# zouyunkai/MedicalSemSeg

Measured on AMD Instinct MI355X. Metric: 96^3 vols/sec fwd+bwd (train), higher is better.
Workload: dtype bf16; 1 GPU; UNet base (MONAI BasicUNet 32-32-64-128-256-32) 1->3cls, 96^3 patches, DiceCE + AdamW, per-GPU batch 2; global_batch=2, parallelism=dp1, grad_sync=none (single rank)

## Files before the change

### include/msseg.h

```cpp
#ifndef MSSEG_H_
#define MSSEG_H_

#include <stddef.h>
#include <stdint.h>

#ifdef __cplusplus
extern "C" {
#endif

#define MSSEG_ABI_VERSION 1

#define MSSEG_OK 0
#define MSSEG_EINVAL (-1)
#define MSSEG_ELAUNCH (-2)
#define MSSEG_EWORKSPACE (-3)

#define MSSEG_F32 0
#define MSSEG_BF16 1

typedef void* msseg_stream_t;

int msseg_abi_version(void);
const char* msseg_last_error(void);
int msseg_num_cus(void);

int msseg_ktimer_enable(int on);
int msseg_ktimer_reset(void);
int msseg_ktimer_count(void);
int msseg_ktimer_get(int i, char* name, int cap, float* ms);

size_t msseg_packed_weight_bytes(int M, int T, int K, int cout_block, int dtype);
int msseg_pack_weights(const float* src, void* dst, int dtype, int M, int M0, int T, int K, int K0,
                       long long s_m1, long long s_m0, long long s_t, long long s_k1, long long s_k0,
                       int flip, int cout_block, msseg_stream_t stream);
typedef struct msseg_pack_job {
    const float* src;
    void* dst;
    long long s_m1, s_m0, s_t, s_k1, s_k0;
    long long total;
    int M, M0, T, K, K0, flip, cout_block, nkb;
} msseg_pack_job;
int msseg_pack_weights_batch(const msseg_pack_job* jobs_dev, int njobs, long long max_total, long long sum_total, int dtype,
                             msseg_stream_t stream);
int msseg_cout_block(int M);
int msseg_conv3d_k3_cout_block(int N, int D, int H, int W, int Cout);
int msseg_conv3d_k3_variant(int N, int D, int H, int W, int Cout);
int msseg_conv3d_k3_kernel(int N, int D, int H, int W, int Cin, int Cout, int dtype);

int msseg_conv3d_k3_fwd(const void* x, long long ldx, const void* wp, const float* bias, void* y, long long ldy,
                        int N, int D, int H, int W, int Cin, int Cout, float* stats ,
                        void* scratch, size_t scratch_bytes, int dtype, msseg_stream_t stream);
int msseg_conv3d_k3_fwd_accumulate(const void* x, long long ldx, const void* wp, void* y, long long ldy, int N, int D, int H,
                                   int W, int Cin, int Cout, float* stats, void* scratch, size_t scratch_bytes, int dtype,
                                   msseg_stream_t stream);
int msseg_conv3d_k3_dgrad_inbwd(const void* dy, long long lddy, const void* wp, void* da, long long ldda, int N, int D,
                                int H, int W, int Cin, int Cout, const void* yraw, long long ldyraw, const void* act,
                                long long ldact, const float* fwd_stats, float slope, float eps, float* red,
                                float* dgamma, float* dbeta, int accumulate, void* scratch, size_t scratch_bytes,
                                int dtype, msseg_stream_t stream);
int msseg_conv3d_k3s2_fwd(const void* x, long long ldx, const void* wp, const float* bias, void* y, long long ldy,
                          int N, int ID, int IH, int IW, int Cin, int Cout, int dtype, msseg_stream_t stream);
int msseg_zero_stuff2(const void* dy, long long lddy, void* out, long long ldo, int N, int OD, int OH, int OW, int ID,
                      int IH, int IW, int C, int dtype, msseg_stream_t stream);
int msseg_conv3d_stem_fwd(const void* x, long long ldx, const void* wp, const float* bias, void* y, long long ldy,
                          int N, int D, int H, int W, int Cout, float* stats, void* scratch, size_t scratch_bytes,
                          int dtype, msseg_stream_t stream);
int msseg_conv3d_stem_k1_fwd(const void* x, long long ldx, const void* wp, const float* bias, void* y, long long ldy,
                             int N, int D, int H, int W, int Cout, float* stats, void* scratch, size_t scratch_bytes,
                             int dtype, msseg_stream_t stream);
int msseg_conv3d_stem_norm_fwd(const void* x, long long ldx, const void* wp, const float* bias, const float* stats,
                               const float* gamma, const float* beta, float eps, float slope, void* y, long long ldy, int N,
                               int D, int H, int W, int Cout, int dtype, msseg_stream_t stream);
int msseg_conv3d_k1_fwd(const void* x, long long ldx, const void* wp, const float* bias, void* y, long long ldy,
                        long long NV, int Cin, int Cout, int dtype, msseg_stream_t stream);
int msseg_conv3d_k1_head_fwd(const void* x, long long ldx, const float* w, const float* bias, void* y, long long ldy,
                             long long NV, int Cin, int Cout, int dtype, msseg_stream_t stream);
int msseg_conv3d_k1_head_dgrad_inbwd(const void* dy, long long lddy, const float* w, void* da, long long ldda, int N,
                                     long long S, int C, int Cout, const void* yraw, long long ldyraw,
                                     const float* fwd_stats, const float* gamma, const float* beta, float slope, float eps,
                                     float* red, float* dgamma, float* dbeta, int accumulate, void* scratch,
                                     size_t scratch_bytes, int dtype, msseg_stream_t stream);
int msseg_conv3d_k1_head_norm_fwd(const void* x, long long ldx, const float* stats, const float* gamma, const float* beta,
                                  float slope, float eps, const float* w, const float* bias, void* y, long long ldy, int N,
                                  long long S, int Cin, int Cout, int dtype, msseg_stream_t stream);
int msseg_conv3d_k1_head_bwd_fused(const void* dy, long long lddy, const float* w, void* da, long long ldda, int N,
                                   long long S, int C, int Cout, const void* yraw, long long ldyraw, const float* fwd_stats,
                                   const float* gamma, const float* beta, float slope, float eps, float* red, float* dgamma,
                                   float* dbeta, int accumulate, float* dw, int dw_accumulate, void* scratch,
                                   size_t scratch_bytes, int dtype, msseg_stream_t stream);

int msseg_conv3d_gather_fwd(const void* x, long long ldx, const void* wp, const float* bias, void* y, long long ldy,
                            int N, int ID, int IH, int IW, int Cin, int Cout, int k, int s, int p, int dtype,
                            msseg_stream_t stream);
int msseg_deconv_k2s2_fwd(const void* x, long long ldx, const void* wp, const float* bias, void* y, long long ldy,
                          int N, int D, int H, int W, int Cin, int Cout, int dtype, msseg_stream_t stream);
int msseg_deconv_k2s2_bwd_data(const void* dy, long long lddy, const void* wp, void* dx, long long lddx,
                               int N, int D, int H, int W, int Cin, int Cout, int dtype, msseg_stream_t stream);
int msseg_conv3d_k1_dgrad_inbwd(const void* dy, long long lddy, const void* wp, void* da, long long ldda, int N,
                                long long S, int Cin, int Cout, const void* yraw, long long ldyraw, const void* act,
                                long long ldact, const float* fwd_stats, float slope, float eps, float* red,
                                float* dgamma, float* dbeta, int accumulate, void* scratch, size_t scratch_bytes,
                                int dtype, msseg_stream_t stream);
int msseg_deconv_k2s2_bwd_data_inbwd(const void* dy, long long lddy, const void* wp, void* dx, long long lddx, int N,
                                     int D, int H, int W, int Cin, int Cout, const void* yraw, long long ldyraw,
                                     const void* act, long long ldact, const float* fwd_stats, float slope, float eps,
                                     float* red, float* dgamma, float* dbeta, int accumulate, void* scratch,
                                     size_t scratch_bytes, int dtype, msseg_stream_t stream);
int msseg_deconv_k2s2_bwd_fused(const void* dy, long long lddy, const void* wp, void* dx, long long lddx, int N,
                                int D, int H, int W, int Cin, int Cout, const void* yraw, long long ldyraw,
                                const void* act, long long ldact, const float* fwd_stats, float slope, float eps,
                                float* red, float* dgamma, float* dbeta, int accumulate, float* dbias, int dbias_accumulate,
                                void* scratch, size_t scratch_bytes, int dtype, msseg_stream_t stream);

int msseg_deconv_k2s2_bwd_partials_ok(int Cin, int Cout, int dtype);
int msseg_deconv_k2s2_bwd_partials(const void* dy, long long lddy, const void* wp, float* part, size_t part_bytes, int N,
                                   int D, int H, int W, int Cin, int Cout, int dtype, msseg_stream_t stream);


size_t msseg_wgrad_workspace_bytes(int M, int T, int K);
int msseg_conv3d_k3_wgrad_kernel(int N, int D, int H, int W, int Cin, int Cout, int dtype);
int msseg_conv3d_k3_wgrad(const void* x, long long ldx, const void* dy, long long lddy, float* dw,
                          int N, int D, int H, int W, int Cin, int Cout, int accumulate,
                          void* workspace, size_t workspace_bytes, int dtype, msseg_stream_t stream);
int msseg_conv3d_k1_wgrad(const void* x, long long ldx, const void* dy, long long lddy, float* dw,
                          long long NV, int Cin, int Cout, int accumulate,
                          void* workspace, size_t workspace_bytes, int dtype, msseg_stream_t stream);
int msseg_linear_wgrad_ok(long long NV, int Cin, int Cout, int dtype);
int msseg_linear_wgrad(const void* x, long long ldx, const void* dy, long long lddy, float* dw, float* dbias, long long NV,
                       int Cin, int Cout, int accumulate_w, int accumulate_b, void* workspace, size_t workspace_bytes,
                       int dtype, msseg_stream_t stream);
int msseg_conv3d_gather_wgrad(const void* x, long long ldx, const void* dy, long long lddy, float* dw,
                              int N, int ID, int IH, int IW, int Cin, int Cout, int k, int s, int p, int accumulate,
                              void* workspace, size_t workspace_bytes, int dtype, msseg_stream_t stream);
int msseg_deconv_k2s2_wgrad(const void* x, long long ldx, const void* dy, long long lddy, float* dw,
                            int N, int D, int H, int W, int Cin, int Cout, int accumulate,
                            void* workspace, size_t workspace_bytes, int dtype, msseg_stream_t stream);

int msseg_conv3d_k3_small_ok(int N, int D, int H, int W, int Cin, int Cout, int dtype);
int msseg_conv3d_k3_small_stage_groups(int N, int D, int H, int W, int Cin, int Cout);
size_t msseg_conv3d_k3_small_workspace_bytes(int N, int D, int H, int W, int Cin, int Cout);
int msseg_conv3d_k3_small_partials(const void* x, long long ldx, const void* wp, float* part, size_t part_bytes, int N,
                                   int D, int H, int W, int Cin, int Cout, msseg_stream_t stream);
int msseg_conv3d_k3_small_fwd_finish(const float* part, int nstages, const float* bias, const float* gamma,
                                     const float* beta, float eps, float slope, void* yraw, long long ldy, void* act,
                                     long long lda, void* pooled, long long ldp, float* stats, int N, int D, int H, int W,
                                     int Cout, msseg_stream_t stream);
int msseg_conv3d_k3_small_fwd_finish_res(const float* part, int nstages, const float* bias, const float* gamma,
                                         const float* beta, float eps, float slope, void* yraw, long long ldy, void* act,
                                         long long lda, const void* residual, long long ldr, void* pooled, long long ldp,
                                         float* stats, int N, int D, int H, int W, int Cout, msseg_stream_t stream);
int msseg_conv3d_k3_small_bwd_finish(const float* part, int nstages, void* dx, long long lddx, const void* unit_yraw,
                                     long long lduy, const float* unit_stats, const float* unit_gamma,
                                     const float* unit_beta, float eps, float slope, float* dgamma, float* dbeta,
                                     int accumulate, int N, int D, int H, int W, int Cin, msseg_stream_t stream);

int msseg_dwconv3d_k3_fwd(const void* x, long long ldx, const void* w_taps, const float* bias, void* y, long long ldy, int N,
                          int D, int H, int W, int C, int flip, int dtype, msseg_stream_t stream);
int msseg_avgpool3d_k3(const void* x, long long ldx, void* y, long long ldy, int N, int D, int H, int W, int C, int dtype,
                       msseg_stream_t stream);
int msseg_dwconv3d_k3_wgrad(const void* x, long long ldx, const void* dy, long long lddy, float* dw, float* dbias,
                            int accumulate_w, int accumulate_b, int N, int D, int H, int W, int C, void* scratch,
                            size_t scratch_bytes, int dtype, msseg_stream_t stream);

int msseg_interp_trilinear_fwd(const void* x, long long ldx, void* y, long long ldy, int N, int ID, int IH, int IW, int OD,
                               int OH, int OW, int C, int dtype, msseg_stream_t stream);
size_t msseg_interp_trilinear_bwd_workspace_bytes(int N, int ID, int IH, int IW, int OD, int OH, int OW, int C);
int msseg_interp_trilinear_bwd(const void* dy, long long lddy, void* dx, long long lddx, int N, int ID, int IH, int IW, int OD,
                               int OH, int OW, int C, void* workspace, size_t workspace_bytes, int dtype, msseg_stream_t stream);
int msseg_kv_attention_fwd(const void* q, const void* kv, void* o, float* lse, int B, int N, int M, int heads, int head_dim,
                           float scale, int dtype, msseg_stream_t stream);
size_t msseg_kv_attention_bwd_workspace_bytes(int B, int N, int M, int heads, int head_dim);
int msseg_kv_attention_bwd(const void* q, const void* kv, const void* o, const float* lse, const void* dout, void* dq, void* dkv,
                           int B, int N, int M, int heads, int head_dim, float scale, void* workspace, size_t workspace_bytes,
                           int dtype, msseg_stream_t stream);
int msseg_scale_channels(const void* x, const float* scale, void* y, int N, long long S, int C, int dtype, msseg_stream_t stream);

size_t msseg_reduce_scratch_bytes(void);
int msseg_channel_stats(const void* x, long long ldx, float* stats, int N, long long S, int C, void* scratch,
                        size_t scratch_bytes, int dtype, msseg_stream_t stream);
int msseg_instnorm_act_fwd(const void* x, long long ldx, const float* stats, const float* gamma, const float* beta,
                           const void* residual, long long ldr, void* y, long long ldy, int N, long long S, int C,
                           float eps, float slope, int dtype, msseg_stream_t stream);
int msseg_instnorm_act_pool_fwd(const void* x, long long ldx, const float* stats, const float* gamma, const float* beta,
                                void* y, long long ldy, void* pooled, long long ldp, int N, int D, int H, int W, int C,
                                float eps, float slope, int dtype, msseg_stream_t stream);
int msseg_instnorm_act_poolbwd_reduce(const void* x, long long ldx, const float* stats, const float* gamma,
                                      const float* beta, const void* skip, long long lds, const void* g, long long ldg,
                                      void* da, long long ldda, float* red, float* dgamma, float* dbeta, int accumulate,
                                      int N, int D, int H, int W, int C, float eps, float slope, void* scratch,
                                      size_t scratch_bytes, int dtype, msseg_stream_t stream);
int msseg_instnorm_act_bwd_reduce(const void* x, long long ldx, const float* stats, const float* gamma,
                                  const float* beta, const void* y, long long ldy,
                                  const void* dy, long long lddy, float* red, float* dgamma, float* dbeta,
                                  int accumulate, int N, long long S, int C, float eps, float slope, void* scratch,
                                  size_t scratch_bytes, int dtype, msseg_stream_t stream);
int msseg_instnorm_act_bwd_apply(const void* x, long long ldx, const float* stats, const float* gamma,
                                 const float* beta, const void* y, long long ldy, const void* dy, long long lddy, const float* red, void* dx,
                                 long long lddx, void* dres, long long lddres, int N, long long S, int C, float eps,
                                 float slope, int dtype, msseg_stream_t stream);
int msseg_maxpool2_fwd(const void* x, long long ldx, void* y, long long ldy, int N, int D, int H, int W, int C,
                       int dtype, msseg_stream_t stream);
int msseg_maxpool2_bwd(const void* x, long long ldx, const void* dy, long long lddy, void* dx, long long lddx,
                       int N, int D, int H, int W, int C, int accumulate, int dtype, msseg_stream_t stream);
int msseg_ncdhw_to_ndhwc(const void* src, int src_dtype, void* dst, long long ldd, int dst_dtype, int N, int C,
                         long long S, msseg_stream_t stream);
int msseg_ndhwc_to_ncdhw(const void* src, long long lds, int src_dtype, void* dst, int dst_dtype, int N, int C,
                         long long S, msseg_stream_t stream);
int msseg_channel_sum(const void* x, long long ldx, float* out, long long rows, int C, int accumulate, void* scratch,
                      size_t scratch_bytes, int dtype, msseg_stream_t stream);
int msseg_add(const void* a, long long lda, const void* b, long long ldb, void* y, long long ldy, long long rows,
              int C, int dtype, msseg_stream_t stream);
int msseg_axpy_rows(const void* a, const void* b, const float* scale, void* y, int N, long long elems_per_sample, int dtype,
                    msseg_stream_t stream);


int msseg_window_attention_fwd(const void* qkv, const float* qkv_bias, const float* table, void* out, float* lse, int B,
                               int S, int H, int W, int C, int heads, int ws, int shift, int dtype,
                               msseg_stream_t stream);
int msseg_window_attention_bwd(const void* qkv, const float* qkv_bias, const float* table, const void* out,
                               const float* lse, const void* dout, void* dqkv, float* dtable, int B, int S, int H, int W,
                               int C, int heads, int ws, int shift, int dtype, msseg_stream_t stream);
size_t msseg_window_attention_bwd_workspace_bytes(int B, int S, int H, int W, int C, int heads, int ws, int shift, int dtype);
int msseg_window_attention_fwd2(const void* qkv, const float* qkv_bias, const float* table, void* out, float* lse, int B,
                                int S, int H, int W, int C, int heads, int ws, int shift, int bias_ws, int dtype,
                                msseg_stream_t stream);
int msseg_window_attention_bwd2(const void* qkv, const float* qkv_bias, const float* table, const void* out,
                                const float* lse, const void* dout, void* dqkv, float* dtable, int B, int S, int H, int W,
                                int C, int heads, int ws, int shift, int bias_ws, int dtype, void* workspace,
                                size_t workspace_bytes, msseg_stream_t stream);
int msseg_window_attention_bwd_ws(const void* qkv, const float* qkv_bias, const float* table, const void* out,
                                  const float* lse, const void* dout, void* dqkv, float* dtable, int B, int S, int H, int W,
                                  int C, int heads, int ws, int shift, int dtype, void* workspace, size_t workspace_bytes,
                                  msseg_stream_t stream);
int msseg_window_attention_fwd3(const void* qkv, const float* qkv_bias, const float* table, void* out, float* lse, int B,
                                int S, int H, int W, int C, int heads, int ws, int shift, int bias_ws, long long table_stride,
                                int dtype, msseg_stream_t stream);
int msseg_window_attention_bwd3(const void* qkv, const float* qkv_bias, const float* table, const void* out,
                                const float* lse, const void* dout, void* dqkv, float* dtable, int B, int S, int H, int W,
                                int C, int heads, int ws, int shift, int bias_ws, long long table_stride, int dtype,
                                void* workspace, size_t workspace_bytes, msseg_stream_t stream);
size_t msseg_window_attention_bwd3_workspace_bytes(int B, int S, int H, int W, int C, int heads, int ws, int shift,
                                                   int bias_ws, long long table_stride, int dtype);
int msseg_rel_bias_affine_fold(const float* table, const float* emb, const float* lin_w, const float* lin_b,
                               const float* aff, float* T, int B, int M3, int heads, msseg_stream_t stream);
size_t msseg_rel_bias_affine_grad_workspace_bytes(int M3, int heads);
#define MSSEG_AFFINE_ACC_TABLE 1
#define MSSEG_AFFINE_ACC_EMB 2
#define MSSEG_AFFINE_ACC_LIN_W 4
#define MSSEG_AFFINE_ACC_LIN_B 8
int msseg_rel_bias_affine_grad(const float* dT, const float* emb, const float* lin_w, const float* aff, float* dtable,
                               float* demb, float* dlin_w, float* dlin_b, int B, int M3, int heads, int flags,
                               void* workspace, size_t workspace_bytes, msseg_stream_t stream);
int msseg_layernorm_fwd(const void* x, long long ldx, const float* gamma, const float* beta, void* y, long long ldy,
                        float* mean, float* rstd, long long rows, int C, float eps, int dtype, msseg_stream_t stream);
int msseg_layernorm_bwd(const void* x, long long ldx, const float* gamma, const float* mean, const float* rstd,
                        const void* dy, long long lddy, void* dx, long long lddx, long long rows, int C, int dtype,
                        msseg_stream_t stream);
int msseg_layernorm_bwd_add(const void* x, long long ldx, const float* gamma, const float* mean, const float* rstd,
                            const void* dy, long long lddy, const void* add, long long ldadd, void* dx, long long lddx,
                            long long rows, int C, int dtype, msseg_stream_t stream);
int msseg_layernorm_param_grad(const void* x, long long ldx, const float* mean, const float* rstd, const void* dy,
                               long long lddy, float* dgamma, float* dbeta, int accumulate, long long rows, int C,
                               void* scratch, size_t scratch_bytes, int dtype, msseg_stream_t stream);
int msseg_gelu_fwd(const void* x, void* y, long long n, int dtype, msseg_stream_t stream);
int msseg_gelu_bwd(const void* x, const void* dy, void* dx, long long n, int dtype, msseg_stream_t stream);
int msseg_linear_gelu_ok(long long NV, int Cin, int Cout, int dtype);
int msseg_linear_gelu_fwd(const void* x, long long ldx, const void* wp, const float* bias, void* pre, long long ldpre, void* act,
                          long long ldact, long long NV, int Cin, int Cout, int dtype, msseg_stream_t stream);
int msseg_linear_gelu_bwd(const void* dy, long long lddy, const void* wp, const void* pre, long long ldpre, void* dpre,
                          long long lddpre, long long NV, int Cin, int Cout, int dtype, msseg_stream_t stream);
int msseg_linear_add_ok(long long NV, int Cin, int Cout, int dtype);
int msseg_linear_add_fwd(const void* x, long long ldx, const void* wp, const float* bias, const void* res, long long ldres,
                         void* y, long long ldy, long long NV, int Cin, int Cout, int dtype, msseg_stream_t stream);

int msseg_dice_ce_partials(const void* logits, long long ld, int dtype, const void* labels, int label_dtype,
                           float* partial, float* hard, int N, long long S, int C, msseg_stream_t stream);
// ... 56 lines not shown
```

### medicalsemseg_amd/csrc/conv3d_k3_wgrad_pp.hip

```cpp
#include "k3pp.h"

#include <stdlib.h>

#include <type_traits>

namespace {

constexpr int TD = 4, TH = 4, TW = 16;
constexpr int PD = TD + 2, PH = TH + 2, PW = TW + 2;
constexpr int PWP = PW;
constexpr int HV = PD * PH * PWP;
constexpr int TV = TD * TH * TW;
constexpr int Q_BYTES = HV * 64;
constexpr int P_BYTES = TV * 64;
constexpr int GRP_BYTES = Q_BYTES + P_BYTES;
constexpr int NIQ = (HV + 15) / 16;
constexpr int NIP = TV / 16;
constexpr int NIQ_W = (NIQ + 3) / 4, NIP_W = NIP / 4;
constexpr int NKS = TV / 16;
constexpr int TAPW = 7;
constexpr int NTHREADS = 512;
constexpr int SLAB_FLOATS = 27 * 32 * 32;

__device__ u32x4_t g_wg_zero_chunk;
__device__ unsigned long long g_k3wg_cycles[8];

MSSEG_DEVFN void glds16(const void* g, void* l) {
    __builtin_amdgcn_global_load_lds((const __attribute__((address_space(1))) void*)g,
                                     (__attribute__((address_space(3))) void*)l, 16, 0, 0);
}

typedef __attribute__((address_space(3))) unsigned char lds_u8;
typedef __attribute__((ext_vector_type(16))) float f32x16_t;

MSSEG_DEVFN bf16x4_t lds_tr(lds_u8* p) {
    return __builtin_amdgcn_ds_read_tr16_b64_v4bf16((__attribute__((address_space(3))) bf16x4_t*)p);
}

MSSEG_DEVFN u32x4_t tr_frag(lds_u8* r0, lds_u8* r1) {
    const bf16x4_t lo = lds_tr(r0), hi = lds_tr(r1);
    const bf16x8_t f = {lo[0], lo[1], lo[2], lo[3], hi[0], hi[1], hi[2], hi[3]};
    return __builtin_bit_cast(u32x4_t, f);
}

struct TileCo { int n, d0, h0, w0; };

constexpr int ks_row(int ks) { return ((ks / TH) * PH + ks % TH) * PWP; }

template <int TIMING>
__global__ __launch_bounds__(NTHREADS, 1) void k3wg_pp_kernel(const K3WgParams p) {
    extern __shared__ __attribute__((aligned(256))) unsigned char smem[];
    const int tid = threadIdx.x, lane = tid & 63;
    const int wave = __builtin_amdgcn_readfirstlane(tid >> 6);
    const int grp = wave >> 2, wq = wave & 3;
    lds_u8* smem3 = (lds_u8*)smem;
    unsigned char* ldsQ = smem + grp * GRP_BYTES;
    unsigned char* ldsP = ldsQ + Q_BYTES;
    const int mblk = blockIdx.y / p.kblks, kblk = blockIdx.y % p.kblks;
    const unsigned char* pg = (const unsigned char*)p.pten + mblk * 64;
    const unsigned char* qg = (const unsigned char*)p.qten + kblk * 64;

    const int tiles_w = (p.W + TW - 1) / TW, tiles_h = (p.H + TH - 1) / TH, tiles_d = (p.D + TD - 1) / TD;
    const int ntiles = p.N * tiles_d * tiles_h * tiles_w;
    int t_first, t_step, t_end;
    if ((gridDim.x & 7) == 0) {
        const int chunk = (ntiles + 7) >> 3, xcd = blockIdx.x & 7;
        t_first = xcd * chunk + (blockIdx.x >> 3);
        t_step = gridDim.x >> 3;
        t_end = min(ntiles, (xcd + 1) * chunk);
    } else {
        t_first = blockIdx.x; t_step = gridDim.x; t_end = ntiles;
    }
    const int n_my = t_first < t_end ? (t_end - t_first + t_step - 1) / t_step : 0;
    auto tile_of = [&](int k) {
        int t = t_first + k * t_step;
        TileCo tc;
        tc.w0 = (t % tiles_w) * TW; t /= tiles_w;
        tc.h0 = (t % tiles_h) * TH; t /= tiles_h;
        tc.d0 = (t % tiles_d) * TD; t /= tiles_d;
        tc.n = t;
        return tc;
    };

    const int lrow = lane >> 2;
    const int lchunk = lane & 3;
    constexpr unsigned SKIP = 0xffffffffu;
    unsigned q_off[NIQ_W], p_off[NIP_W];
#pragma unroll
    for (int j = 0; j < NIQ_W; ++j) {
        const int hv = (wq + 4 * j) * 16 + lrow;
        const int hd = hv / (PH * PWP), rem = hv - hd * (PH * PWP), hh = rem / PWP, hw = rem - hh * PWP;
        q_off[j] = (hv < HV && hw < PW) ? (unsigned)((((long long)hd * p.H + hh) * p.W + hw) * p.ldq * 2 + lchunk * 16) : SKIP;
    }
#pragma unroll
    for (int j = 0; j < NIP_W; ++j) {
        const int tv = (wq + 4 * j) * 16 + lrow;
        const int td = tv / (TH * TW), th = (tv / TW) % TH, tw = tv % TW;
        p_off[j] = (unsigned)((((long long)td * p.H + th) * p.W + tw) * p.ldp * 2 + lchunk * 16);
    }
    const bool p_cok = mblk * 32 + lchunk * 8 < p.M, q_cok = kblk * 32 + lchunk * 8 < p.K;
    const bool chunks_full = (mblk + 1) * 32 <= p.M && (kblk + 1) * 32 <= p.K;
    auto load_tile = [&](const TileCo& tc) {
        const int dB = tc.d0 - 1, hB = tc.h0 - 1, wB = tc.w0 - 1;
        const long long qvox = (((long long)tc.n * p.D + dB) * p.H + hB) * p.W + wB;
        const long long pvox = (((long long)tc.n * p.D + tc.d0) * p.H + tc.h0) * p.W + tc.w0;
        const unsigned char* qb = qg + qvox * p.ldq * 2;
        const unsigned char* pb = pg + pvox * p.ldp * 2;
        const bool interior = chunks_full && dB >= 0 && dB + PD <= p.D && hB >= 0 && hB + PH <= p.H && wB >= 0 && wB + PW <= p.W;
        if (interior) {
#pragma unroll
            for (int j = 0; j < NIQ_W; ++j) {
                if (q_off[j] != SKIP) glds16(qb + q_off[j], ldsQ + (wq + 4 * j) * 1024);
            }
#pragma unroll
            for (int j = 0; j < NIP_W; ++j) glds16(pb + p_off[j], ldsP + (wq + 4 * j) * 1024);
        } else {
            const unsigned char* zsrc = (const unsigned char*)&g_wg_zero_chunk;
#pragma unroll
            for (int j = 0; j < NIQ_W; ++j) {
                const int it = wq + 4 * j;
                const int hv = it * 16 + lrow;
                const int hd = hv / (PH * PWP), rem = hv - hd * (PH * PWP), hh = rem / PWP, hw = rem - hh * PWP;
                const bool inb = q_cok && (unsigned)(dB + hd) < (unsigned)p.D && (unsigned)(hB + hh) < (unsigned)p.H &&
                                 (unsigned)(wB + hw) < (unsigned)p.W;
                const unsigned char* src = inb ? qb + q_off[j] : zsrc;
                if (q_off[j] != SKIP) glds16(src, ldsQ + it * 1024);
            }
#pragma unroll
            for (int j = 0; j < NIP_W; ++j) {
                const int tv = (wq + 4 * j) * 16 + lrow;
                const int td = tv / (TH * TW), th = (tv / TW) % TH, tw = tv % TW;
                const bool inb = p_cok && tc.d0 + td < p.D && tc.h0 + th < p.H && tc.w0 + tw < p.W;
                const unsigned char* src = inb ? pb + p_off[j] : zsrc;
                glds16(src, ldsP + (wq + 4 * j) * 1024);
            }
        }
    };

    const int G = lane >> 4, qr = (lane >> 2) & 3, pc = lane & 3;
    const unsigned qbase = grp * GRP_BYTES, pbase = qbase + Q_BYTES;
    unsigned p_rd[2], q_rd[TAPW][2];
#pragma unroll
    for (int i = 0; i < 2; ++i) {
        const int lrow = 8 * (G >> 1) + 4 * i + qr;
        p_rd[i] = pbase + lrow * 64 + ((G & 1) << 5) + pc * 8;
#pragma unroll
        for (int tt = 0; tt < TAPW; ++tt) {
            int tap = wq * TAPW + tt;
            if (tap > 26) tap = 26;
            const int row = ((tap / 9) * PH + ((tap / 3) % 3)) * PWP + (tap % 3) + lrow;
            q_rd[tt][i] = qbase + row * 64 + ((G & 1) << 5) + pc * 8;
        }
    }

    f32x16_t acc[TAPW];
#pragma unroll
    for (int t = 0; t < TAPW; ++t)
#pragma unroll
        for (int e = 0; e < 16; ++e) acc[t][e] = 0.f;

    auto compute = [&]() {
        constexpr int NSTEP = NKS * TAPW;
        constexpr int QA = 2;
        u32x4_t pf[2], qf[QA + 1];
        auto ldp = [&](int ks) { pf[ks & 1] = tr_frag(smem3 + p_rd[0] + ks * 1024, smem3 + p_rd[1] + ks * 1024); };
        auto ldq = [&](int s) {
            const int ks = s / TAPW, tt = s % TAPW;
            qf[s % (QA + 1)] = tr_frag(smem3 + q_rd[tt][0] + ks_row(ks) * 64, smem3 + q_rd[tt][1] + ks_row(ks) * 64);
        };
        ldp(0);
#pragma unroll
        for (int s = 0; s < QA; ++s) ldq(s);
#pragma unroll
        for (int ks = 0; ks < NKS; ++ks) {
#pragma unroll
            for (int tt = 0; tt < TAPW; ++tt) {
                const int s = ks * TAPW + tt;
                if (s + QA < NSTEP) ldq(s + QA);
                if (tt == 0 && ks + 1 < NKS) ldp(ks + 1);
                __builtin_amdgcn_sched_barrier(0);
                acc[tt] = __builtin_amdgcn_mfma_f32_32x32x16_bf16(__builtin_bit_cast(bf16x8_t, pf[ks & 1]),
                                                                  __builtin_bit_cast(bf16x8_t, qf[s % (QA + 1)]),
                                                                  acc[tt], 0, 0, 0);
                __builtin_amdgcn_sched_barrier(0);
            }
        }
    };

    if (grp == 0 && n_my > 0) load_tile(tile_of(0));
    asm volatile("s_waitcnt vmcnt(0)" ::: "memory");
    __syncthreads();

    unsigned long long tcyc[4] = {0, 0, 0, 0};
    for (int ph = 0; ph < n_my; ++ph) {
        unsigned long long t0 = 0;
        if constexpr (TIMING) t0 = __builtin_readcyclecounter();
        if ((ph & 1) == grp) {
            compute();
            if constexpr (TIMING) tcyc[0] += __builtin_readcyclecounter() - t0;
        } else {
            if (ph + 1 < n_my && !(TIMING && p.dbg_noload)) load_tile(tile_of(ph + 1));
            if constexpr (TIMING) tcyc[1] += __builtin_readcyclecounter() - t0;
        }
        if constexpr (TIMING) t0 = __builtin_readcyclecounter();
        asm volatile("s_waitcnt vmcnt(0)" ::: "memory");
        if constexpr (TIMING) { tcyc[2] += __builtin_readcyclecounter() - t0; t0 = __builtin_readcyclecounter(); }
        __syncthreads();
        if constexpr (TIMING) tcyc[3] += __builtin_readcyclecounter() - t0;
    }
    if constexpr (TIMING) {
        if (blockIdx.x == 0 && blockIdx.y == 0 && lane == 0 && wave == 0) {
#pragma unroll
            for (int k = 0; k < 4; ++k) g_k3wg_cycles[k] = tcyc[k];
        }
    }

    float* xch = (float*)smem;
    const int col = lane & 31, rb = 4 * (lane >> 5);
    const int tap0 = wq * TAPW;
    if (grp == 1) {
#pragma unroll
        for (int tt = 0; tt < TAPW; ++tt) {
            if (tap0 + tt < 27) {
#pragma unroll
                for (int e = 0; e < 16; ++e)
                    xch[((tap0 + tt) * 32 + (e & 3) + 8 * (e >> 2) + rb) * 32 + col] = acc[tt][e];
            }
        }
    }
    __syncthreads();
    if (grp == 0) {
        float* slab = p.slabs + ((long long)blockIdx.y * gridDim.x + blockIdx.x) * SLAB_FLOATS;
#pragma unroll
        for (int tt = 0; tt < TAPW; ++tt) {
            if (tap0 + tt < 27) {
#pragma unroll
                for (int e = 0; e < 16; ++e) {
                    const int idx = ((tap0 + tt) * 32 + (e & 3) + 8 * (e >> 2) + rb) * 32 + col;
                    slab[idx] = acc[tt][e] + xch[idx];
                }
            }
        }
    }
}

}

bool msseg_k3wg_pp_eligible(const K3WgParams& p) {
    static const bool off = getenv("MSSEG_NO_K3PP") != nullptr;
    if (off) return false;
    if (p.M % 8 || p.K % 8) return false;
    if ((p.ldp % 8) || (p.ldq % 8) || ((uintptr_t)p.pten & 15) || ((uintptr_t)p.qten & 15)) return false;
    const long long ldm = p.ldp > p.ldq ? p.ldp : p.ldq;
    if ((long long)(PD + 1) * p.H * p.W * ldm * 2 >= 0x7fffffffLL) return false;
    const long long tiles = (long long)p.N * ceil_div(p.D, TD) * ceil_div(p.H, TH) * ceil_div(p.W, TW);
    if (tiles > 0x7fffffffLL) return false;
    return tiles * ceil_div(p.M, 32) * ceil_div(p.K, 32) >= 2LL * msseg_num_cus();
}

int msseg_k3wg_pp_grid(const K3WgParams& p) {
    const int pairs = ceil_div(p.M, 32) * ceil_div(p.K, 32);
    const int tiles = p.N * ceil_div(p.D, TD) * ceil_div(p.H, TH) * ceil_div(p.W, TW);
    int gx = msseg_num_cus() / pairs;
    gx &= ~7;
    if (gx < 8) gx = 8;
    if (gx > tiles) gx = tiles;
    return gx;
}

int msseg_k3wg_pp_launch(const K3WgParams& p, int gx, hipStream_t stream) {
    static const bool timing = getenv("MSSEG_K3PP_TIMING") != nullptr;
    static const bool noload = getenv("MSSEG_K3PP_NOLOAD") != nullptr;
    K3WgParams pl = p;
    pl.dbg_noload = noload ? 1 : 0;
    const int lds = 2 * GRP_BYTES;
    static msseg_lds_attr_once attr[2];
    if (!attr[0].ensure((const void*)k3wg_pp_kernel<0>, lds) || !attr[1].ensure((const void*)k3wg_pp_kernel<1>, lds))
        MSSEG_FAIL(MSSEG_ELAUNCH, "conv3d_k3_wgrad_pp: cannot set dynamic LDS size %d", lds);
    const int pairs = ceil_div(p.M, 32) * ceil_div(p.K, 32);
    if (timing) hipLaunchKernelGGL(k3wg_pp_kernel<1>, dim3(gx, pairs, 1), dim3(NTHREADS), lds, stream, pl);
    else MSSEG_KTIMED("k3wg_pp_kernel", stream, hipLaunchKernelGGL(k3wg_pp_kernel<0>, dim3(gx, pairs, 1), dim3(NTHREADS), lds, stream, pl));
    MSSEG_CHECK_LAUNCH("conv3d_k3_wgrad_pp");
    return MSSEG_OK;
}

extern "C" int msseg_debug_k3wg_cycles(unsigned long long* out4) {
    return hipMemcpyFromSymbol(out4, HIP_SYMBOL(g_k3wg_cycles), 4 * sizeof(unsigned long long)) == hipSuccess ? 0 : -1;
}
```

### medicalsemseg_amd/csrc/elementwise.hip

```cpp
#include "common.h"

#include <stdarg.h>
#include <string.h>

static thread_local char g_err[512] = "";
void msseg_set_error(const char* fmt, ...) {
    va_list ap;
    va_start(ap, fmt);
    vsnprintf(g_err, sizeof(g_err), fmt, ap);
    va_end(ap);
}

extern "C" {
int msseg_abi_version(void) { return MSSEG_ABI_VERSION; }
const char* msseg_last_error(void) { return g_err; }
int msseg_num_cus(void) {
    static int cus = 0;
    if (cus == 0) {
        int dev = 0;
        hipDeviceProp_t prop;
        if (hipGetDevice(&dev) == hipSuccess && hipGetDeviceProperties(&prop, dev) == hipSuccess)
            cus = prop.multiProcessorCount;
        if (cus <= 0) cus = 256;
    }
    return cus;
}
}

namespace {

template <typename T> struct Chunk {
    static constexpr int EPC = DT<T>::EPC;
    float v[EPC];
    MSSEG_DEVFN void load(const T* p) {
        if constexpr (sizeof(T) == 4) {
            f32x4_t t = *(const f32x4_t*)p;
#pragma unroll
            for (int e = 0; e < 4; ++e) v[e] = t[e];
        } else {
            bf16x8_t t = *(const bf16x8_t*)p;
#pragma unroll
            for (int e = 0; e < 8; ++e) v[e] = (float)t[e];
        }
    }
    MSSEG_DEVFN void store(T* p) const {
        if constexpr (sizeof(T) == 4) {
            f32x4_t t = {v[0], v[1], v[2], v[3]};
            *(f32x4_t*)p = t;
        } else {
            bf16x8_t t;
#pragma unroll
            for (int e = 0; e < 8; ++e) t[e] = (bf16_t)v[e];
            *(bf16x8_t*)p = t;
        }
    }
};

inline bool vec_ok(const void* p, long long ld, int C, int esz) {
    const int epc = 16 / esz;
    return (C % epc) == 0 && (ld % epc) == 0 && (((uintptr_t)p) & 15) == 0;
}

struct RowMap {
    int groups;
    int rows_par;
};
inline RowMap row_map(int C, int width, int nthr = 256) {
    RowMap m;
    m.groups = ceil_div(C, width);
    if (m.groups > nthr) m.groups = nthr;
    m.rows_par = nthr / m.groups;
    if (m.rows_par < 1) m.rows_par = 1;
    return m;
}

MSSEG_DEVFN void finalize_channels(const float* ws, int N, int nblk, int C, int nper, int mode, float* out,
                                   float* dp0, float* dp1, int accumulate) {
    __shared__ float fin[256];
    const int L = C * nper;
    const int cols = L < 256 ? L : 256;
    const int G = 256 / cols;
    const int col = threadIdx.x % cols, rg = threadIdx.x / cols;
    const bool in256 = threadIdx.x < 256;
    const int n_step = mode == 0 ? (int)gridDim.y : 1, n_first = mode == 0 ? (int)blockIdx.y : 0;
    for (int c0 = blockIdx.x * cols; c0 < L; c0 += gridDim.x * cols) {
        const int o = c0 + col;
        const bool ok = in256 && o < L && rg < G;
        float tot = 0.f;
        for (int n = n_first; n < N; n += n_step) {
            float s = 0.f;
            if (ok) {
                const float* src = ws + (long long)n * nblk * L + o;
#pragma unroll 16
                for (int bb = rg; bb < nblk; bb += G) s += src[(long long)bb * L];
            }
            __syncthreads();
            if (in256) fin[threadIdx.x] = s;
            __syncthreads();
            if (ok && rg == 0) {
                float t = 0.f;
                for (int g = 0; g < G; ++g) t += fin[g * cols + col];
                if (mode != 1) out[(long long)n * L + o] = t;
                tot += t;
            }
        }
        if (ok && rg == 0) {
            if (mode == 1) {
                out[o] = accumulate ? out[o] + tot : tot;
            } else if (mode == 2) {
                const int c = o / nper, k = o % nper;
                float* dp = (k == 0) ? dp0 : dp1;
                if (dp) dp[c] = accumulate ? dp[c] + tot : tot;
            }
        }
    }
}

struct FinalizeArgs {
    const float* ws; int N, nblk, C, nper, mode; float* out; float* dp0; float* dp1; int accumulate;
};
__global__ __launch_bounds__(256) void channels_finalize_kernel(const FinalizeArgs a) {
    finalize_channels(a.ws, a.N, a.nblk, a.C, a.nper, a.mode, a.out, a.dp0, a.dp1, a.accumulate);
}

static inline dim3 channels_finalize_grid(const FinalizeArgs& a) {
    const int L = a.C * a.nper;
    int gx = (L + 255) / 256;
    if (gx > 64) gx = 64;
    if (gx < 1) gx = 1;
    return dim3((unsigned)gx, a.mode == 0 ? (unsigned)(a.N < 1 ? 1 : a.N) : 1u);
}

constexpr int RED_THREADS = 512;
constexpr int RED_STAGE2 = 16;

template <int W>
MSSEG_DEVFN void block_rows_reduce(float* red, int groups, int rows_par, int g, int rl, bool act) {
    if (act && rl < RED_STAGE2 && rl < rows_par) {
#pragma unroll
        for (int e = 0; e < W; ++e) {
            float a = 0.f, b = 0.f;
            for (int k = rl; k < rows_par; k += RED_STAGE2) {
                a += red[((k * groups + g) * W + e) * 2 + 0];
                b += red[((k * groups + g) * W + e) * 2 + 1];
            }
            red[((rl * groups + g) * W + e) * 2 + 0] = a;
            red[((rl * groups + g) * W + e) * 2 + 1] = b;
        }
    }
    __syncthreads();
}

template <typename T, bool VEC>
// ... 44 lines not shown
#pragma unroll
            for (int e = 0; e < W; ++e) {
                float a = 0.f, b = 0.f;
                for (int k = 0; k < kmax; ++k) {
                    a += red[((k * groups + g) * W + e) * 2 + 0];
                    b += red[((k * groups + g) * W + e) * 2 + 1];
                }
                const int c = gg * W + e;
                wsb[c * nacc + 0] = a;
                if (nacc == 2) wsb[c * nacc + 1] = b;
            }
        }
    }
}

template <typename T, bool VEC>
__global__ __launch_bounds__(256) void ln_param_grad_kernel(const T* __restrict__ x, long long ldx,
                                                            const T* __restrict__ dy, long long lddy,
                                                            const float* __restrict__ mean, const float* __restrict__ rstd,
                                                            long long rows, int C, int groups, int rows_par,
                                                            long long rows_per_block, float* ws, unsigned int* counter,
                                                            float* dgamma, float* dbeta, int accumulate) {
    constexpr int W = VEC ? DT<T>::EPC : 1;
    __shared__ float red[256 * 2 * (VEC ? DT<T>::EPC : 1)];
    __shared__ int lflag;
    const int g = threadIdx.x % groups, rl = threadIdx.x / groups;
    const long long r0 = (long long)blockIdx.x * rows_per_block;
    long long r1 = r0 + rows_per_block;
    if (r1 > rows) r1 = rows;
    float* wsb = ws + (long long)blockIdx.x * C * 2;
    for (int gbase = 0; gbase * W < C; gbase += groups) {
        const int gg = gbase + g;
        const bool act = gg * W < C;
        float s[W], s2[W];
#pragma unroll
        for (int e = 0; e < W; ++e) s[e] = s2[e] = 0.f;
        if (act && rl < rows_par) {
#pragma unroll 4
            for (long long r = r0 + rl; r < r1; r += rows_par) {
                const float mu = mean[r], rs = rstd[r];
                if constexpr (VEC) {
                    Chunk<T> cx, cd;
                    cx.load(x + r * ldx + gg * W);
                    cd.load(dy + r * lddy + gg * W);
#pragma unroll
                    for (int e = 0; e < W; ++e) { s[e] += cd.v[e] * (cx.v[e] - mu) * rs; s2[e] += cd.v[e]; }
                } else {
                    const float d = DT<T>::ld(dy + r * lddy + gg);
                    s[0] += d * (DT<T>::ld(x + r * ldx + gg) - mu) * rs;
                    s2[0] += d;
                }
            }
        }
        __syncthreads();
#pragma unroll
        for (int e = 0; e < W; ++e) {
            red[(threadIdx.x * W + e) * 2 + 0] = s[e];
            red[(threadIdx.x * W + e) * 2 + 1] = s2[e];
        }
        __syncthreads();
        if (act && rl == 0) {
#pragma unroll
            for (int e = 0; e < W; ++e) {
                float a = 0.f, b = 0.f;
                for (int k = 0; k < rows_par; ++k) {
                    a += red[((k * groups + g) * W + e) * 2 + 0];
                    b += red[((k * groups + g) * W + e) * 2 + 1];
                }
                wsb[(gg * W + e) * 2 + 0] = a;
                wsb[(gg * W + e) * 2 + 1] = b;
            }
        }
    }
}

inline long long reduce_blocks(long long S, int rows_par, int N, int C, int nper);

template <typename T>
int launch_ln_param_grad(const void* x, long long ldx, const void* dy, long long lddy, const float* mean, const float* rstd,
                         float* dgamma, float* dbeta, int accumulate, long long rows, int C, void* scratch, hipStream_t st) {
    const bool vec = vec_ok(x, ldx, C, sizeof(T)) && vec_ok(dy, lddy, C, sizeof(T));
    const RowMap m = row_map(C, vec ? DT<T>::EPC : 1);
    long long blocks = reduce_blocks(rows, m.rows_par, 1, C, 2);
    const long long rpb = ceil_div_ll(rows, blocks);
    blocks = ceil_div_ll(rows, rpb);
    unsigned int* counter = (unsigned int*)scratch;
    float* ws = (float*)((unsigned char*)scratch + MSSEG_SCRATCH_COUNTER_BYTES);
    if (vec)
        hipLaunchKernelGGL((ln_param_grad_kernel<T, true>), dim3((unsigned)blocks), dim3(256), 0, st, (const T*)x, ldx,
                           (const T*)dy, lddy, mean, rstd, rows, C, m.groups, m.rows_par, rpb, ws, counter, dgamma, dbeta, accumulate);
    else
        hipLaunchKernelGGL((ln_param_grad_kernel<T, false>), dim3((unsigned)blocks), dim3(256), 0, st, (const T*)x, ldx,
                           (const T*)dy, lddy, mean, rstd, rows, C, m.groups, m.rows_par, rpb, ws, counter, dgamma, dbeta, accumulate);
    MSSEG_CHECK_LAUNCH("ln_param_grad");
    {
        FinalizeArgs a{ws, 1, (int)blocks, C, 2, 2, ws + blocks * C * 2, dgamma, dbeta, accumulate};
        hipLaunchKernelGGL(channels_finalize_kernel, channels_finalize_grid(a), dim3(256), 0, st, a);
        MSSEG_CHECK_LAUNCH("channels_finalize");
    }
    return MSSEG_OK;
}

inline long long reduce_blocks(long long S, int rows_par, int N, int C, int nper) {
    long long blocks = ceil_div_ll(S, (long long)rows_par * 8);
    long long cap = (long long)msseg_num_cus() / (N > 0 ? N : 1);
    if (cap < 1) cap = 1;
    const long long fit = (long long)(((size_t)16 << 20) / ((size_t)N * C * nper * 4));
    if (cap > fit) cap = fit;
    if (blocks > cap) blocks = cap;
    if (blocks < 1) blocks = 1;
    return blocks;
}

template <typename T>
int launch_stats(const void* x, long long ldx, float* out, int N, long long S, int C, int nacc, int accumulate,
                 void* scratch, hipStream_t st) {
    const bool vec = vec_ok(x, ldx, C, sizeof(T));
    const RowMap m = row_map(C, vec ? DT<T>::EPC : 1, RED_THREADS);
    long long blocks = reduce_blocks(S, m.rows_par, N, C, nacc);
    const long long rpb = ceil_div_ll(S, blocks);
    blocks = ceil_div_ll(S, rpb);
    dim3 grid((unsigned)blocks, N);
    unsigned int* counter = (unsigned int*)scratch;
    float* ws = (float*)((unsigned char*)scratch + MSSEG_SCRATCH_COUNTER_BYTES);
    if (vec)
        hipLaunchKernelGGL((channel_stats_kernel<T, true>), grid, dim3(RED_THREADS), 0, st, (const T*)x, ldx, out, S, C,
                           m.groups, m.rows_par, rpb, nacc, accumulate, ws, counter);
    else
        hipLaunchKernelGGL((channel_stats_kernel<T, false>), grid, dim3(RED_THREADS), 0, st, (const T*)x, ldx, out, S, C,
                           m.groups, m.rows_par, rpb, nacc, accumulate, ws, counter);
    MSSEG_CHECK_LAUNCH("channel_stats");
    {
        FinalizeArgs a{ws, N, (int)blocks, C, nacc, nacc == 2 ? 0 : 1, out, nullptr, nullptr, accumulate};
        hipLaunchKernelGGL(channels_finalize_kernel, channels_finalize_grid(a), dim3(256), 0, st, a);
        MSSEG_CHECK_LAUNCH("channels_finalize");
    }
    return MSSEG_OK;
}

struct NormParams {
    const void* x; long long ldx;
    const float* stats; const float* gamma; const float* beta;
    const void* res; long long ldr;
    void* y; long long ldy;
    const void* dy; long long lddy;
    float* red;
    void* dx; long long lddx;
    void* dres; long long lddres;
    long long S; int C; float eps, slope;
    long long rows_per_block; int groups, rows_par;
    float* ws; unsigned int* counter; float* dgamma; float* dbeta; int accumulate;
};

MSSEG_DEVFN void mean_rstd(const float* stats, int n, int C, int c, long long S, float eps, float& mean, float& rstd) {
    const float inv = 1.0f / (float)S;
    const float s = stats[((long long)n * C + c) * 2 + 0], s2 = stats[((long long)n * C + c) * 2 + 1];
    mean = s * inv;
    float var = s2 * inv - mean * mean;
    var = var > 0.f ? var : 0.f;
    rstd = rsqrtf(var + eps);
}

template <typename T, bool VEC, int MODE>
__global__ __launch_bounds__(MODE == 1 ? RED_THREADS : 256) void instnorm_kernel(const NormParams p) {
    constexpr int W = VEC ? DT<T>::EPC : 1;
    __shared__ float red[(MODE == 1) ? RED_THREADS * 2 * W : 1];
    __shared__ int lflag;
    const int n = blockIdx.y;
    const int g = threadIdx.x % p.groups, rl = threadIdx.x / p.groups;
    const long long r0 = (long long)blockIdx.x * p.rows_per_block;
    long long r1 = r0 + p.rows_per_block;
    if (r1 > p.S) r1 = p.S;
    const T* xn = (const T*)p.x + (long long)n * p.S * p.ldx;
    const T* yn = (MODE != 0 && p.y != nullptr) ? (const T*)p.y + (long long)n * p.S * p.ldy : nullptr;
    T* yo = (MODE == 0) ? (T*)p.y + (long long)n * p.S * p.ldy : nullptr;
    const T* dyn = (MODE != 0) ? (const T*)p.dy + (long long)n * p.S * p.lddy : nullptr;
    const T* resn = (MODE == 0 && p.res) ? (const T*)p.res + (long long)n * p.S * p.ldr : nullptr;
    T* dxn = (MODE == 2) ? (T*)p.dx + (long long)n * p.S * p.lddx : nullptr;
    T* drn = (MODE == 2 && p.dres) ? (T*)p.dres + (long long)n * p.S * p.lddres : nullptr;
    const float invS = 1.0f / (float)p.S;

    for (int gbase = 0; gbase * W < p.C; gbase += p.groups) {
        const int gg = gbase + g;
        const bool act = gg * W < p.C;
        float mean[W], rstd[W], sc[W], sh[W], k0[W], k1[W], a0[W], a1[W];
#pragma unroll
        for (int e = 0; e < W; ++e) {
            const int c = act ? gg * W + e : 0;
            mean_rstd(p.stats, n, p.C, c, p.S, p.eps, mean[e], rstd[e]);
            const float ga = p.gamma ? p.gamma[c] : 1.f;
            sc[e] = rstd[e] * ga;
            sh[e] = (p.beta ? p.beta[c] : 0.f) - mean[e] * sc[e];
            a0[e] = a1[e] = 0.f;
            if constexpr (MODE == 2) {
                k0[e] = p.red[((long long)n * p.C + c) * 2 + 0] * invS;
                k1[e] = p.red[((long long)n * p.C + c) * 2 + 1] * invS;
            }
        }
        if (act && rl < p.rows_par) {
#pragma unroll 4
            for (long long r = r0 + rl; r < r1; r += p.rows_par) {
                float xv[W], o[W], yv[W], dv[W];
                if constexpr (VEC) {
                    Chunk<T> c; c.load(xn + r * p.ldx + gg * W);
#pragma unroll
                    for (int e = 0; e < W; ++e) xv[e] = c.v[e];
                } else {
                    xv[0] = DT<T>::ld(xn + r * p.ldx + gg);
                }
                if constexpr (MODE == 0) {
                    float rv[W];
#pragma unroll
                    for (int e = 0; e < W; ++e) rv[e] = 0.f;
                    if (resn) {
                        if constexpr (VEC) {
                            Chunk<T> c; c.load(resn + r * p.ldr + gg * W);
#pragma unroll
                            for (int e = 0; e < W; ++e) rv[e] = c.v[e];
                        } else {
                            rv[0] = DT<T>::ld(resn + r * p.ldr + gg);
                        }
                    }
#pragma unroll
                    for (int e = 0; e < W; ++e) {
                        const float z = xv[e] * sc[e] + sh[e] + rv[e];
                        o[e] = z > 0.f ? z : z * p.slope;
                    }
                    if constexpr (VEC) {
                        Chunk<T> c;
#pragma unroll
                        for (int e = 0; e < W; ++e) c.v[e] = o[e];
                        c.store(yo + r * p.ldy + gg * W);
                    } else {
                        DT<T>::st(yo + r * p.ldy + gg, o[0]);
                    }
                } else {
                    if constexpr (VEC) {
                        Chunk<T> d; d.load(dyn + r * p.lddy + gg * W);
#pragma unroll
                        for (int e = 0; e < W; ++e) dv[e] = d.v[e];
                        if (yn != nullptr) {
                            Chunk<T> c; c.load(yn + r * p.ldy + gg * W);
#pragma unroll
                            for (int e = 0; e < W; ++e) yv[e] = c.v[e];
                        } else {
#pragma unroll
                            for (int e = 0; e < W; ++e) yv[e] = xv[e] * sc[e] + sh[e];
                        }
                    } else {
                        dv[0] = DT<T>::ld(dyn + r * p.lddy + gg);
                        yv[0] = (yn != nullptr) ? DT<T>::ld(yn + r * p.ldy + gg) : xv[0] * sc[0] + sh[0];
                    }
#pragma unroll
                    for (int e = 0; e < W; ++e) {
                        const float dz = yv[e] > 0.f ? dv[e] : dv[e] * p.slope;
                        const float xh = (xv[e] - mean[e]) * rstd[e];
                        if constexpr (MODE == 1) {
                            a0[e] += dz;
                            a1[e] += dz * xh;
                        } else {
                            o[e] = sc[e] * (dz - k0[e] - xh * k1[e]);
                            dv[e] = dz;
                        }
                    }
                    if constexpr (MODE == 2) {
                        if constexpr (VEC) {
                            Chunk<T> c;
#pragma unroll
                            for (int e = 0; e < W; ++e) c.v[e] = o[e];
                            c.store(dxn + r * p.lddx + gg * W);
                            if (drn) {
#pragma unroll
                                for (int e = 0; e < W; ++e) c.v[e] = dv[e];
                                c.store(drn + r * p.lddres + gg * W);
                            }
                        } else {
                            DT<T>::st(dxn + r * p.lddx + gg, o[0]);
                            if (drn) DT<T>::st(drn + r * p.lddres + gg, dv[0]);
                        }
                    }
                }
            }
        }
        if constexpr (MODE == 1) {
            __syncthreads();
#pragma unroll
            for (int e = 0; e < W; ++e) {
                red[(threadIdx.x * W + e) * 2 + 0] = a0[e];
                red[(threadIdx.x * W + e) * 2 + 1] = a1[e];
            }
            __syncthreads();
            block_rows_reduce<W>(red, p.groups, p.rows_par, g, rl, act);
            if (act && rl == 0) {
                const int kmax = p.rows_par < RED_STAGE2 ? p.rows_par : RED_STAGE2;
#pragma unroll
                for (int e = 0; e < W; ++e) {
                    float a = 0.f, b = 0.f;
                    for (int k = 0; k < kmax; ++k) {
                        a += red[((k * p.groups + g) * W + e) * 2 + 0];
                        b += red[((k * p.groups + g) * W + e) * 2 + 1];
                    }
                    const int c = gg * W + e;
                    float* wsb = p.ws + ((long long)n * gridDim.x + blockIdx.x) * p.C * 2;
                    wsb[c * 2 + 0] = a;
                    wsb[c * 2 + 1] = b;
                }
            }
        }
    }
}

struct NormPoolParams {
    const void* x; long long ldx;
    const float* stats; const float* gamma; const float* beta;
    void* y; long long ldy;
    void* pooled; long long ldp;
    int N, D, H, W, C; float eps, slope;
};

template <typename T>
__global__ __launch_bounds__(256) void instnorm_pool_fwd_kernel(const NormPoolParams p) {
    constexpr int WD = DT<T>::EPC;
    const int OD = p.D / 2, OH = p.H / 2, OW = p.W / 2;
    const unsigned ug = (unsigned)(p.C / WD);
    const unsigned total = (unsigned)((long long)p.N * OD * OH * OW * ug);
    const long long S = (long long)p.D * p.H * p.W;
    for (unsigned i = blockIdx.x * 256u + threadIdx.x; i < total; i += gridDim.x * 256u) {
        unsigned t = i / ug;
        const int g = (int)(i - t * ug);
        unsigned t2 = t / (unsigned)OW;
        const int ow = (int)(t - t2 * (unsigned)OW);
        t = t2 / (unsigned)OH;
        const int oh = (int)(t2 - t * (unsigned)OH);
        const int n = (int)(t / (unsigned)OD);
        const int od = (int)(t - (unsigned)n * (unsigned)OD);
        float sc[WD], sh[WD], best[WD];
#pragma unroll
        for (int e = 0; e < WD; ++e) {
            const int c = g * WD + e;
            float mean, rstd;
            mean_rstd(p.stats, n, p.C, c, S, p.eps, mean, rstd);
            sc[e] = rstd * (p.gamma ? p.gamma[c] : 1.f);
            sh[e] = (p.beta ? p.beta[c] : 0.f) - mean * sc[e];
            best[e] = -INFINITY;
        }
        Chunk<T> in[8];
#pragma unroll
        for (int k = 0; k < 8; ++k) {
            const long long vox = (((long long)n * p.D + 2 * od + (k >> 2)) * p.H + 2 * oh + ((k >> 1) & 1)) * p.W + 2 * ow + (k & 1);
            in[k].load((const T*)p.x + vox * p.ldx + g * WD);
        }
#pragma unroll
        for (int k = 0; k < 8; ++k) {
            const long long vox = (((long long)n * p.D + 2 * od + (k >> 2)) * p.H + 2 * oh + ((k >> 1) & 1)) * p.W + 2 * ow + (k & 1);
            Chunk<T> o;
#pragma unroll
            for (int e = 0; e < WD; ++e) {
                const float z = in[k].v[e] * sc[e] + sh[e];
                const float a = (float)(T)(z > 0.f ? z : z * p.slope);
                o.v[e] = a;
                if (a > best[e] || a != a) best[e] = a;
            }
            o.store((T*)p.y + vox * p.ldy + g * WD);
        }
        Chunk<T> b;
#pragma unroll
        for (int e = 0; e < WD; ++e) b.v[e] = best[e];
        const long long ovox = (((long long)n * OD + od) * OH + oh) * OW + ow;
        b.store((T*)p.pooled + ovox * p.ldp + g * WD);
    }
}

struct NormPoolBwdParams {
    const void* x; long long ldx;
    const float* stats; const float* gamma; const float* beta;
    const void* skip; long long lds;
    const void* g; long long ldg;
    void* da; long long ldda;
    int N, D, H, W, C; float eps, slope;
    int groups, rows_par; long long cells_per_block;
    float* ws;
};

template <typename T>
__global__ __launch_bounds__(RED_THREADS) void instnorm_poolbwd_reduce_kernel(const NormPoolBwdParams p) {
    constexpr int WD = DT<T>::EPC;
    __shared__ float red[RED_THREADS * 2 * WD];
    const int n = blockIdx.y;
    const int g = threadIdx.x % p.groups, rl = threadIdx.x / p.groups;
    const int OD = p.D / 2, OH = p.H / 2, OW = p.W / 2;
    const long long cells = (long long)OD * OH * OW, S = (long long)p.D * p.H * p.W;
    const long long c0 = (long long)blockIdx.x * p.cells_per_block;
    long long c1 = c0 + p.cells_per_block;
    if (c1 > cells) c1 = cells;
    const T* xn = (const T*)p.x + (long long)n * S * p.ldx;
    const T* sn = (const T*)p.skip + (long long)n * S * p.lds;
    const T* gn = (const T*)p.g + (long long)n * cells * p.ldg;
    T* dn = (T*)p.da + (long long)n * S * p.ldda;
    for (int gbase = 0; gbase * WD < p.C; gbase += p.groups) {
        const int gg = gbase + g;
        const bool act = gg * WD < p.C;
        float mean[WD], rstd[WD], sc[WD], sh[WD], a0[WD], a1[WD];
#pragma unroll
        for (int e = 0; e < WD; ++e) {
            const int c = act ? gg * WD + e : 0;
            mean_rstd(p.stats, n, p.C, c, S, p.eps, mean[e], rstd[e]);
            sc[e] = rstd[e] * (p.gamma ? p.gamma[c] : 1.f);
            sh[e] = (p.beta ? p.beta[c] : 0.f) - mean[e] * sc[e];
            a0[e] = a1[e] = 0.f;
        }
        if (act && rl < p.rows_par) {
            for (long long cell = c0 + rl; cell < c1; cell += p.rows_par) {
                const int ow = (int)(cell % OW), oh = (int)((cell / OW) % OH), od = (int)(cell / ((long long)OW * OH));
                Chunk<T> xin[8], gv;
// ... 1082 lines not shown
```

### medicalsemseg_amd/csrc/igemm_wgrad.hip

```cpp
#include "common.h"
#include "k3pp.h"

#include <stdlib.h>

namespace {

enum { Q_DIRECT = 0, Q_GATHER = 1, Q_DECONV = 2 };

struct WgradParams {
    const void* pten;
    long long ldp;
    const void* qten;
    long long ldq;
    float* slabs;
    int N, D, H, W;
    int ID, IH, IW;
    int OD, OH, OW;
    int M, K;
    int mblks, kblks;
    int tiles_d, tiles_h, tiles_w, ntiles;
    int cin, k, s, p;
    int creal;
    int rel32_ok;
};
// ... 407 lines not shown
    const int nk = min(32, p.K - kb * 32);
    float* dst = p.dw + (long long)m * p.s_m0 + (long long)kb * 32 * T;
    for (int o = threadIdx.x; o < nk * T; o += 256) {
        const int k = o / T, t = o - k * T;
        dst[o] = p.accumulate ? dst[o] + tile[t][k] : tile[t][k];
    }
}

int launch_reduce(const ReduceParams& rp, hipStream_t stream) {
    const long long total = (long long)rp.M * rp.T * rp.K;
    if (total >= 0x7fffffffLL) MSSEG_FAIL(MSSEG_EINVAL, "wgrad: weight tensor too large");
    const bool conv_layout = rp.s_t == 1 && rp.s_k0 == rp.T && rp.K0 == rp.K && rp.M0 == rp.M && rp.T > 1 && rp.T <= 32 &&
                             rp.s_m0 == (long long)rp.K * rp.T && (rp.cbw == 32 || rp.cbw == 16);
    static const bool no_rows = getenv("MSSEG_NO_REDUCE_ROWS") != nullptr;
    if (rp.nslots <= 32 && conv_layout && !no_rows && ceil_div(rp.K, 32) <= 65535) {
        hipLaunchKernelGGL(wgrad_reduce_rows_kernel, dim3(rp.M, ceil_div(rp.K, 32)), dim3(256), 0, stream, rp);
    } else if (rp.nslots <= 32) {
        int rb = (int)((total + 255) / 256);
        if (rb > 8192) rb = 8192;
        hipLaunchKernelGGL(wgrad_reduce_small_kernel, dim3(rb), dim3(256), 0, stream, rp);
    } else {
        int rb = (int)((total + 31) / 32);
        if (rb > 4096) rb = 4096;
        hipLaunchKernelGGL(wgrad_reduce_kernel, dim3(rb), dim3(256), 0, stream, rp);
    }
    MSSEG_CHECK_LAUNCH("wgrad_reduce");
    return MSSEG_OK;
}

template <typename T, int NTAPS, int QSRC, int TD, int TH, int TW>
int launch_wg(WgradParams& p, ReduceParams& rp, void* workspace, size_t ws_bytes, hipStream_t stream) {
    using C = WgCfg<T, NTAPS, TD, TH, TW>;
    p.tiles_d = ceil_div(p.D, TD);
    p.tiles_h = ceil_div(p.H, TH);
    p.tiles_w = ceil_div(p.W, TW);
    const long long nt = (long long)p.N * p.tiles_d * p.tiles_h * p.tiles_w;
    if (nt > 0x7fffffffLL) MSSEG_FAIL(MSSEG_EINVAL, "wgrad: too many tiles");
    p.ntiles = (int)nt;
    p.mblks = ceil_div(p.M, C::CBW);
    p.kblks = ceil_div(p.K, C::CBW);
    {
        const long long ldm = p.ldp > p.ldq ? p.ldp : p.ldq;
        p.rel32_ok = ((long long)(C::PD + 1) * p.H * p.W * ldm < 0x7fffffffLL) ? 1 : 0;
    }
    const int pairs = p.mblks * p.kblks;
    const int wave_slots = 1;
    const size_t slab_bytes = (size_t)C::SLAB_FLOATS * 4;
    long long gx = msseg_num_cus() * ((C::LDS_BYTES > 80 * 1024) ? 1 : 2);
    static const int flat_per_cu = getenv("MSSEG_WG_FLAT_PER_CU") ? atoi(getenv("MSSEG_WG_FLAT_PER_CU")) : 3;
    if (NTAPS == 1 && C::LDS_BYTES * flat_per_cu <= 160 * 1024) gx = (long long)msseg_num_cus() * flat_per_cu;
    static const int wgs_env = getenv("MSSEG_WG_TOTAL") ? atoi(getenv("MSSEG_WG_TOTAL")) : 0;
    if (NTAPS == 27 && (long long)p.ntiles * pairs <= 4LL * msseg_num_cus()) gx = wgs_env > 0 ? wgs_env : msseg_num_cus() / 2;
    if (pairs > 1) gx = (gx + pairs - 1) / pairs;
    if (gx > p.ntiles) gx = p.ntiles;
    const long long fit = (long long)(ws_bytes / (slab_bytes * pairs * wave_slots));
    if (fit < 1) MSSEG_FAIL(MSSEG_EWORKSPACE, "wgrad: workspace %zu B too small (need >= %zu)", ws_bytes,
                            slab_bytes * pairs * wave_slots);
    if (gx > fit) gx = fit;
    if (gx < 1) gx = 1;
    p.slabs = (float*)workspace;
    auto kern = igemm_wgrad_kernel<T, NTAPS, QSRC, TD, TH, TW>;
    static msseg_lds_attr_once attr;
    if (!attr.ensure((const void*)kern, C::LDS_BYTES)) MSSEG_FAIL(MSSEG_ELAUNCH, "wgrad: cannot set dynamic LDS size %d", C::LDS_BYTES);
    MSSEG_KTIMED(NTAPS == 27 ? "igemm_wgrad_kernel<27>" : "igemm_wgrad_kernel<flat>", stream,
                 hipLaunchKernelGGL(kern, dim3((unsigned)gx, pairs, 1), dim3(256), C::LDS_BYTES, stream, p));
    MSSEG_CHECK_LAUNCH("igemm_wgrad");
    rp.slabs = p.slabs;
    rp.mblks = p.mblks; rp.kblks = p.kblks; rp.nslots = (int)gx * wave_slots; rp.cbw = C::CBW;
    return launch_reduce(rp, stream);
}

template <typename T> int launch_wg_k3(WgradParams& p, ReduceParams& rp, void* ws, size_t wsb, hipStream_t st) {
    if constexpr (sizeof(T) == 2) {
        K3WgParams pp{};
        pp.pten = p.pten; pp.ldp = p.ldp; pp.qten = p.qten; pp.ldq = p.ldq;
        pp.N = p.N; pp.D = p.D; pp.H = p.H; pp.W = p.W; pp.M = p.M; pp.K = p.K; pp.kblks = ceil_div(p.K, 32);
        static const int pp_min_dim = getenv("MSSEG_K3WG_MINDIM") ? atoi(getenv("MSSEG_K3WG_MINDIM")) : 8;
        const int mnd = p.D < p.H ? (p.D < p.W ? p.D : p.W) : (p.H < p.W ? p.H : p.W);
        if (mnd >= pp_min_dim && msseg_k3wg_pp_eligible(pp)) {
            const int pairs = ceil_div(p.M, 32) * ceil_div(p.K, 32);
            int gx = msseg_k3wg_pp_grid(pp);
            const long long fit = (long long)(wsb / ((size_t)27 * 32 * 32 * 4 * pairs));
            if (fit >= 8) {
                if (gx > fit) gx = (int)(fit & ~7LL);
                pp.slabs = (float*)ws;
                const int rc = msseg_k3wg_pp_launch(pp, gx, st);
                if (rc) return rc;
                rp.slabs = pp.slabs;
                rp.mblks = ceil_div(p.M, 32); rp.kblks = ceil_div(p.K, 32); rp.nslots = gx; rp.cbw = 32;
                return launch_reduce(rp, st);
            }
        }
    }
    const int mn = p.D < p.H ? (p.D < p.W ? p.D : p.W) : (p.H < p.W ? p.H : p.W);
    if (mn >= 32) {
        static const bool two_wg = getenv("MSSEG_WGRAD_2WG") != nullptr;
        if (two_wg) return launch_wg<T, 27, Q_DIRECT, 2, 8, 16>(p, rp, ws, wsb, st);
        return launch_wg<T, 27, Q_DIRECT, 4, 8, 16>(p, rp, ws, wsb, st);
    }
    if (mn >= 12) return launch_wg<T, 27, Q_DIRECT, 4, 4, 8>(p, rp, ws, wsb, st);
    return launch_wg<T, 27, Q_DIRECT, 2, 4, 8>(p, rp, ws, wsb, st);
}

int wg_check(const void* a, long long lda, const void* b, long long ldb, const void* dw, const void* ws, int dtype) {
    if (!a || !b || !dw || !ws) MSSEG_FAIL(MSSEG_EINVAL, "wgrad: null pointer");
    if (dtype != MSSEG_F32 && dtype != MSSEG_BF16) MSSEG_FAIL(MSSEG_EINVAL, "wgrad: bad dtype");
    const int esz = dtype == MSSEG_F32 ? 4 : 2;
    if ((((uintptr_t)a | (uintptr_t)b | (uintptr_t)ws) & 15) || (lda * esz) % 16 || (ldb * esz) % 16)
        MSSEG_FAIL(MSSEG_EINVAL, "wgrad: operands must be 16-byte aligned with 16-byte row strides");
    return MSSEG_OK;
}

}

bool msseg_lwg_deconv_ok(int dtype, long long NV, int Cin, int Cout, const void* x, long long ldx, const void* dy, long long lddy);
int msseg_lwg_deconv_wgrad(const void* x, long long ldx, const void* dy, long long lddy, float* dw, int N, int D, int H, int W,
                           int Cin, int Cout, int accumulate, void* workspace, size_t workspace_bytes, hipStream_t stream);

extern "C" {

size_t msseg_wgrad_workspace_bytes(int M, int T, int K) {
    const size_t padM = (size_t)((M + 31) / 32) * 32, padK = (size_t)((K + 31) / 32) * 32;
    const size_t per_slot = padM * padK * (size_t)T * 4;
    size_t slots = 256;
    while (slots > 8 && per_slot * slots * (T == 1 ? 4 : 1) > ((size_t)256 << 20)) slots /= 2;
    return per_slot * slots * (T == 1 ? 4 : 1);
}

int msseg_conv3d_k3_wgrad_kernel(int N, int D, int H, int W, int Cin, int Cout, int dtype) {
    if (dtype != MSSEG_BF16) return 0;
    K3WgParams pp{};
    pp.pten = (const void*)256; pp.ldp = Cout; pp.qten = (const void*)256; pp.ldq = Cin;
    pp.N = N; pp.D = D; pp.H = H; pp.W = W; pp.M = Cout; pp.K = Cin; pp.kblks = ceil_div(Cin, 32);
    return msseg_k3wg_pp_eligible(pp) ? 3 : 0;
}

int msseg_conv3d_k3_wgrad(const void* x, long long ldx, const void* dy, long long lddy, float* dw, int N, int D, int H,
                          int W, int Cin, int Cout, int accumulate, void* workspace, size_t workspace_bytes, int dtype,
                          msseg_stream_t stream) {
    int rc = wg_check(x, ldx, dy, lddy, dw, workspace, dtype);
    if (rc) return rc;
    const int esz = dtype == MSSEG_F32 ? 4 : 2;
    if (Cin % (16 / esz)) MSSEG_FAIL(MSSEG_EINVAL, "conv3d_k3_wgrad: Cin %% %d != 0", 16 / esz);
    WgradParams p{};
    p.pten = dy; p.ldp = lddy; p.qten = x; p.ldq = ldx;
    p.N = N; p.D = D; p.H = H; p.W = W; p.M = Cout; p.K = Cin;
    ReduceParams rp{};
    rp.dw = dw; rp.M = Cout; rp.M0 = Cout; rp.T = 27; rp.K = Cin; rp.K0 = Cin;
    rp.s_m1 = 0; rp.s_m0 = (long long)Cin * 27; rp.s_t = 1; rp.s_k1 = 0; rp.s_k0 = 27; rp.accumulate = accumulate;
    return dtype == MSSEG_F32 ? launch_wg_k3<float>(p, rp, workspace, workspace_bytes, (hipStream_t)stream)
                              : launch_wg_k3<bf16_t>(p, rp, workspace, workspace_bytes, (hipStream_t)stream);
}

int msseg_conv3d_k1_wgrad(const void* x, long long ldx, const void* dy, long long lddy, float* dw, long long NV, int Cin,
                          int Cout, int accumulate, void* workspace, size_t workspace_bytes, int dtype,
                          msseg_stream_t stream) {
    int rc = wg_check(x, ldx, dy, lddy, dw, workspace, dtype);
    if (rc) return rc;
    const int esz = dtype == MSSEG_F32 ? 4 : 2;
    if (Cin % (16 / esz) || NV < 1 || NV > 0x7fffffffLL) MSSEG_FAIL(MSSEG_EINVAL, "conv3d_k1_wgrad: bad shape");
    WgradParams p{};
    p.pten = dy; p.ldp = lddy; p.qten = x; p.ldq = ldx;
    p.N = 1; p.D = 1; p.H = 1; p.W = (int)NV; p.M = Cout; p.K = Cin;
    ReduceParams rp{};
    rp.dw = dw; rp.M = Cout; rp.M0 = Cout; rp.T = 1; rp.K = Cin; rp.K0 = Cin;
    rp.s_m0 = Cin; rp.s_k0 = 1; rp.accumulate = accumulate;
    return dtype == MSSEG_F32
               ? launch_wg<float, 1, Q_DIRECT, 1, 1, 256>(p, rp, workspace, workspace_bytes, (hipStream_t)stream)
               : launch_wg<bf16_t, 1, Q_DIRECT, 1, 1, 256>(p, rp, workspace, workspace_bytes, (hipStream_t)stream);
}

int msseg_conv3d_gather_wgrad(const void* x, long long ldx, const void* dy, long long lddy, float* dw, int N, int ID,
                              int IH, int IW, int Cin, int Cout, int k, int s, int pd, int accumulate, void* workspace,
                              size_t workspace_bytes, int dtype, msseg_stream_t stream) {
    if (!x || !dy || !dw || !workspace) MSSEG_FAIL(MSSEG_EINVAL, "conv3d_gather_wgrad: null pointer");
    if (dtype != MSSEG_F32 && dtype != MSSEG_BF16) MSSEG_FAIL(MSSEG_EINVAL, "conv3d_gather_wgrad: bad dtype");
    const int esz = dtype == MSSEG_F32 ? 4 : 2;
    if (((uintptr_t)dy & 15) || (lddy * esz) % 16) MSSEG_FAIL(MSSEG_EINVAL, "conv3d_gather_wgrad: dy alignment");
    if (k < 1 || s < 1 || pd < 0) MSSEG_FAIL(MSSEG_EINVAL, "conv3d_gather_wgrad: bad kernel");
    const int OD = (ID + 2 * pd - k) / s + 1, OH = (IH + 2 * pd - k) / s + 1, OW = (IW + 2 * pd - k) / s + 1;
    const long long NV = (long long)N * OD * OH * OW;
    if (OD < 1 || OH < 1 || OW < 1 || NV > 0x7fffffffLL) MSSEG_FAIL(MSSEG_EINVAL, "conv3d_gather_wgrad: bad shape");
    const int KT = k * k * k;
    if (msseg_stem_eligible(dtype, Cin, Cout, k, s, pd, ldx, lddy, dy) && (lddy % 8) == 0 &&
        workspace_bytes >= (size_t)8 * 4096 * ceil_div(Cout, 32)) {
        StemWgParams sp{};
        sp.x = x; sp.ldx = ldx; sp.dy = dy; sp.lddy = lddy; sp.N = N; sp.D = ID; sp.H = IH; sp.W = IW; sp.M = Cout;
        int gx = msseg_stem_wgrad_grid(sp);
        const long long fit = (long long)(workspace_bytes / ((size_t)4096 * ceil_div(Cout, 32)));
        if (gx > fit) gx = (int)(fit & ~7LL);
        sp.slabs = (float*)workspace;
        int rc = msseg_stem_wgrad_launch(sp, gx, (hipStream_t)stream);
        if (rc) return rc;
        ReduceParams rq{};
        rq.dw = dw; rq.M = Cout; rq.M0 = Cout; rq.T = 1; rq.K = KT; rq.K0 = 1;
        rq.s_m0 = KT; rq.s_k1 = 1; rq.s_k0 = KT; rq.accumulate = accumulate;
        rq.slabs = sp.slabs + (k == 1 ? 13 : 0); rq.mblks = ceil_div(Cout, 32); rq.kblks = 1; rq.nslots = gx; rq.cbw = 32;
        return launch_reduce(rq, (hipStream_t)stream);
    }
    WgradParams p{};
    p.pten = dy; p.ldp = lddy; p.qten = x; p.ldq = ldx;
    p.N = 1; p.D = 1; p.H = 1; p.W = (int)NV; p.M = Cout; p.K = Cin * KT;
    p.ID = ID; p.IH = IH; p.IW = IW; p.OD = OD; p.OH = OH; p.OW = OW; p.cin = Cin; p.k = k; p.s = s; p.p = pd;
    ReduceParams rp{};
    rp.dw = dw; rp.M = Cout; rp.M0 = Cout; rp.T = 1; rp.K = Cin * KT; rp.K0 = Cin;
    rp.s_m0 = (long long)Cin * KT; rp.s_k1 = 1; rp.s_k0 = KT; rp.accumulate = accumulate;
    return dtype == MSSEG_F32
               ? launch_wg<float, 1, Q_GATHER, 1, 1, 256>(p, rp, workspace, workspace_bytes, (hipStream_t)stream)
               : launch_wg<bf16_t, 1, Q_GATHER, 1, 1, 256>(p, rp, workspace, workspace_bytes, (hipStream_t)stream);
}

int msseg_deconv_k2s2_wgrad(const void* x, long long ldx, const void* dy, long long lddy, float* dw, int N, int D, int H,
                            int W, int Cin, int Cout, int accumulate, void* workspace, size_t workspace_bytes,
                            int dtype, msseg_stream_t stream) {
    int rc = wg_check(x, ldx, dy, lddy, dw, workspace, dtype);
    if (rc) return rc;
    const int esz = dtype == MSSEG_F32 ? 4 : 2;
    const long long NV = (long long)N * D * H * W;
    if (Cout % (16 / esz) || NV < 1 || NV > 0x7fffffffLL / 8) MSSEG_FAIL(MSSEG_EINVAL, "deconv_k2s2_wgrad: bad shape");
    if (msseg_lwg_deconv_ok(dtype, NV, Cin, Cout, x, ldx, dy, lddy))
        return msseg_lwg_deconv_wgrad(x, ldx, dy, lddy, dw, N, D, H, W, Cin, Cout, accumulate, workspace, workspace_bytes,
                                      (hipStream_t)stream);
    WgradParams p{};
    p.pten = x; p.ldp = ldx; p.qten = dy; p.ldq = lddy;
    p.N = 1; p.D = 1; p.H = 1; p.W = (int)NV; p.M = Cin; p.K = 8 * Cout;
    p.OD = D; p.OH = H; p.OW = W; p.creal = Cout;
    ReduceParams rp{};
    rp.dw = dw; rp.M = Cin; rp.M0 = Cin; rp.T = 1; rp.K = 8 * Cout; rp.K0 = Cout;
    rp.s_m0 = (long long)Cout * 8; rp.s_k1 = 1; rp.s_k0 = 8; rp.accumulate = accumulate;
    return dtype == MSSEG_F32
               ? launch_wg<float, 1, Q_DECONV, 1, 1, 256>(p, rp, workspace, workspace_bytes, (hipStream_t)stream)
               : launch_wg<bf16_t, 1, Q_DECONV, 1, 1, 256>(p, rp, workspace, workspace_bytes, (hipStream_t)stream);
}

}
```

### medicalsemseg_amd/csrc/k3pp.h

```cpp
#pragma once
#include "common.h"

struct K3ppParams {
    const void* x;
    long long ldx;
    const void* wp;
    const float* bias;
    void* y;
    long long ldy;
    int N, D, H, W, K, M;
    float* stats;
    float* stats_ws;
    unsigned int* counter;
    const void* nb_y; long long nb_ldy;
    const void* nb_a; long long nb_lda;
    const float* nb_stats;
    float nb_slope, nb_eps; long long nb_S;
    float* nb_dgamma; float* nb_dbeta; int nb_acc;
    int accumulate;
};

bool msseg_k3pp_eligible(const K3ppParams& p);
int msseg_k3pp_launch(const K3ppParams& p, hipStream_t stream);

bool msseg_k3c48_shape_ok(int N, int D, int H, int W, int M);
bool msseg_k3c48_eligible(const K3ppParams& p);
int msseg_k3c48_launch(const K3ppParams& p, hipStream_t stream);

struct K3FinParams {
    const float* ws;
    int R, N, coutb, M;
    float* stats;
    const float* nb_stats;
    float nb_eps; long long nb_S;
    float* nb_dgamma; float* nb_dbeta; int nb_acc;
};
int msseg_k3_stats_finalize(const K3FinParams& f, int ncb, hipStream_t stream);

struct K3WgParams {
    const void* pten; long long ldp;
    const void* qten; long long ldq;
    float* slabs;
    int N, D, H, W, M, K, kblks;
    int dbg_noload;
};
bool msseg_k3wg_pp_eligible(const K3WgParams& p);
int msseg_k3wg_pp_grid(const K3WgParams& p);
int msseg_k3wg_pp_launch(const K3WgParams& p, int gx, hipStream_t stream);

struct StemParams {
    const void* x; long long ldx;
    const void* wp;
    const float* bias;
    void* y; long long ldy;
    int N, D, H, W, M;
    float* stats; float* stats_ws;
    int taps;
    const float* nstats; const float* gamma; const float* beta; float eps, slope;
};
struct StemWgParams {
    const void* x; long long ldx;
    const void* dy; long long lddy;
    float* slabs;
    int N, D, H, W, M;
};
bool msseg_stem_eligible(int dtype, int Cin, int Cout, int k, int s, int pd, long long ldx, long long ldy, const void* y);
int msseg_stem_fwd_launch(const StemParams& p, hipStream_t stream);
int msseg_stem_wgrad_grid(const StemWgParams& p);
int msseg_stem_wgrad_launch(const StemWgParams& p, int gx, hipStream_t stream);

bool msseg_deconv2_fast_eligible(int dtype, int Cin, int Cout, const void* coarse, long long ldc, const void* fine,
                                 long long ldf, const float* bias);
int msseg_deconv2_fwd_launch(const void* x, long long ldx, const void* wp, const float* bias, void* y, long long ldy, int N,
                             int D, int H, int W, int Cin, int Cout, hipStream_t stream);
int msseg_deconv2_bwd_launch(const void* dy, long long lddy, const void* wp, void* dx, long long lddx, int N, int D, int H,
                             int W, int Cin, int Cout, const void* yraw, long long ldyraw, const void* act, long long ldact,
                             const float* fwd_stats, float slope, float eps, float* red, float* dgamma, float* dbeta,
                             int accumulate, float* dbias, int dbias_accumulate, void* scratch, size_t scratch_bytes,
                             hipStream_t stream);

bool msseg_deconv2g_fwd_eligible(int dtype, int Cin, int Cout, const void* coarse, long long ldc, const void* fine,
                                 long long ldf, const float* bias);
int msseg_deconv2g_fwd_launch(const void* x, long long ldx, const void* wp, const float* bias, void* y, long long ldy, int N,
                              int D, int H, int W, int Cin, int Cout, hipStream_t stream);
bool msseg_deconv2g_bwd_eligible(int dtype, int Cin, int Cout, const void* coarse, long long ldc, const void* fine,
                                 long long ldf);
int msseg_deconv2g_bwd_launch(const void* dy, long long lddy, const void* wp, void* dx, long long lddx, float* part, int N,
                              int D, int H, int W, int Cin, int Cout, hipStream_t stream);
bool msseg_linear_regw_eligible(int dtype, long long NV, int Cin, int Cout, const void* x, long long ldx, const void* y,
                                long long ldy, const float* bias);
int msseg_linear_regw_launch(const void* x, long long ldx, const void* wp, const float* bias, void* y, long long ldy,
                             long long NV, int Cin, int Cout, hipStream_t stream);
```

### medicalsemseg_amd/csrc/stem_conv.hip

```cpp
#include "k3pp.h"

namespace {

constexpr int TD = 4, TH = 4, TW = 16;
constexpr int PD = TD + 2, PH = TH + 2, PW = TW + 2;
constexpr int HV = PD * PH * PW;

typedef __attribute__((address_space(3))) unsigned char lds_u8;
typedef __attribute__((ext_vector_type(16))) float f32x16_t;

struct TileCo { int n, d0, h0, w0; };

struct Sched {
    int tiles_w, tiles_h, tiles_d, t_first, t_step, n_my;
    MSSEG_DEVFN void init(int N, int D, int H, int W) {
        tiles_w = (W + TW - 1) / TW; tiles_h = (H + TH - 1) / TH; tiles_d = (D + TD - 1) / TD;
        const int ntiles = N * tiles_d * tiles_h * tiles_w;
        int t_end;
        if ((gridDim.x & 7) == 0) {
            const int chunk = (ntiles + 7) >> 3, xcd = blockIdx.x & 7;
            t_first = xcd * chunk + (blockIdx.x >> 3);
            t_step = gridDim.x >> 3;
            t_end = min(ntiles, (xcd + 1) * chunk);
        } else {
            t_first = blockIdx.x; t_step = gridDim.x; t_end = ntiles;
        }
        n_my = t_first < t_end ? (t_end - t_first + t_step - 1) / t_step : 0;
    }
    MSSEG_DEVFN TileCo tile(int k) const {
        int t = t_first + k * t_step;
        TileCo tc;
        tc.w0 = (t % tiles_w) * TW; t /= tiles_w;
        tc.h0 = (t % tiles_h) * TH; t /= tiles_h;
        tc.d0 = (t % tiles_d) * TD; t /= tiles_d;
        tc.n = t;
        return tc;
    }
};

constexpr int F_THREADS = 512;
template <int STATS, int JT, int NORM = 0>
__global__ __launch_bounds__(F_THREADS) void stem_fwd_kernel(const StemParams p) {
    constexpr int CBW = JT * 16;
    constexpr int F_STAT_FLOATS = 8 * MSSEG_STATS_NMAX * CBW * 2;
    __shared__ __attribute__((aligned(16))) unsigned short halo[2][HV + 8];
    __shared__ float ldsS[STATS ? F_STAT_FLOATS : 1];
    const int tid = threadIdx.x, lane = tid & 63;
    const int wave = __builtin_amdgcn_readfirstlane(tid >> 6);
    const int r = lane & 15, q = lane >> 4;
    const int coutblk = blockIdx.y;
    const unsigned short* __restrict__ xg = (const unsigned short*)p.x;
    bf16_t* __restrict__ yg = (bf16_t*)p.y;
    Sched sc;
    sc.init(p.N, p.D, p.H, p.W);

    u32x4_t wf[JT];
#pragma unroll
    for (int jt = 0; jt < JT; ++jt)
        wf[jt] = *(const u32x4_t*)((const unsigned char*)p.wp + (long long)coutblk * (4 * CBW * 16) + (q * CBW + jt * 16 + r) * 16);
    f32x4_t bv[JT];
#pragma unroll
    for (int jt = 0; jt < JT; ++jt) {
        bv[jt] = f32x4_t{0.f, 0.f, 0.f, 0.f};
        if (p.bias) bv[jt] = *(const f32x4_t*)(p.bias + coutblk * CBW + jt * 16 + q * 4);
    }
    const int ntaps = p.taps == 1 ? 1 : 27;
    int toff[8];
#pragma unroll
    for (int j = 0; j < 8; ++j) {
        const int k = q * 8 + j;
        toff[j] = ntaps == 1 ? (PH + 1) * PW + 1 : ((k < 27) ? ((k / 9) * PH + ((k / 3) % 3)) * PW + (k % 3) : 0);
    }
    if (STATS) {
        for (int i = tid; i < F_STAT_FLOATS; i += F_THREADS) ldsS[i] = 0.f;
    }
    float nsc[NORM ? JT : 1][4], nsh[NORM ? JT : 1][4];
    int n_n = -1;
    auto load_norm = [&](int n) {
        if constexpr (NORM != 0) {
            const float inv = 1.0f / (float)((long long)p.D * p.H * p.W);
#pragma unroll
            for (int jt = 0; jt < JT; ++jt)
#pragma unroll
                for (int e = 0; e < 4; ++e) {
                    const int c = coutblk * CBW + jt * 16 + q * 4 + e;
                    const float su = p.nstats[((long long)n * p.M + c) * 2 + 0], su2 = p.nstats[((long long)n * p.M + c) * 2 + 1];
                    const float mean = su * inv;
                    float var = su2 * inv - mean * mean;
                    var = var > 0.f ? var : 0.f;
                    const float rstd = rsqrtf(var + p.eps);
                    nsc[jt][e] = rstd * (p.gamma ? p.gamma[c] : 1.f);
                    nsh[jt][e] = (p.beta ? p.beta[c] : 0.f) - mean * nsc[jt][e];
                }
        }
    };
    float s1[JT][4], s2[JT][4];
    int s_n = -1;
#pragma unroll
    for (int jt = 0; jt < JT; ++jt)
#pragma unroll
        for (int e = 0; e < 4; ++e) s1[jt][e] = s2[jt][e] = 0.f;
    auto flush_stats = [&]() {
        if (s_n < 0) return;
        float* slot = ldsS + ((wave * MSSEG_STATS_NMAX + s_n) * CBW) * 2;
#pragma unroll
        for (int jt = 0; jt < JT; ++jt)
#pragma unroll
            for (int e = 0; e < 4; ++e) {
                float a = s1[jt][e], b = s2[jt][e];
#pragma unroll
                for (int o = 1; o < 16; o <<= 1) {
                    a += __shfl_xor(a, o);
                    b += __shfl_xor(b, o);
                }
                if (r == 0) {
                    float* sp = slot + (jt * 16 + q * 4 + e) * 2;
                    sp[0] += a;
                    sp[1] += b;
                }
                s1[jt][e] = s2[jt][e] = 0.f;
            }
    };

    unsigned short st[2];
    auto fetch = [&](const TileCo& tc) {
#pragma unroll
        for (int it = 0; it < 2; ++it) {
            const int hv = tid + it * F_THREADS;
            const int hd = hv / (PH * PW), rem = hv - hd * (PH * PW), hh = rem / PW, hw = rem - hh * PW;
            const int d = tc.d0 - 1 + hd, h = tc.h0 - 1 + hh, w = tc.w0 - 1 + hw;
            const bool inb = hv < HV && (unsigned)d < (unsigned)p.D && (unsigned)h < (unsigned)p.H && (unsigned)w < (unsigned)p.W;
            st[it] = inb ? xg[((((long long)tc.n * p.D + d) * p.H + h) * p.W + w) * p.ldx] : (unsigned short)0;
        }
    };
    auto commit = [&](int buf) {
#pragma unroll
        for (int it = 0; it < 2; ++it) {
            const int hv = tid + it * F_THREADS;
            if (hv < HV) halo[buf][hv] = st[it];
        }
    };

    if (sc.n_my > 0) {
        fetch(sc.tile(0));
        commit(0);
    }
    __syncthreads();
    const int dw = wave >> 1, h2 = (wave & 1) * 2;
    for (int k = 0; k < sc.n_my; ++k) {
        const TileCo tc = sc.tile(k);
        if (k + 1 < sc.n_my) fetch(sc.tile(k + 1));
        const unsigned short* hb = halo[k & 1];
        if constexpr (STATS != 0) {
            if (tc.n != s_n) { flush_stats(); s_n = tc.n; }
        }
        if constexpr (NORM != 0) {
            if (tc.n != n_n) { load_norm(tc.n); n_n = tc.n; }
        }
#pragma unroll
        for (int m = 0; m < 2; ++m) {
            const int hrow = h2 + m;
            const int base = (dw * PH + hrow) * PW + r;
            unsigned short v[8];
#pragma unroll
            for (int j = 0; j < 8; ++j) v[j] = hb[base + toff[j]];
            u32x4_t xf;
#pragma unroll
            for (int j = 0; j < 4; ++j) xf[j] = (unsigned)v[2 * j] | ((unsigned)v[2 * j + 1] << 16);
            const int d = tc.d0 + dw, h = tc.h0 + hrow, w = tc.w0 + r;
            const bool ok = d < p.D && h < p.H && w < p.W;
            const long long vox = (((long long)tc.n * p.D + d) * p.H + h) * p.W + w;
#pragma unroll
            for (int jt = 0; jt < JT; ++jt) {
                f32x4_t acc = {0.f, 0.f, 0.f, 0.f};
                mma_chunk<bf16_t>(acc, wf[jt], xf);
                const f32x4_t o = acc + bv[jt];
                const bf16x4_t ob = {(bf16_t)o[0], (bf16_t)o[1], (bf16_t)o[2], (bf16_t)o[3]};
                if constexpr (NORM != 0) {
                    bf16x4_t oa;
#pragma unroll
                    for (int e = 0; e < 4; ++e) {
                        const float z = (float)ob[e] * nsc[jt][e] + nsh[jt][e];
                        oa[e] = (bf16_t)(z > 0.f ? z : z * p.slope);
                    }
                    if (ok) *(bf16x4_t*)(yg + vox * p.ldy + coutblk * CBW + jt * 16 + q * 4) = oa;
                } else {
                    if (ok && yg != nullptr) *(bf16x4_t*)(yg + vox * p.ldy + coutblk * CBW + jt * 16 + q * 4) = ob;
                }
                if constexpr (STATS != 0) {
#pragma unroll
                    for (int e = 0; e < 4; ++e) {
                        const float rv = ok ? (float)ob[e] : 0.f;
                        s1[jt][e] += rv;
                        s2[jt][e] += rv * rv;
                    }
                }
            }
        }
        if (k + 1 < sc.n_my) commit((k + 1) & 1);
        __syncthreads();
    }
    if constexpr (STATS != 0) {
        flush_stats();
        __syncthreads();
        const int PN = p.N * CBW * 2;
        float* wsp = p.stats_ws + ((long long)blockIdx.y * gridDim.x + blockIdx.x) * PN;
        for (int i = tid; i < PN; i += F_THREADS) {
            float s = 0.f;
#pragma unroll
            for (int wv = 0; wv < 8; ++wv) s += ldsS[wv * MSSEG_STATS_NMAX * CBW * 2 + i];
            wsp[i] = s;
        }
    }
}

constexpr int W_THREADS = 256;
constexpr int XP = 24;
constexpr int XS_ELEMS = PD * PH * XP;
constexpr int P_BYTES = TD * TH * TW * 64;

__device__ u32x4_t g_stem_zero_chunk;

MSSEG_DEVFN void glds16(const void* g, void* l) {
    __builtin_amdgcn_global_load_lds((const __attribute__((address_space(1))) void*)g,
                                     (__attribute__((address_space(3))) void*)l, 16, 0, 0);
}
MSSEG_DEVFN bf16x4_t lds_tr(lds_u8* p) {
    return __builtin_amdgcn_ds_read_tr16_b64_v4bf16((__attribute__((address_space(3))) bf16x4_t*)p);
}

__global__ __launch_bounds__(W_THREADS) void stem_wgrad_kernel(const StemWgParams p) {
    extern __shared__ __attribute__((aligned(256))) unsigned char smem[];
    constexpr int BUF_BYTES = P_BYTES + 3 * XS_ELEMS * 2 + 64;
    lds_u8* smem3 = (lds_u8*)smem;
    const int tid = threadIdx.x, lane = tid & 63;
    const int wave = __builtin_amdgcn_readfirstlane(tid >> 6);
    const int mblk = blockIdx.y;
    const unsigned char* dyg = (const unsigned char*)p.dy + mblk * 64;
    const unsigned short* __restrict__ xg = (const unsigned short*)p.x;
    Sched sc;
    sc.init(p.N, p.D, p.H, p.W);

    unsigned p_off[4];
#pragma unroll
    for (int j = 0; j < 4; ++j) {
        const int tv = (wave + 4 * j) * 16 + (lane >> 2);
        const int td = tv / (TH * TW), th = (tv / TW) % TH, tw = tv % TW;
        p_off[j] = (unsigned)((((long long)td * p.H + th) * p.W + tw) * p.lddy * 2 + (lane & 3) * 16);
    }
    unsigned short st[3];
    auto load_tile = [&](const TileCo& tc, int buf) {
        unsigned char* base = smem + buf * BUF_BYTES;
        const long long pvox = (((long long)tc.n * p.D + tc.d0) * p.H + tc.h0) * p.W + tc.w0;
        const unsigned char* pb = dyg + pvox * p.lddy * 2;
        const bool full = tc.d0 + TD <= p.D && tc.h0 + TH <= p.H && tc.w0 + TW <= p.W;
        const unsigned char* zsrc = (const unsigned char*)&g_stem_zero_chunk;
        const bool ch_ok = mblk * 32 + (lane & 3) * 8 < p.M;
#pragma unroll
        for (int j = 0; j < 4; ++j) {
            const unsigned char* src = pb + p_off[j];
            if (!ch_ok) src = zsrc;
            if (!full) {
                const int tv = (wave + 4 * j) * 16 + (lane >> 2);
                const int td = tv / (TH * TW), th = (tv / TW) % TH, tw = tv % TW;
                if (!(tc.d0 + td < p.D && tc.h0 + th < p.H && tc.w0 + tw < p.W)) src = zsrc;
            }
            glds16(src, base + (wave + 4 * j) * 1024);
        }
#pragma unroll
        for (int it = 0; it < 3; ++it) {
            const int hv = tid + it * W_THREADS;
            const int hd = hv / (PH * PW), rem = hv - hd * (PH * PW), hh = rem / PW, hw = rem - hh * PW;
            const int d = tc.d0 - 1 + hd, h = tc.h0 - 1 + hh, w = tc.w0 - 1 + hw;
            const bool inb = hv < HV && (unsigned)d < (unsigned)p.D && (unsigned)h < (unsigned)p.H && (unsigned)w < (unsigned)p.W;
            st[it] = inb ? xg[((((long long)tc.n * p.D + d) * p.H + h) * p.W + w) * p.ldx] : (unsigned short)0;
        }
    };
    auto commit_x = [&](int buf) {
        unsigned short* xs = (unsigned short*)(smem + buf * BUF_BYTES + P_BYTES);
#pragma unroll
        for (int it = 0; it < 3; ++it) {
            const int hv = tid + it * W_THREADS;
            if (hv < HV) {
                const int hd = hv / (PH * PW), rem = hv - hd * (PH * PW), hh = rem / PW, hw = rem - hh * PW;
#pragma unroll
                for (int c = 0; c < 3; ++c) {
                    const int slot = hw - c;
                    if (slot >= 0 && slot < TW) xs[c * XS_ELEMS + (hd * PH + hh) * XP + slot] = st[it];
                }
            }
        }
    };

    const int G = lane >> 4, qr = (lane >> 2) & 3, pc = lane & 3;
    unsigned a_rd[2];
#pragma unroll
    for (int i = 0; i < 2; ++i) a_rd[i] = (8 * (G >> 1) + 4 * i + qr) * 64 + ((G & 1) << 5) + pc * 8;
    const int tap = lane & 31;
    const bool tap_ok = tap < 27;
    const int tkd = tap / 9, tkh = (tap / 3) % 3, tkw = tap % 3;
    const unsigned b_rd = tap_ok ? (unsigned)(P_BYTES + (tkw * XS_ELEMS + (tkd * PH + tkh) * XP + 8 * (lane >> 5)) * 2) : 0u;

    f32x16_t acc;
#pragma unroll
    for (int e = 0; e < 16; ++e) acc[e] = 0.f;

    if (sc.n_my > 0) {
        load_tile(sc.tile(0), 0);
        commit_x(0);
    }
    asm volatile("s_waitcnt vmcnt(0)" ::: "memory");
    __syncthreads();
    for (int k = 0; k < sc.n_my; ++k) {
        const int buf = k & 1;
        if (k + 1 < sc.n_my) load_tile(sc.tile(k + 1), buf ^ 1);
        lds_u8* bb = smem3 + buf * BUF_BYTES;
#pragma unroll
        for (int i4 = 0; i4 < 4; ++i4) {
            const int row = wave * 4 + i4;
            const int td = row >> 2, th = row & 3;
            const bf16x4_t lo = lds_tr(bb + a_rd[0] + row * 1024), hi = lds_tr(bb + a_rd[1] + row * 1024);
            const bf16x8_t af = {lo[0], lo[1], lo[2], lo[3], hi[0], hi[1], hi[2], hi[3]};
            u32x4_t bfr = *(const u32x4_t*)(smem + buf * BUF_BYTES + b_rd + ((td * PH + th) * XP) * 2);
            if (!tap_ok) bfr = u32x4_t{0u, 0u, 0u, 0u};
            acc = __builtin_amdgcn_mfma_f32_32x32x16_bf16(af, __builtin_bit_cast(bf16x8_t, bfr), acc, 0, 0, 0);
        }
        if (k + 1 < sc.n_my) commit_x(buf ^ 1);
        asm volatile("s_waitcnt vmcnt(0)" ::: "memory");
        __syncthreads();
    }
    float* xch = (float*)smem;
    const int col = lane & 31, rb = 4 * (lane >> 5);
#pragma unroll
    for (int e = 0; e < 16; ++e) xch[(wave * 32 + (e & 3) + 8 * (e >> 2) + rb) * 32 + col] = acc[e];
    __syncthreads();
    float* slab = p.slabs + ((long long)blockIdx.y * gridDim.x + blockIdx.x) * 1024;
    for (int i = tid; i < 1024; i += W_THREADS) slab[i] = xch[i] + xch[1024 + i] + xch[2048 + i] + xch[3072 + i];
}

}

bool msseg_stem_eligible(int dtype, int Cin, int Cout, int k, int s, int pd, long long ldx, long long ldy, const void* y) {
    static const bool off = getenv("MSSEG_NO_STEM") != nullptr;
    return !off && dtype == MSSEG_BF16 && Cin == 1 && ((k == 3 && pd == 1) || (k == 1 && pd == 0)) && s == 1 &&
           (Cout % 32 == 0 || Cout % 48 == 0) && Cout <= 256 &&
           ldx >= 1 && (ldy % 4) == 0 && (((uintptr_t)y) & 7) == 0;
}

int msseg_stem_fwd_launch(const StemParams& p, hipStream_t stream) {
    const int cbw = (p.M % 32 == 0) ? 32 : 48;
    const int ncb = p.M / cbw;
    const int tiles = p.N * ceil_div(p.D, TD) * ceil_div(p.H, TH) * ceil_div(p.W, TW);
    int gx = msseg_num_cus() * 2 / ncb;
    gx &= ~7;
    if (gx < 8) gx = 8;
    if (gx > tiles) gx = tiles;
    if (p.nstats != nullptr && p.stats != nullptr) MSSEG_FAIL(MSSEG_EINVAL, "stem_fwd: the normalised form emits no statistics");
    if (p.y == nullptr && p.stats == nullptr) MSSEG_FAIL(MSSEG_EINVAL, "stem_fwd: nothing to produce");
    if (cbw == 32) {
        if (p.nstats) hipLaunchKernelGGL((stem_fwd_kernel<0, 2, 1>), dim3(gx, ncb), dim3(F_THREADS), 0, stream, p);
        else if (p.stats) hipLaunchKernelGGL((stem_fwd_kernel<1, 2>), dim3(gx, ncb), dim3(F_THREADS), 0, stream, p);
        else hipLaunchKernelGGL((stem_fwd_kernel<0, 2>), dim3(gx, ncb), dim3(F_THREADS), 0, stream, p);
    } else {
        if (p.nstats) hipLaunchKernelGGL((stem_fwd_kernel<0, 3, 1>), dim3(gx, ncb), dim3(F_THREADS), 0, stream, p);
        else if (p.stats) hipLaunchKernelGGL((stem_fwd_kernel<1, 3>), dim3(gx, ncb), dim3(F_THREADS), 0, stream, p);
        else hipLaunchKernelGGL((stem_fwd_kernel<0, 3>), dim3(gx, ncb), dim3(F_THREADS), 0, stream, p);
    }
    MSSEG_CHECK_LAUNCH("stem_fwd");
    if (p.stats) {
        K3FinParams f{};
        f.ws = p.stats_ws; f.R = gx; f.N = p.N; f.coutb = cbw; f.M = p.M; f.stats = p.stats;
        return msseg_k3_stats_finalize(f, ncb, stream);
    }
    return MSSEG_OK;
}

int msseg_stem_wgrad_grid(const StemWgParams& p) {
    const int tiles = p.N * ceil_div(p.D, TD) * ceil_div(p.H, TH) * ceil_div(p.W, TW);
    int gx = msseg_num_cus() * 2 / ceil_div(p.M, 32);
    gx &= ~7;
    if (gx < 8) gx = 8;
    if (gx > tiles) gx = tiles;
    return gx;
}

int msseg_stem_wgrad_launch(const StemWgParams& p, int gx, hipStream_t stream) {
    const int lds = 2 * (P_BYTES + 3 * XS_ELEMS * 2 + 64);
    static msseg_lds_attr_once attr;
    if (!attr.ensure((const void*)stem_wgrad_kernel, lds)) MSSEG_FAIL(MSSEG_ELAUNCH, "stem_wgrad: cannot set dynamic LDS size %d", lds);
    hipLaunchKernelGGL(stem_wgrad_kernel, dim3(gx, ceil_div(p.M, 32)), dim3(W_THREADS), lds, stream, p);
    MSSEG_CHECK_LAUNCH("stem_wgrad");
    return MSSEG_OK;
}
```

### medicalsemseg_amd/hip.py

```python
from __future__ import annotations

import ctypes as C
import os
from typing import Optional

import torch

_HERE = os.path.dirname(os.path.abspath(__file__))
LIB_PATH = os.environ.get("MSSEG_LIB") or os.path.join(_HERE, "libmsseg_hip.so")

F32, BF16 = 0, 1
_DT = {torch.float32: F32, torch.bfloat16: BF16}
_LAB = {torch.float32: 0, torch.bfloat16: 1, torch.uint8: 2, torch.int64: 3}

_lib = None

_vp, _ll, _i, _f, _sz = C.c_void_p, C.c_longlong, C.c_int, C.c_float, C.c_size_t

SIGNATURES = {
    "msseg_abi_version": ([], _i),
    "msseg_last_error": ([], C.c_char_p),
    "msseg_num_cus": ([], _i),
    "msseg_packed_weight_bytes": ([_i, _i, _i, _i, _i], _sz),
    "msseg_pack_weights": ([_vp, _vp, _i, _i, _i, _i, _i, _i, _ll, _ll, _ll, _ll, _ll, _i, _i, _vp], _i),
    "msseg_pack_weights_batch": ([_vp, _i, _ll, _ll, _i, _vp], _i),
    "msseg_cout_block": ([_i], _i),
    "msseg_conv3d_k3_cout_block": ([_i, _i, _i, _i, _i], _i),
    "msseg_conv3d_k3_variant": ([_i, _i, _i, _i, _i], _i),
    "msseg_conv3d_k3_kernel": ([_i, _i, _i, _i, _i, _i, _i], _i),
    "msseg_conv3d_k3_fwd": ([_vp, _ll, _vp, _vp, _vp, _ll, _i, _i, _i, _i, _i, _i, _vp, _vp, _sz, _i, _vp], _i),
    "msseg_conv3d_k3_fwd_accumulate": ([_vp, _ll, _vp, _vp, _ll, _i, _i, _i, _i, _i, _i, _vp, _vp, _sz, _i, _vp], _i),
    "msseg_dwconv3d_k3_fwd": ([_vp, _ll, _vp, _vp, _vp, _ll, _i, _i, _i, _i, _i, _i, _i, _vp], _i),
    "msseg_dwconv3d_k3_wgrad": ([_vp, _ll, _vp, _ll, _vp, _vp, _i, _i, _i, _i, _i, _i, _i, _vp, _sz, _i, _vp], _i),
    "msseg_interp_trilinear_fwd": ([_vp, _ll, _vp, _ll, _i, _i, _i, _i, _i, _i, _i, _i, _i, _vp], _i),
    "msseg_interp_trilinear_bwd_workspace_bytes": ([_i, _i, _i, _i, _i, _i, _i, _i], _sz),
    "msseg_interp_trilinear_bwd": ([_vp, _ll, _vp, _ll, _i, _i, _i, _i, _i, _i, _i, _i, _vp, _sz, _i, _vp], _i),
    "msseg_kv_attention_fwd": ([_vp, _vp, _vp, _vp, _i, _i, _i, _i, _i, _f, _i, _vp], _i),
    "msseg_kv_attention_bwd_workspace_bytes": ([_i, _i, _i, _i, _i], _sz),
    "msseg_kv_attention_bwd": ([_vp, _vp, _vp, _vp, _vp, _vp, _vp, _i, _i, _i, _i, _i, _f, _vp, _sz, _i, _vp], _i),
    "msseg_scale_channels": ([_vp, _vp, _vp, _i, _ll, _i, _i, _vp], _i),
    "msseg_reduce_scratch_bytes": ([], _sz),
    "msseg_conv3d_k3_dgrad_inbwd": ([_vp, _ll, _vp, _vp, _ll, _i, _i, _i, _i, _i, _i, _vp, _ll, _vp, _ll, _vp, _f, _f, _vp,
                                     _vp, _vp, _i, _vp, _sz, _i, _vp], _i),
    "msseg_conv3d_k1_dgrad_inbwd": ([_vp, _ll, _vp, _vp, _ll, _i, _ll, _i, _i, _vp, _ll, _vp, _ll, _vp, _f, _f, _vp,
                                     _vp, _vp, _i, _vp, _sz, _i, _vp], _i),
    "msseg_deconv_k2s2_bwd_data_inbwd": ([_vp, _ll, _vp, _vp, _ll, _i, _i, _i, _i, _i, _i, _vp, _ll, _vp, _ll, _vp, _f, _f,
                                          _vp, _vp, _vp, _i, _vp, _sz, _i, _vp], _i),
    "msseg_deconv_k2s2_bwd_fused": ([_vp, _ll, _vp, _vp, _ll, _i, _i, _i, _i, _i, _i, _vp, _ll, _vp, _ll, _vp, _f, _f,
                                     _vp, _vp, _vp, _i, _vp, _i, _vp, _sz, _i, _vp], _i),
    "msseg_conv3d_k3s2_fwd": ([_vp, _ll, _vp, _vp, _vp, _ll, _i, _i, _i, _i, _i, _i, _i, _vp], _i),
    "msseg_zero_stuff2": ([_vp, _ll, _vp, _ll, _i, _i, _i, _i, _i, _i, _i, _i, _i, _vp], _i),
    "msseg_window_attention_fwd": ([_vp, _vp, _vp, _vp, _vp, _i, _i, _i, _i, _i, _i, _i, _i, _i, _vp], _i),
    "msseg_window_attention_bwd": ([_vp, _vp, _vp, _vp, _vp, _vp, _vp, _vp, _i, _i, _i, _i, _i, _i, _i, _i, _i, _vp], _i),
    "msseg_window_attention_bwd_ws": ([_vp, _vp, _vp, _vp, _vp, _vp, _vp, _vp, _i, _i, _i, _i, _i, _i, _i, _i, _i, _vp,
                                       _sz, _vp], _i),
    "msseg_window_attention_fwd2": ([_vp, _vp, _vp, _vp, _vp, _i, _i, _i, _i, _i, _i, _i, _i, _i, _i, _vp], _i),
    "msseg_window_attention_bwd2": ([_vp, _vp, _vp, _vp, _vp, _vp, _vp, _vp, _i, _i, _i, _i, _i, _i, _i, _i, _i, _i, _vp,
                                     _sz, _vp], _i),
    "msseg_window_attention_bwd_workspace_bytes": ([_i, _i, _i, _i, _i, _i, _i, _i, _i], _sz),
    "msseg_window_attention_fwd3": ([_vp, _vp, _vp, _vp, _vp, _i, _i, _i, _i, _i, _i, _i, _i, _i, _ll, _i, _vp], _i),
    "msseg_window_attention_bwd3": ([_vp, _vp, _vp, _vp, _vp, _vp, _vp, _vp, _i, _i, _i, _i, _i, _i, _i, _i, _i, _ll, _i,
                                     _vp, _sz, _vp], _i),
    "msseg_window_attention_bwd3_workspace_bytes": ([_i, _i, _i, _i, _i, _i, _i, _i, _i, _ll, _i], _sz),
    "msseg_rel_bias_affine_fold": ([_vp, _vp, _vp, _vp, _vp, _vp, _i, _i, _i, _vp], _i),
    "msseg_rel_bias_affine_grad_workspace_bytes": ([_i, _i], _sz),
    "msseg_rel_bias_affine_grad": ([_vp, _vp, _vp, _vp, _vp, _vp, _vp, _vp, _i, _i, _i, _i, _vp, _sz, _vp], _i),
    "msseg_layernorm_fwd": ([_vp, _ll, _vp, _vp, _vp, _ll, _vp, _vp, _ll, _i, _f, _i, _vp], _i),
    "msseg_layernorm_bwd": ([_vp, _ll, _vp, _vp, _vp, _vp, _ll, _vp, _ll, _ll, _i, _i, _vp], _i),
    "msseg_layernorm_bwd_add": ([_vp, _ll, _vp, _vp, _vp, _vp, _ll, _vp, _ll, _vp, _ll, _ll, _i, _i, _vp], _i),
    "msseg_layernorm_param_grad": ([_vp, _ll, _vp, _vp, _vp, _ll, _vp, _vp, _i, _ll, _i, _vp, _sz, _i, _vp], _i),
    "msseg_gelu_fwd": ([_vp, _vp, _ll, _i, _vp], _i),
    "msseg_gelu_bwd": ([_vp, _vp, _vp, _ll, _i, _vp], _i),
    "msseg_linear_wgrad_ok": ([_ll, _i, _i, _i], _i),
    "msseg_linear_wgrad": ([_vp, _ll, _vp, _ll, _vp, _vp, _ll, _i, _i, _i, _i, _vp, _sz, _i, _vp], _i),
    "msseg_linear_gelu_ok": ([_ll, _i, _i, _i], _i),
    "msseg_linear_gelu_fwd": ([_vp, _ll, _vp, _vp, _vp, _ll, _vp, _ll, _ll, _i, _i, _i, _vp], _i),
    "msseg_linear_gelu_bwd": ([_vp, _ll, _vp, _vp, _ll, _vp, _ll, _ll, _i, _i, _i, _vp], _i),
    "msseg_linear_add_ok": ([_ll, _i, _i, _i], _i),
    "msseg_linear_add_fwd": ([_vp, _ll, _vp, _vp, _vp, _ll, _vp, _ll, _ll, _i, _i, _i, _vp], _i),
    "msseg_conv3d_stem_fwd": ([_vp, _ll, _vp, _vp, _vp, _ll, _i, _i, _i, _i, _i, _vp, _vp, _sz, _i, _vp], _i),
    "msseg_conv3d_stem_k1_fwd": ([_vp, _ll, _vp, _vp, _vp, _ll, _i, _i, _i, _i, _i, _vp, _vp, _sz, _i, _vp], _i),
    "msseg_conv3d_stem_norm_fwd": ([_vp, _ll, _vp, _vp, _vp, _vp, _vp, _f, _f, _vp, _ll, _i, _i, _i, _i, _i, _i, _vp], _i),
    "msseg_conv3d_k1_head_dgrad_inbwd": ([_vp, _ll, _vp, _vp, _ll, _i, _ll, _i, _i, _vp, _ll, _vp, _vp, _vp, _f, _f, _vp, _vp,
                                          _vp, _i, _vp, _sz, _i, _vp], _i),
    "msseg_conv3d_k1_head_norm_fwd": ([_vp, _ll, _vp, _vp, _vp, _f, _f, _vp, _vp, _vp, _ll, _i, _ll, _i, _i, _i, _vp], _i),
    "msseg_conv3d_k1_head_bwd_fused": ([_vp, _ll, _vp, _vp, _ll, _i, _ll, _i, _i, _vp, _ll, _vp, _vp, _vp, _f, _f, _vp, _vp,
                                        _vp, _i, _vp, _i, _vp, _sz, _i, _vp], _i),
    "msseg_conv3d_k1_head_fwd": ([_vp, _ll, _vp, _vp, _vp, _ll, _ll, _i, _i, _i, _vp], _i),
    "msseg_conv3d_k1_fwd": ([_vp, _ll, _vp, _vp, _vp, _ll, _ll, _i, _i, _i, _vp], _i),
    "msseg_conv3d_gather_fwd": ([_vp, _ll, _vp, _vp, _vp, _ll, _i, _i, _i, _i, _i, _i, _i, _i, _i, _i, _vp], _i),
    "msseg_deconv_k2s2_fwd": ([_vp, _ll, _vp, _vp, _vp, _ll, _i, _i, _i, _i, _i, _i, _i, _vp], _i),
    "msseg_deconv_k2s2_bwd_data": ([_vp, _ll, _vp, _vp, _ll, _i, _i, _i, _i, _i, _i, _i, _vp], _i),
    "msseg_wgrad_workspace_bytes": ([_i, _i, _i], _sz),
    "msseg_conv3d_k3_wgrad_kernel": ([_i, _i, _i, _i, _i, _i, _i], _i),
    "msseg_conv3d_k3_wgrad": ([_vp, _ll, _vp, _ll, _vp, _i, _i, _i, _i, _i, _i, _i, _vp, _sz, _i, _vp], _i),
    "msseg_conv3d_k1_wgrad": ([_vp, _ll, _vp, _ll, _vp, _ll, _i, _i, _i, _vp, _sz, _i, _vp], _i),
    "msseg_conv3d_gather_wgrad": ([_vp, _ll, _vp, _ll, _vp, _i, _i, _i, _i, _i, _i, _i, _i, _i, _i, _vp, _sz, _i, _vp], _i),
    "msseg_deconv_k2s2_wgrad": ([_vp, _ll, _vp, _ll, _vp, _i, _i, _i, _i, _i, _i, _i, _vp, _sz, _i, _vp], _i),
    "msseg_channel_stats": ([_vp, _ll, _vp, _i, _ll, _i, _vp, _sz, _i, _vp], _i),
    "msseg_instnorm_act_fwd": ([_vp, _ll, _vp, _vp, _vp, _vp, _ll, _vp, _ll, _i, _ll, _i, _f, _f, _i, _vp], _i),
    "msseg_instnorm_act_poolbwd_reduce": ([_vp, _ll, _vp, _vp, _vp, _vp, _ll, _vp, _ll, _vp, _ll, _vp, _vp, _vp, _i,
                                           _i, _i, _i, _i, _i, _f, _f, _vp, _sz, _i, _vp], _i),
    "msseg_instnorm_act_pool_fwd": ([_vp, _ll, _vp, _vp, _vp, _vp, _ll, _vp, _ll, _i, _i, _i, _i, _i, _f, _f, _i, _vp], _i),
    "msseg_instnorm_act_bwd_reduce": ([_vp, _ll, _vp, _vp, _vp, _vp, _ll, _vp, _ll, _vp, _vp, _vp, _i, _i, _ll, _i, _f, _f, _vp, _sz, _i, _vp], _i),
    "msseg_instnorm_act_bwd_apply": ([_vp, _ll, _vp, _vp, _vp, _vp, _ll, _vp, _ll, _vp, _vp, _ll, _vp, _ll, _i, _ll, _i, _f, _f, _i, _vp], _i),
    "msseg_maxpool2_fwd": ([_vp, _ll, _vp, _ll, _i, _i, _i, _i, _i, _i, _vp], _i),
    "msseg_maxpool2_bwd": ([_vp, _ll, _vp, _ll, _vp, _ll, _i, _i, _i, _i, _i, _i, _i, _vp], _i),
    "msseg_ncdhw_to_ndhwc": ([_vp, _i, _vp, _ll, _i, _i, _i, _ll, _vp], _i),
    "msseg_ndhwc_to_ncdhw": ([_vp, _ll, _i, _vp, _i, _i, _i, _ll, _vp], _i),
    "msseg_channel_sum": ([_vp, _ll, _vp, _ll, _i, _i, _vp, _sz, _i, _vp], _i),
    "msseg_axpy_rows": ([_vp, _vp, _vp, _vp, _i, _ll, _i, _vp], _i),
    "msseg_add": ([_vp, _ll, _vp, _ll, _vp, _ll, _ll, _i, _i, _vp], _i),
    "msseg_dice_ce_partials": ([_vp, _ll, _i, _vp, _i, _vp, _vp, _i, _ll, _i, _vp], _i),
    "msseg_dice_ce_fwd": ([_vp, _ll, _i, _vp, _i, _vp, _vp, _vp, _i, _ll, _i, _f, _f, _vp, _sz, _vp], _i),
    "msseg_dice_ce_finalize": ([_vp, _vp, _i, _ll, _i, _f, _f, _vp], _i),
    "msseg_dice_ce_bwd": ([_vp, _ll, _i, _vp, _i, _vp, _vp, _vp, _ll, _i, _ll, _i, _f, _f, _vp], _i),
    "msseg_adamw_step": ([_vp, _vp, _vp, _vp, _vp, _ll, _f, _f, _f, _f, _f, _i, _vp, _vp, _vp], _i),
    "msseg_sumsq": ([_vp, _ll, _vp, _vp, _i, _vp], _i),
    "msseg_sw_blend": ([_vp, _ll, _i, _vp, _vp, _vp, _i, _i, _i, _i, _i, _i, _i, _i, _i, _i, _vp], _i),
    "msseg_sw_normalize": ([_vp, _vp, _i, _ll, _vp], _i),
    "msseg_sw_gather": ([_vp, _vp, _i, _i, _i, _i, _i, _i, _i, _i, _i, _i, _i, _f, _vp], _i),
    "msseg_box_copy": ([_vp, _ll, _i, _i, _i, _vp, _ll, _i, _i, _i, _i, _i, _i, _vp], _i),
    "msseg_merge_gather_fwd": ([_vp, _ll, _i, _i, _i, _vp, _ll, _i, _i, C.c_uint, _i, _vp], _i),
    "msseg_merge_gather_bwd": ([_vp, _ll, _vp, _ll, _i, _i, _i, _i, _i, C.c_uint, _i, _vp], _i),
    "msseg_argmax_u8": ([_vp, _i, _ll, _vp, _vp], _i),
    "msseg_resample_nearest_u8": ([_vp, _i, _i, _i, _vp, _i, _i, _i, _vp], _i),
    "msseg_majority_vote_u8": ([_vp, _i, _ll, _i, _vp, _vp], _i),
    "msseg_aug_crop_batch": ([_vp, _vp, _i, _i, _i, _i, _vp, _i, _vp, _i, _vp, _i, _vp], _i),
    "msseg_sw_gather_batch": ([_vp, _ll, _vp, _ll, _i, _vp, _i, _i, _i, _i, _i, _i, _i, _i, _f, _vp], _i),
    "msseg_sw_blend_batch": ([_vp, _ll, _i, _vp, _vp, _ll, _vp, _ll, _vp, _i, _i, _i, _i, _i, _i, _i, _i, _vp], _i),
    "msseg_deconv_k2s2_bwd_partials_ok": ([_i, _i, _i], _i),
    "msseg_deconv_k2s2_bwd_partials": ([_vp, _ll, _vp, _vp, _sz, _i, _i, _i, _i, _i, _i, _i, _vp], _i),
    "msseg_conv3d_k3_small_ok": ([_i, _i, _i, _i, _i, _i, _i], _i),
    "msseg_conv3d_k3_small_workspace_bytes": ([_i, _i, _i, _i, _i, _i], _sz),
    "msseg_conv3d_k3_small_stage_groups": ([_i, _i, _i, _i, _i, _i], _i),
    "msseg_conv3d_k3_small_partials": ([_vp, _ll, _vp, _vp, _sz, _i, _i, _i, _i, _i, _i, _vp], _i),
    "msseg_conv3d_k3_small_fwd_finish": ([_vp, _i, _vp, _vp, _vp, _f, _f, _vp, _ll, _vp, _ll, _vp, _ll, _vp, _i, _i, _i, _i,
                                          _i, _vp], _i),
    "msseg_conv3d_k3_small_fwd_finish_res": ([_vp, _i, _vp, _vp, _vp, _f, _f, _vp, _ll, _vp, _ll, _vp, _ll, _vp, _ll, _vp, _i, _i, _i, _i,
                                              _i, _vp], _i),
    "msseg_conv3d_k3_small_bwd_finish": ([_vp, _i, _vp, _ll, _vp, _ll, _vp, _vp, _vp, _f, _f, _vp, _vp, _i, _i, _i, _i, _i,
                                          _i, _vp], _i),
    "msseg_avgpool3d_k3": ([_vp, _ll, _vp, _ll, _i, _i, _i, _i, _i, _i, _vp], _i),
    "msseg_hd_edges": ([_vp, _vp, _i, _i, _i, _i, _vp, _vp, _vp, _vp], _i),
    "msseg_hd_directed_workspace_bytes": ([_i, _i, _i], _sz),
    "msseg_hd_directed_hist": ([_vp, _vp, _i, _i, _i, _i, _vp, _vp, _sz, _vp, _i, _vp], _i),
    "msseg_ktimer_enable": ([_i], _i),
    "msseg_ktimer_reset": ([], _i),
    "msseg_ktimer_count": ([], _i),
    "msseg_ktimer_get": ([_i, C.c_char_p, _i, C.POINTER(C.c_float)], _i),
}


def load_library(path: Optional[str] = None):
    global _lib
    if _lib is not None and path is None:
        return _lib
    p = path or LIB_PATH
    if not os.path.exists(p):
        raise RuntimeError(
            f"{p} not found: build it with `python -c 'import __graft_entry__ as g; g.build()'` "
            f"(or `make -C medicalsemseg_amd/csrc`).  There is no CPU fallback.")
    lib = C.CDLL(p)
    for name, (args, res) in SIGNATURES.items():
        fn = getattr(lib, name)
        fn.argtypes = args
        fn.restype = res
    if lib.msseg_abi_version() != 1:
        raise RuntimeError("libmsseg_hip.so ABI version mismatch")
    _lib = lib
    return lib


def lib():
    real = _lib if _lib is not None else load_library()
    if TIMER.enabled:
        return _TimedLib(real)
    return real


class MssegError(RuntimeError):
    pass


def _ck(rc: int, what: str):
    if rc != 0:
        raise MssegError(f"{what} failed ({rc}): {lib().msseg_last_error().decode()}")


def _stream() -> int:
    return torch.cuda.current_stream().cuda_stream


def _need_gpu(*ts):
    for t in ts:
        if t is not None and not t.is_cuda:
            raise RuntimeError("medicalsemseg_amd kernels run on the GPU only (got a CPU tensor); "
                               "there is no CPU fallback")


def dt(t: torch.Tensor) -> int:
    try:
        return _DT[t.dtype]
    except KeyError:
        raise TypeError(f"unsupported dtype {t.dtype} (float32 / bfloat16 only)")


def ld(t: torch.Tensor) -> int:
    C = t.shape[-1]
    if C > 1 and t.stride(-1) != 1:
        raise ValueError("channels-last tensor must have unit channel stride")
    l = None
    exp = None
    for d in range(t.dim() - 2, -1, -1):
        if t.shape[d] > 1:
            if l is None:
                l = t.stride(d)
                exp = l * t.shape[d]
            else:
                if t.stride(d) != exp:
                    raise ValueError(f"tensor is not a dense channels-last volume: shape {tuple(t.shape)} "
                                     f"stride {t.stride()}")
                exp *= t.shape[d]
    if l is None:
        l = C
    if l < C:
        raise ValueError("voxel stride smaller than the channel count")
    return l


def _nbytes(*ts) -> float:
    return float(sum(t.numel() * t.element_size() for t in ts if t is not None))


def _p(t: Optional[torch.Tensor]):
    return None if t is None else t.data_ptr()


def cout_block(M: int) -> int:
    return lib().msseg_cout_block(M)


def conv_k3_cout_block(N, D, H, W, cout) -> int:
    return lib().msseg_conv3d_k3_cout_block(N, D, H, W, cout)


class PackJob(C.Structure):
    _fields_ = [("src", C.c_void_p), ("dst", C.c_void_p),
# ... 325 lines not shown

def conv3d_k1_head_norm(yraw, stats, gamma, beta, slope, eps, w, bias, y, cin, cout):
    _need_gpu(yraw, stats, w, y)
    N = yraw.shape[0]
    S = yraw.numel() // yraw.shape[-1] // N
    _ck(lib().msseg_conv3d_k1_head_norm_fwd(_p(yraw), ld(yraw), _p(stats), _p(gamma), _p(beta), slope, eps, _p(w), _p(bias),
                                            _p(y), ld(y), N, S, cin, cout, dt(yraw), _stream()), "conv3d_k1_head_norm_fwd")
    return y


def conv3d_k1_head_bwd_fused(dy, w, da, cin, cout, yraw, fwd_stats, gamma, beta, slope, eps, dw, dw_accumulate,
                             dgamma=None, dbeta=None, accumulate=False):
    _need_gpu(dy, w, da, yraw, fwd_stats, dw)
    N = dy.shape[0]
    S = dy.numel() // dy.shape[-1] // N
    red = torch.empty(N, cin, 2, dtype=torch.float32, device=dy.device)
    sc = scratch(dy.device)
    _ck(lib().msseg_conv3d_k1_head_bwd_fused(_p(dy), ld(dy), _p(w), _p(da), ld(da), N, S, cin, cout, _p(yraw), ld(yraw),
                                             _p(fwd_stats), _p(gamma), _p(beta), slope, eps, _p(red), _p(dgamma),
                                             _p(dbeta), int(accumulate), _p(dw), int(dw_accumulate), _p(sc), sc.numel(),
                                             dt(dy), _stream()), "conv3d_k1_head_bwd_fused")
    return red


def conv3d_k1(x, wp, bias, y, cin, cout):
    _need_gpu(x, wp, y)
    nv = x.numel() // x.shape[-1]
    _ck(lib().msseg_conv3d_k1_fwd(_p(x), ld(x), _p(wp), _p(bias), _p(y), ld(y), nv, cin, cout, dt(x), _stream()),
        "conv3d_k1_fwd")
    return y


def conv3d_k1_dgrad_inbwd(dy, wp, da, cin, cout, yraw, act, fwd_stats, slope, eps, dgamma=None, dbeta=None,
                          accumulate=False):
    _need_gpu(dy, wp, da, yraw, act, fwd_stats)
    N = da.shape[0]
    S = da.numel() // (N * da.shape[-1])
    red = torch.empty(N, cout, 2, dtype=torch.float32, device=dy.device)
    sc = scratch(dy.device)
    _ck(lib().msseg_conv3d_k1_dgrad_inbwd(_p(dy), ld(dy), _p(wp), _p(da), ld(da), N, S, cin, cout, _p(yraw), ld(yraw),
                                          _p(act), ld(act), _p(fwd_stats), slope, eps, _p(red), _p(dgamma), _p(dbeta),
                                          int(accumulate), _p(sc), sc.numel(), dt(dy), _stream()), "conv3d_k1_dgrad_inbwd")
    return red


def deconv_k2s2_bwd_data_inbwd(dy, wp, dx, cin, cout, yraw, act, fwd_stats, slope, eps, dgamma=None, dbeta=None,
                               accumulate=False):
    _need_gpu(dy, wp, dx, yraw, act, fwd_stats)
    N, D, H, W = dx.shape[:4]
    red = torch.empty(N, cin, 2, dtype=torch.float32, device=dy.device)
    sc = scratch(dy.device)
    _ck(lib().msseg_deconv_k2s2_bwd_data_inbwd(_p(dy), ld(dy), _p(wp), _p(dx), ld(dx), N, D, H, W, cin, cout, _p(yraw),
                                               ld(yraw), _p(act), ld(act), _p(fwd_stats), slope, eps, _p(red),
                                               _p(dgamma), _p(dbeta), int(accumulate), _p(sc), sc.numel(), dt(dy),
                                               _stream()), "deconv_k2s2_bwd_data_inbwd")
    return red


def deconv_k2s2_bwd_fused(dy, wp, dx, cin, cout, next_norm=None, dbias=None, dbias_accumulate=False, dgamma=None, dbeta=None,
                          accumulate=False):
    _need_gpu(dy, wp, dx)
    N, D, H, W = dx.shape[:4]
    red = None
    yraw = act = stats = None
    slope = eps = 0.0
    if next_norm is not None:
        yraw, act, stats, slope, eps = next_norm
        red = torch.empty(N, cin, 2, dtype=torch.float32, device=dy.device)
    sc = scratch(dy.device)
    _ck(lib().msseg_deconv_k2s2_bwd_fused(_p(dy), ld(dy), _p(wp), _p(dx), ld(dx), N, D, H, W, cin, cout, _p(yraw),
                                          ld(yraw) if yraw is not None else 0, _p(act), ld(act) if act is not None else 0,
                                          _p(stats), slope, eps, _p(red), _p(dgamma), _p(dbeta), int(accumulate), _p(dbias),
                                          int(dbias_accumulate), _p(sc), sc.numel(), dt(dy), _stream()),
        "deconv_k2s2_bwd_fused")
    return red


def conv3d_gather(x, wp, bias, y, cin, cout, k, s, p):
    _need_gpu(x, wp, y)
    N, D, H, W = x.shape[:4]
    _ck(lib().msseg_conv3d_gather_fwd(_p(x), ld(x), _p(wp), _p(bias), _p(y), ld(y), N, D, H, W, cin, cout, k, s, p,
                                      dt(x), _stream()), "conv3d_gather_fwd")
    return y


def conv3d_stem_norm(x, wp, bias, stats, gamma, beta, eps, slope, y, cout):
    _need_gpu(x, wp, y, stats)
    N, D, H, W = x.shape[:4]
    _ck(lib().msseg_conv3d_stem_norm_fwd(_p(x), ld(x), _p(wp), _p(bias), _p(stats), _p(gamma), _p(beta), eps, slope, _p(y), ld(y),
                                         N, D, H, W, cout, dt(x), _stream()), "conv3d_stem_norm_fwd")
    return y


def conv3d_stem(x, wp, bias, y, cout, stats=None, k=3):
    _need_gpu(x, wp)
    N, D, H, W = x.shape[:4]
    sc = scratch(x.device) if stats is not None else None
    fn = lib().msseg_conv3d_stem_fwd if k == 3 else lib().msseg_conv3d_stem_k1_fwd
    _ck(fn(_p(x), ld(x), _p(wp), _p(bias), _p(y), ld(y) if y is not None else 0, N, D, H, W, cout, _p(stats), _p(sc),
                                    sc.numel() if sc is not None else 0, dt(x), _stream()), "conv3d_stem_fwd")
    return y


def deconv_k2s2(x, wp, bias, y, cin, cout):
    _need_gpu(x, wp, y)
    N, D, H, W = x.shape[:4]
    _ck(lib().msseg_deconv_k2s2_fwd(_p(x), ld(x), _p(wp), _p(bias), _p(y), ld(y), N, D, H, W, cin, cout, dt(x),
                                    _stream()), "deconv_k2s2_fwd")
    return y


def deconv_k2s2_bwd_data(dy, wp, dx, cin, cout):
    _need_gpu(dy, wp, dx)
    N, D, H, W = dx.shape[:4]
    _ck(lib().msseg_deconv_k2s2_bwd_data(_p(dy), ld(dy), _p(wp), _p(dx), ld(dx), N, D, H, W, cin, cout, dt(dy),
                                         _stream()), "deconv_k2s2_bwd_data")
    return dx


_ws_cache = {}
_ws_retired = []


def workspace(nbytes: int, device) -> torch.Tensor:
    key = (device.index if device.index is not None else torch.cuda.current_device())
    buf = _ws_cache.get(key)
    if buf is None or buf.numel() < nbytes:
        if buf is not None:
            _ws_retired.append(buf)
        buf = torch.empty(max(nbytes, 64 << 20), dtype=torch.uint8, device=device)
        _ws_cache[key] = buf
    return buf


def _wg_ws(M, T, K, device):
    return workspace(lib().msseg_wgrad_workspace_bytes(M, T, K), device)


def conv3d_k3_wgrad(x, dy, dw, cin, cout, accumulate=False):
    _need_gpu(x, dy, dw)
    N, D, H, W = x.shape[:4]
    ws = _wg_ws(cout, 27, cin, x.device)
    nv = N * D * H * W

    def go():
        _ck(lib().msseg_conv3d_k3_wgrad(_p(x), ld(x), _p(dy), ld(dy), _p(dw), N, D, H, W, cin, cout, int(accumulate),
                                        _p(ws), ws.numel(), dt(x), _stream()), "conv3d_k3_wgrad")
    key = "conv3d_k3_wgrad"
    if TIMER.enabled:
        key += "/v%d" % lib().msseg_conv3d_k3_wgrad_kernel(N, D, H, W, cin, cout, dt(x))
    TIMER.launch(key, 2.0 * nv * 27 * cin * cout, nv * (cin + cout) * x.element_size() + 27 * cin * cout * 4, go)


def conv3d_k1_wgrad(x, dy, dw, cin, cout, accumulate=False):
    _need_gpu(x, dy, dw)
    nv = x.numel() // x.shape[-1]
    ws = _wg_ws(cout, 1, cin, x.device)
    _ck(lib().msseg_conv3d_k1_wgrad(_p(x), ld(x), _p(dy), ld(dy), _p(dw), nv, cin, cout, int(accumulate), _p(ws),
                                    ws.numel(), dt(x), _stream()), "conv3d_k1_wgrad")


def linear_wgrad_ok(x, cin, cout) -> bool:
    return bool(x.is_cuda and x.dtype == torch.bfloat16 and
                lib().msseg_linear_wgrad_ok(x.numel() // x.shape[-1], cin, cout, BF16))


def linear_wgrad(x, dy, dw, dbias, cin, cout, accumulate_w=False, accumulate_b=False):
    _need_gpu(x, dy, dw)
    nv = x.numel() // x.shape[-1]
    ws = _wg_ws(cout, 1, cin, x.device)
    esz = x.element_size()
    TIMER.launch("linear_wgrad", 2.0 * nv * cin * cout, nv * (cin + cout) * esz + cin * cout * 4,
                 lambda: _ck(lib().msseg_linear_wgrad(_p(x), ld(x), _p(dy), ld(dy), _p(dw), _p(dbias), nv, cin, cout,
                                                      int(accumulate_w), int(accumulate_b), _p(ws), ws.numel(), dt(x),
                                                      _stream()), "linear_wgrad"))


def conv3d_gather_wgrad(x, dy, dw, cin, cout, k, s, p, accumulate=False):
    _need_gpu(x, dy, dw)
    N, D, H, W = x.shape[:4]
    ws = _wg_ws(cout, 1, cin * k ** 3, x.device)
    _ck(lib().msseg_conv3d_gather_wgrad(_p(x), ld(x), _p(dy), ld(dy), _p(dw), N, D, H, W, cin, cout, k, s, p,
                                        int(accumulate), _p(ws), ws.numel(), dt(x), _stream()), "conv3d_gather_wgrad")


def deconv_k2s2_wgrad(x, dy, dw, cin, cout, accumulate=False):
    _need_gpu(x, dy, dw)
    N, D, H, W = x.shape[:4]
    ws = _wg_ws(cin, 1, 8 * cout, x.device)
    _ck(lib().msseg_deconv_k2s2_wgrad(_p(x), ld(x), _p(dy), ld(dy), _p(dw), N, D, H, W, cin, cout, int(accumulate),
                                      _p(ws), ws.numel(), dt(x), _stream()), "deconv_k2s2_wgrad")


def _nsc(x):
    N, C = x.shape[0], x.shape[-1]
    return N, x.numel() // (N * C), C


def dwconv3d_k3(x, w_taps, bias, y, flip=False):
    if w_taps.dtype != x.dtype:
        raise ValueError("dwconv3d_k3: the weight table must have the activation dtype")
    _need_gpu(x, w_taps, y)
    N, D, H, W, C = x.shape
    _ck(lib().msseg_dwconv3d_k3_fwd(_p(x), ld(x), _p(w_taps), _p(bias), _p(y), ld(y), N, D, H, W, C, int(flip), dt(x),
                                    _stream()), "dwconv3d_k3_fwd")
    return y


def avgpool3d_k3(x, y):
    _need_gpu(x, y)
    N, D, H, W, Cc = x.shape
    _ck(lib().msseg_avgpool3d_k3(_p(x), ld(x), _p(y), ld(y), N, D, H, W, Cc, dt(x), _stream()), "avgpool3d_k3")
    return y


def dwconv3d_k3_wgrad(x, dy, dw, dbias, acc_w=False, acc_b=False):
    _need_gpu(x, dy)
    N, D, H, W, C = x.shape
    sc = scratch(x.device)
    _ck(lib().msseg_dwconv3d_k3_wgrad(_p(x), ld(x), _p(dy), ld(dy), _p(dw), _p(dbias), int(acc_w), int(acc_b), N, D, H, W, C,
                                      _p(sc), sc.numel(), dt(x), _stream()), "dwconv3d_k3_wgrad")


def interp_trilinear(x, y):
    _need_gpu(x, y)
    N, ID, IH, IW, C = x.shape
    _ck(lib().msseg_interp_trilinear_fwd(_p(x), ld(x), _p(y), ld(y), N, ID, IH, IW, y.shape[1], y.shape[2], y.shape[3], C,
                                         dt(x), _stream()), "interp_trilinear_fwd")
    return y


def interp_trilinear_bwd(dy, dx):
    _need_gpu(dy, dx)
    N, ID, IH, IW, C = dx.shape
    OD, OH, OW = dy.shape[1:4]
    nb = lib().msseg_interp_trilinear_bwd_workspace_bytes(N, ID, IH, IW, OD, OH, OW, C)
    ws = torch.empty(nb, dtype=torch.uint8, device=dx.device)
    _ck(lib().msseg_interp_trilinear_bwd(_p(dy), ld(dy), _p(dx), ld(dx), N, ID, IH, IW, OD, OH, OW, C, _p(ws), nb, dt(dx),
                                         _stream()), "interp_trilinear_bwd")
    return dx


def kv_attention_fwd(q, kv, heads, scale):
    _need_gpu(q, kv)
    B, N, C = q.shape
    M = kv.shape[1]
    o = torch.empty_like(q)
    lse = torch.empty(B, heads, N, dtype=torch.float32, device=q.device)
    _ck(lib().msseg_kv_attention_fwd(_p(q), _p(kv), _p(o), _p(lse), B, N, M, heads, C // heads, scale, dt(q), _stream()),
        "kv_attention_fwd")
    return o, lse


def kv_attention_bwd(q, kv, o, lse, dout, heads, scale):
    _need_gpu(q, kv, o, lse, dout)
    B, N, C = q.shape
    M = kv.shape[1]
    dq, dkv = torch.empty_like(q), torch.empty_like(kv)
    nb = lib().msseg_kv_attention_bwd_workspace_bytes(B, N, M, heads, C // heads)
    ws = torch.empty(nb, dtype=torch.uint8, device=q.device)
    _ck(lib().msseg_kv_attention_bwd(_p(q), _p(kv), _p(o), _p(lse), _p(dout), _p(dq), _p(dkv), B, N, M, heads, C // heads,
                                     scale, _p(ws), nb, dt(q), _stream()), "kv_attention_bwd")
    return dq, dkv


def scale_channels(x, scale, y):
    _need_gpu(x, scale, y)
    N, C = x.shape[0], x.shape[-1]
    _ck(lib().msseg_scale_channels(_p(x), _p(scale), _p(y), N, x.numel() // (N * C), C, dt(x), _stream()), "scale_channels")
    return y


def channel_stats(x, stats=None):
    _need_gpu(x)
    N, S, Cc = _nsc(x)
    if stats is None:
        stats = torch.empty(N, Cc, 2, dtype=torch.float32, device=x.device)
    sc = scratch(x.device)
    _ck(lib().msseg_channel_stats(_p(x), ld(x), _p(stats), N, S, Cc, _p(sc), sc.numel(), dt(x), _stream()),
        "channel_stats")
    return stats


def instnorm_act_fwd(x, stats, gamma, beta, y, slope, eps=1e-5, residual=None):
    _need_gpu(x, stats, y)
    N, S, Cc = _nsc(x)
    TIMER.launch("instnorm_act_fwd", 0.0, _nbytes(x, y, residual), lambda: _ck(lib().msseg_instnorm_act_fwd(_p(x), ld(x), _p(stats), _p(gamma), _p(beta), _p(residual),
                                     ld(residual) if residual is not None else 0, _p(y), ld(y), N, S, Cc, eps, slope,
                                     dt(x), _stream()), "instnorm_act_fwd"))
    return y


def instnorm_pool_ok(x, y, pooled) -> bool:
    epc = 16 // x.element_size()
    return (x.dim() == 5 and all(int(d) % 2 == 0 for d in x.shape[1:4]) and x.shape[-1] % epc == 0
            and all(ld(t) % epc == 0 and t.data_ptr() % 16 == 0 for t in (x, y, pooled)))


def instnorm_act_pool_fwd(x, stats, gamma, beta, y, pooled, slope, eps=1e-5):
    _need_gpu(x, stats, y, pooled)
    N, D, H, W, Cc = x.shape
    TIMER.launch("instnorm_act_pool_fwd", 0.0, _nbytes(x, y, pooled), lambda: _ck(lib().msseg_instnorm_act_pool_fwd(_p(x), ld(x), _p(stats), _p(gamma), _p(beta), _p(y), ld(y), _p(pooled), ld(pooled),
                                          N, D, H, W, Cc, eps, slope, dt(x), _stream()), "instnorm_act_pool_fwd"))
    return y, pooled


# ... 493 lines not shown
```

### medicalsemseg_amd/layers.py

```python
from __future__ import annotations

import os

from typing import Optional

import torch

from . import hip

weights_epoch = 0


def bump_weights_epoch():
    global weights_epoch
    weights_epoch += 1


class _PackRegistry:

    def __init__(self):
        self.groups = {}

    def add(self, device, dtype, src, dst, job):
        g = self.groups.setdefault((device, dtype), {"jobs": [], "table": None, "keep": []})
# ... 112 lines not shown
        with torch.cuda.stream(st):
            fn()

    def run(self, fn, *tensors):
        if self.active is None or self.mode == self.INLINE:
            return fn()
        self.keep.extend(tensors)
        if self.mode == self.DEFER:
            self.deferred.append(fn)
        else:
            self._issue(fn)

    def flush(self):
        if self.active is not None:
            for fn in self.deferred:
                self._issue(fn)
        self.deferred = []

    def join(self):
        self.flush()
        st, self.active = self.active, None
        self.mode = self.INLINE
        if st is not None:
            torch.cuda.current_stream().wait_stream(st)
        self.keep.clear()


WGRAD_SIDE = _WgradSide()


INFERENCE_FORWARD = False


class _Applied:

    def __repr__(self):
        return "APPLIED"


APPLIED = _Applied()


def _grad_buf(p: torch.nn.Parameter):
    if p.grad is None:
        p.grad = torch.empty_like(p, memory_format=torch.contiguous_format)
        return p.grad, False
    owner = getattr(p, "_msseg_gowner", None)
    if owner is not None and not getattr(p, "_msseg_kgrad", False):
        p._msseg_kgrad = True
        p._msseg_gepoch = owner._gepoch
        return p.grad, True
    if owner is not None and getattr(p, "_msseg_gepoch", -1) != owner._gepoch:
        p._msseg_gepoch = owner._gepoch
        return p.grad, False
    return p.grad, True


def _empty_like_vol(x, C, dtype=None):
    return torch.empty(x.shape[:-1] + (C,), dtype=dtype or x.dtype, device=x.device)


def _norm_grad_bufs(nrm):
    if nrm.gamma is not None and nrm.gamma.requires_grad:
        dg, acc = _grad_buf(nrm.gamma)
        db, _ = _grad_buf(nrm.beta)
        return dg, db, acc
    return None, None, False


class Conv3:

    def __init__(self, weight: torch.nn.Parameter, bias: Optional[torch.nn.Parameter]):
        self.w, self.b = weight, bias
        self.cout, self.cin = weight.shape[0], weight.shape[1]
        self.cache = PackedCache()

    def _gather(self, dtype):
        return self.cin % (8 if dtype == torch.bfloat16 else 4) != 0

    def fwd(self, x, out=None, want_stats=False):
        dtype = x.dtype
        if want_stats and out is None and self.halves_ok(tuple(x.shape[:4]), dtype):
            return self.fwd_halves(x)
        y = out if out is not None else _empty_like_vol(x, self.cout)
        stats = None
        if self._gather(dtype):
            wp = self.cache.get(self.w, dtype, "g", lambda: hip.pack_conv_gather(self.w.detach(), dtype))
            if (self.cin == 1 and dtype == torch.bfloat16 and (self.cout % 32 == 0 or self.cout % 48 == 0) and self.cout <= 256
                    and not os.environ.get("MSSEG_NO_STEM")):
                if want_stats and x.shape[0] <= 8:
                    stats = torch.empty(x.shape[0], self.cout, 2, dtype=torch.float32, device=x.device)
                hip.conv3d_stem(x, wp, self.b, y, self.cout, stats)
            else:
                hip.conv3d_gather(x, wp, self.b, y, self.cin, self.cout, 3, 1, 1)
        else:
            vol = tuple(x.shape[:4])
            wp = self.cache.get(self.w, dtype, ("f", vol), lambda: hip.pack_conv_k3(self.w.detach(), dtype, vol=vol))
            if want_stats and x.shape[0] <= 8:
                stats = torch.empty(x.shape[0], self.cout, 2, dtype=torch.float32, device=x.device)
            hip.conv3d_k3(x, wp, self.b, y, self.cin, self.cout, stats)
        if want_stats:
            return y, (stats if stats is not None else hip.channel_stats(y))
        return y

    def halves_ok(self, vol, dtype) -> int:
        if dtype != torch.bfloat16 or os.environ.get("MSSEG_NO_SPLIT_CAT"):
            return 0
        if self.cin == 96 and hip.lib().msseg_conv3d_k3_kernel(*vol, 48, self.cout, hip.BF16) == 4:
            return 48
        if (INFERENCE_FORWARD and self.cin in (64, 128) and self.cout % 32 == 0 and not os.environ.get("MSSEG_NO_KSPLIT_INFER")
                and hip.lib().msseg_conv3d_k3_kernel(*vol, 32, self.cout, hip.BF16) == 3):
            return 32
        return 0

    def fwd_halves(self, x):
        dtype, vol = x.dtype, tuple(x.shape[:4])
        h = self.halves_ok(vol, dtype)
        y = _empty_like_vol(x, self.cout)
        stats = torch.empty(x.shape[0], self.cout, 2, dtype=torch.float32, device=x.device)
        for i in range(self.cin // h):
            wi = self.w.detach()[:, i * h:(i + 1) * h]
            pi = self.cache.get(wi, dtype, ("fp", i, h, vol), lambda wi=wi: hip.pack_conv_k3(wi, dtype, vol=vol))
            xi = x[..., i * h:(i + 1) * h]
            if i == 0:
                hip.conv3d_k3(xi, pi, self.b, y, h, self.cout)
            else:
                hip.conv3d_k3_accumulate(xi, pi, y, h, self.cout, stats)
        return y, stats

    def split_ok(self, vol, dtype, ca, cb_) -> bool:
        if (os.environ.get("MSSEG_NO_SPLIT_CAT") or dtype != torch.bfloat16 or ca + cb_ != self.cin or ca != 32 or cb_ != 32
                or self.cout % 32 or vol[0] > 8):
            return False
        return hip.lib().msseg_conv3d_k3_kernel(*vol, 32, self.cout, hip.BF16) == 3

    def fwd_split(self, xa, xb):
        dtype = xa.dtype
        vol = tuple(xa.shape[:4])
        wa, wb = self.w.detach()[:, :32], self.w.detach()[:, 32:]
        pa = self.cache.get(wa, dtype, ("fa", vol), lambda: hip.pack_conv_k3(wa, dtype, vol=vol))
        pb = self.cache.get(wb, dtype, ("fb", vol), lambda: hip.pack_conv_k3(wb, dtype, vol=vol))
        y = _empty_like_vol(xa, self.cout)
        hip.conv3d_k3(xa, pa, self.b, y, 32, self.cout)
        stats = torch.empty(xa.shape[0], self.cout, 2, dtype=torch.float32, device=xa.device)
        hip.conv3d_k3_accumulate(xb, pb, y, 32, self.cout, stats)
        return y, stats

    def dgrad_accumulate_ok(self, dy) -> bool:
        if dy.dtype != torch.bfloat16 or self.cout not in (32, 48) or dy.shape[0] > 4 or os.environ.get("MSSEG_NO_DGRAD_ACCUM"):
            return False
        vol = tuple(dy.shape[:4])
        return hip.lib().msseg_conv3d_k3_kernel(*vol, self.cout, self.cin, hip.BF16) == (4 if self.cout == 48 else 3)

    def bwd(self, x, dy, need_dx=True, dx_out=None, bias_grad_is_zero=False, next_norm=None, accumulate_dx=False):
        dtype = x.dtype
        if self.w.requires_grad:
            g, acc = _grad_buf(self.w)
            if self._gather(dtype):
                WGRAD_SIDE.run(lambda: hip.conv3d_gather_wgrad(x, dy, g, self.cin, self.cout, 3, 1, 1, acc), x, dy)
            else:
                WGRAD_SIDE.run(lambda: hip.conv3d_k3_wgrad(x, dy, g, self.cin, self.cout, acc), x, dy)
        if self.b is not None and self.b.requires_grad:
            g, acc = _grad_buf(self.b)
            if bias_grad_is_zero:
                if not acc and not getattr(self.b, "_msseg_grad_is_zero", False):
                    g.zero_()
                    self.b._msseg_grad_is_zero = getattr(self.b, "_msseg_gowner", None) is not None
            else:
                hip.channel_sum(dy, g, acc)
        if not need_dx:
            return None
        if self._gather(dtype):
            raise NotImplementedError("input gradient of a few-channel stem conv is never needed on this path")
        vol = tuple(dy.shape[:4])
        if accumulate_dx:
            assert dx_out is not None and next_norm is None and self.dgrad_accumulate_ok(dy)
            wp = self.cache.get(self.w, dtype, ("d", vol),
                                lambda: hip.pack_conv_k3(self.w.detach(), dtype, dgrad=True, vol=vol))
            unused = torch.empty(dy.shape[0], self.cin, 2, dtype=torch.float32, device=dy.device)
            hip.conv3d_k3_accumulate(dy, wp, dx_out, self.cout, self.cin, unused)
            return dx_out
        if hip.conv3d_k3_small_ok(dy, self.cout, self.cin):
            wp = self.cache.get(self.w, dtype, "ds", lambda: hip.pack_conv_k3(self.w.detach(), dtype, dgrad=True, cb=32))
            part, ng = hip.conv3d_k3_small_partials(dy, wp, self.cout, self.cin)
            dx = dx_out if dx_out is not None else _empty_like_vol(dy, self.cin)
            if next_norm is not None:
                nrm, yraw, stats, act = next_norm
                dg, db, acc = _norm_grad_bufs(nrm)
                hip.conv3d_k3_small_bwd_finish(part, ng, dx, (yraw, stats, nrm.gamma, nrm.beta, nrm.eps, nrm.slope),
                                               dg, db, acc)
                return dx, APPLIED
            return hip.conv3d_k3_small_bwd_finish(part, ng, dx)
        wp = self.cache.get(self.w, dtype, ("d", vol),
                            lambda: hip.pack_conv_k3(self.w.detach(), dtype, dgrad=True, vol=vol))
        dx = dx_out if dx_out is not None else _empty_like_vol(dy, self.cin)
        if next_norm is not None:
            nrm, yraw, stats, act = next_norm
            if dy.shape[0] <= 8 and self.cin % 4 == 0:
                dg = db = None
                acc = False
                if nrm.gamma is not None and nrm.gamma.requires_grad:
                    dg, acc = _grad_buf(nrm.gamma)
                    db, _ = _grad_buf(nrm.beta)
                red = hip.conv3d_k3_dgrad_inbwd(dy, wp, dx, self.cout, self.cin, yraw, act, stats, nrm.slope, nrm.eps,
                                                dg, db, acc)
                return dx, red
            hip.conv3d_k3(dy, wp, None, dx, self.cout, self.cin)
            return dx, None
        hip.conv3d_k3(dy, wp, None, dx, self.cout, self.cin)
        return dx


class Conv1:

    def __init__(self, weight, bias):
        self.w, self.b = weight, bias
        self.cout, self.cin = weight.shape[0], weight.shape[1]
        self.cache = PackedCache()

    def _gather(self, dtype):
        return self.cin % (8 if dtype == torch.bfloat16 else 4) != 0

    def fwd(self, x, out=None, want_stats=False):
        dtype = x.dtype
        y = out if out is not None else _empty_like_vol(x, self.cout)
        if self._gather(dtype):
            wp = self.cache.get(self.w, dtype, "g", lambda: hip.pack_conv_gather(self.w.detach(), dtype))
            if (want_stats and self.cin == 1 and dtype == torch.bfloat16 and x.dim() == 5 and x.shape[0] <= 8 and hip.ld(y) == self.cout
                    and (self.cout % 32 == 0 or self.cout % 48 == 0) and self.cout <= 256 and not os.environ.get("MSSEG_NO_STEM")):
                stats = torch.empty(x.shape[0], self.cout, 2, dtype=torch.float32, device=x.device)
                hip.conv3d_stem(x, wp, self.b, y, self.cout, stats, k=1)
                return y, stats
            hip.conv3d_gather(x, wp, self.b, y, self.cin, self.cout, 1, 1, 0)
        elif (self.cout <= 4 and self.cin <= 64 and x.shape[-1] == self.cin and self.w.is_contiguous()
              and not os.environ.get("MSSEG_NO_HEAD_KERNEL")):
            hip.conv3d_k1_head(x, self.w.detach(), self.b, y, self.cin, self.cout)
        else:
            wp = self.cache.get(self.w, dtype, "f",
                                lambda: hip.pack_conv_k1(self.w.detach().reshape(self.cout, self.cin), dtype))
            hip.conv3d_k1(x, wp, self.b, y, self.cin, self.cout)
        if want_stats:
            return y, hip.channel_stats(y)
        return y

    def head_norm_ok(self, yraw) -> bool:
        epc = 16 // yraw.element_size()
        return (self.cout <= 4 and self.cin <= 64 and self.cin % epc == 0 and yraw.shape[-1] == self.cin
                and hip.ld(yraw) % epc == 0 and yraw.data_ptr() % 16 == 0 and self.w.is_contiguous()
                and not os.environ.get("MSSEG_NO_HEAD_KERNEL") and not os.environ.get("MSSEG_NO_HEAD_FUSE"))

    def fwd_norm(self, yraw, stats, nrm, out):
        return hip.conv3d_k1_head_norm(yraw, stats, nrm.gamma, nrm.beta, nrm.slope, nrm.eps, self.w.detach(), self.b, out,
                                       self.cin, self.cout)

    def bwd_norm(self, dy, dy_channels, nrm, yraw, stats):
        dyk = dy[..., :dy_channels]
        dx = torch.empty(yraw.shape, dtype=yraw.dtype, device=yraw.device)
        dg, db, acc = _norm_grad_bufs(nrm)
        if self.b is not None and self.b.requires_grad:
            g, bacc = _grad_buf(self.b)
            hip.channel_sum(dy[..., :self.cout], g, bacc)
        if self.w.requires_grad:
            gw, wacc = _grad_buf(self.w)
            red = hip.conv3d_k1_head_bwd_fused(dyk, self.w.detach(), dx, self.cin, self.cout, yraw, stats, nrm.gamma, nrm.beta,
                                               nrm.slope, nrm.eps, gw, wacc, dg, db, acc)
        else:
            red = hip.conv3d_k1_head_dgrad_inbwd(dyk, self.w.detach(), dx, self.cin, self.cout, yraw, stats, nrm.gamma,
                                                 nrm.beta, nrm.slope, nrm.eps, dg, db, acc)
        return dx, red

    def bwd(self, x, dy, need_dx=True, dy_channels=None, next_norm=None):
        dtype = x.dtype
        fused_bias = False
        if self.w.requires_grad:
            g, acc = _grad_buf(self.w)
            if self._gather(dtype):
                WGRAD_SIDE.run(lambda: hip.conv3d_gather_wgrad(x, dy[..., :self.cout], g, self.cin, self.cout, 1, 1, 0, acc), x, dy)
            elif hip.linear_wgrad_ok(x, self.cin, self.cout):
                gb, bacc = _grad_buf(self.b) if (self.b is not None and self.b.requires_grad) else (None, False)
                WGRAD_SIDE.run(lambda: hip.linear_wgrad(x, dy[..., :self.cout], g.view(self.cout, self.cin), gb, self.cin,
                                                        self.cout, acc, bacc), x, dy)
                fused_bias = True
            else:
                WGRAD_SIDE.run(lambda: hip.conv3d_k1_wgrad(x, dy[..., :self.cout], g, self.cin, self.cout, acc), x, dy)
        if self.b is not None and self.b.requires_grad and not fused_bias:
            g, acc = _grad_buf(self.b)
            hip.channel_sum(dy[..., :self.cout], g, acc)
        if not need_dx:
            return None
        if self._gather(dtype):
            raise NotImplementedError("input gradient of a few-channel 1x1 conv is never needed on this path")
        dx = _empty_like_vol(dy, self.cin)
        kpad = dy_channels if dy_channels is not None else self.cout
        dyk = dy if dy_channels is None else dy[..., :kpad]
        epc = 16 // dy.element_size()
        if (next_norm is not None and self.cout <= 4 and kpad >= 4 and self.cin <= 64 and self.cin % epc == 0 and hip.ld(dyk) % epc == 0
                and dyk.data_ptr() % 16 == 0 and self.w.is_contiguous() and not os.environ.get("MSSEG_NO_HEAD_KERNEL")):
            nrm, yraw, stats, act = next_norm
            dg, db, acc = _norm_grad_bufs(nrm)
            red = hip.conv3d_k1_head_dgrad_inbwd(dyk, self.w.detach(), dx, self.cin, self.cout, yraw, stats, nrm.gamma,
                                                 nrm.beta, nrm.slope, nrm.eps, dg, db, acc)
            return dx, red
        wp = self.cache.get(self.w, dtype, "d",
                            lambda: hip.pack_conv_k1(self.w.detach().reshape(self.cout, self.cin), dtype, dgrad=True))
        if next_norm is not None:
            nrm, yraw, stats, act = next_norm
            if dy.shape[0] <= 8 and self.cin % 4 == 0:
                dg, db, acc = _norm_grad_bufs(nrm)
                red = hip.conv3d_k1_dgrad_inbwd(dyk, wp, dx, kpad, self.cin, yraw, act, stats, nrm.slope, nrm.eps, dg, db, acc)
                return dx, red
            hip.conv3d_k1(dyk, wp, None, dx, kpad, self.cin)
            return dx, None
        hip.conv3d_k1(dyk, wp, None, dx, kpad, self.cin)
        return dx


class Deconv2:

    def __init__(self, weight, bias):
        self.w, self.b = weight, bias
        self.cin, self.cout = weight.shape[0], weight.shape[1]
        self.cache = PackedCache()

    def fwd(self, x, out=None):
        dtype = x.dtype
        N, D, H, W, _ = x.shape
        y = out if out is not None else torch.empty(N, 2 * D, 2 * H, 2 * W, self.cout, dtype=dtype, device=x.device)
        wp = self.cache.get(self.w, dtype, "f", lambda: hip.pack_deconv(self.w.detach(), dtype))
        hip.deconv_k2s2(x, wp, self.b, y, self.cin, self.cout)
        return y

    def bwd(self, x, dy, need_dx=True, next_norm=None):
        dtype = x.dtype
        if self.w.requires_grad:
            g, acc = _grad_buf(self.w)
            WGRAD_SIDE.run(lambda: hip.deconv_k2s2_wgrad(x, dy, g, self.cin, self.cout, acc), x, dy)
        want_db = self.b is not None and self.b.requires_grad
        if not need_dx:
            if want_db:
                g, acc = _grad_buf(self.b)
                hip.channel_sum(dy, g, acc)
            return None
        wp = self.cache.get(self.w, dtype, "d", lambda: hip.pack_deconv(self.w.detach(), dtype, bwd=True))
        dx = torch.empty_like(x, memory_format=torch.contiguous_format)
        db, dbacc = _grad_buf(self.b) if want_db else (None, False)
        if next_norm is not None and hip.deconv_k2s2_small_unit_ok(tuple(x.shape), self.cin, self.cout, dtype):
            nrm, yraw, stats, act = next_norm
            part = hip.deconv_k2s2_bwd_partials(dy, wp, self.cin, self.cout)
            dg, dbt, nacc = _norm_grad_bufs(nrm)
            hip.conv3d_k3_small_bwd_finish(part, 1, dx, (yraw, stats, nrm.gamma, nrm.beta, nrm.eps, nrm.slope), dg, dbt, nacc)
            if want_db:
                hip.channel_sum(dy, db, dbacc)
            return dx, APPLIED
        nn_ = None
        dg = dbt = None
        nacc = False
        if next_norm is not None:
            nrm, yraw, stats, act = next_norm
            if dy.shape[0] <= 8 and self.cin % 4 == 0:
                dg, dbt, nacc = _norm_grad_bufs(nrm)
                nn_ = (yraw, act, stats, nrm.slope, nrm.eps)
        red = hip.deconv_k2s2_bwd_fused(dy, wp, dx, self.cin, self.cout, nn_, db, dbacc, dg, dbt, nacc)
        return (dx, red) if next_norm is not None else dx


class InstNormAct:

    def __init__(self, gamma: Optional[torch.nn.Parameter], beta: Optional[torch.nn.Parameter], slope: float,
                 eps: float = 1e-5):
        self.gamma, self.beta, self.slope, self.eps = gamma, beta, float(slope), float(eps)

    def fwd(self, y_raw, out=None, residual=None, stats=None, pooled=None):
        if stats is None:
            stats = hip.channel_stats(y_raw)
        a = out if out is not None else torch.empty_like(y_raw, memory_format=torch.contiguous_format)
        if pooled is not None:
            if residual is None and hip.instnorm_pool_ok(y_raw, a, pooled) and not os.environ.get("MSSEG_NO_NORM_POOL"):
                hip.instnorm_act_pool_fwd(y_raw, stats, self.gamma, self.beta, a, pooled, self.slope, self.eps)
                return a, stats
            hip.instnorm_act_fwd(y_raw, stats, self.gamma, self.beta, a, self.slope, self.eps, residual)
            hip.maxpool2_fwd(a, pooled)
            return a, stats
        hip.instnorm_act_fwd(y_raw, stats, self.gamma, self.beta, a, self.slope, self.eps, residual)
        return a, stats

    def pool_bwd_reduce(self, y_raw, stats, skip_grad, pooled_grad):
        if (os.environ.get("MSSEG_NO_NORM_POOL") or os.environ.get("MSSEG_NO_POOL_BWD_FUSE")
                or not hip.instnorm_pool_ok(y_raw, skip_grad, pooled_grad)):
            return None
        da = torch.empty(y_raw.shape, dtype=y_raw.dtype, device=y_raw.device)
        dg, db, acc = _norm_grad_bufs(self)
        red = hip.instnorm_act_poolbwd_reduce(y_raw, stats, self.gamma, self.beta, skip_grad, pooled_grad, da, self.slope,
                                              self.eps, dg, db, acc)
        return da, red

    def bwd(self, y_raw, stats, a, da, want_dres=False, red=None):
        if red is APPLIED:
            if want_dres:
                raise RuntimeError("a residual unit cannot take an already-applied gradient")
            return da
        dy = torch.empty(y_raw.shape, dtype=y_raw.dtype, device=y_raw.device)
        dres = torch.empty(y_raw.shape, dtype=y_raw.dtype, device=y_raw.device) if want_dres else None
        a_in = a if want_dres else None
        if red is not None:
            hip.instnorm_act_bwd_apply(y_raw, stats, self.gamma, a_in, da, red, dy, self.slope, self.eps, dres, self.beta)
            return (dy, dres) if want_dres else dy
        dg = db = None
        acc = False
        if self.gamma is not None and self.gamma.requires_grad:
            dg, acc = _grad_buf(self.gamma)
            db, acc2 = _grad_buf(self.beta)
            assert acc == acc2
        hip.instnorm_act_bwd(y_raw, stats, self.gamma, a_in, da, dy, self.slope, self.eps, dres, dg, db, acc, self.beta)
        return (dy, dres) if want_dres else dy


class ConvNormAct:

    def __init__(self, conv: Conv3, norm: InstNormAct):
        self.conv, self.norm = conv, norm

    def fwd(self, x, out=None, pooled=None):
        cv, nm = self.conv, self.norm
        if (INFERENCE_FORWARD and pooled is None and cv.cin == 1 and x.dtype == torch.bfloat16 and x.shape[0] <= 8
                and (cv.cout % 32 == 0 or cv.cout % 48 == 0) and cv.cout <= 256 and not os.environ.get("MSSEG_NO_STEM")
                and not os.environ.get("MSSEG_NO_STEM_TWICE")):
            wp = cv.cache.get(cv.w, x.dtype, "g", lambda: hip.pack_conv_gather(cv.w.detach(), x.dtype))
            stats = torch.empty(x.shape[0], cv.cout, 2, dtype=torch.float32, device=x.device)
            hip.conv3d_stem(x, wp, cv.b, None, cv.cout, stats)
            a = out if out is not None else _empty_like_vol(x, cv.cout)
            hip.conv3d_stem_norm(x, wp, cv.b, stats, nm.gamma, nm.beta, nm.eps, nm.slope, a, cv.cout)
            return a, (x, None, stats, a)
        if (not cv._gather(x.dtype) and hip.conv3d_k3_small_ok(x, cv.cin, cv.cout)
                and (pooled is None or hip.instnorm_pool_ok(x, x, pooled))):
            wp = cv.cache.get(cv.w, x.dtype, "fs", lambda: hip.pack_conv_k3(cv.w.detach(), x.dtype, cb=32))
            part, ng = hip.conv3d_k3_small_partials(x, wp, cv.cin, cv.cout)
            y = _empty_like_vol(x, cv.cout)
            a = out if out is not None else _empty_like_vol(x, cv.cout)
            stats = torch.empty(x.shape[0], cv.cout, 2, dtype=torch.float32, device=x.device)
            hip.conv3d_k3_small_fwd_finish(part, ng, cv.b, nm.gamma, nm.beta, nm.eps, nm.slope, y, a, pooled, stats)
            return a, (x, y, stats, a)
        y, stats = self.conv.fwd(x, want_stats=True)
        a, stats = self.norm.fwd(y, out, stats=stats, pooled=pooled)
        return a, (x, y, stats, a)

    def bwd(self, saved, da, need_dx=True, red=None, next_saved=None, next_cna=None):
        x, y, stats, a = saved
        dy = self.norm.bwd(y, stats, a, da, red=red)
        if next_cna is not None and need_dx:
            nx, ny, nstats, na = next_saved
            return self.conv.bwd(x, dy, True, bias_grad_is_zero=True, next_norm=(next_cna.norm, ny, nstats, na))
        return self.conv.bwd(x, dy, need_dx, bias_grad_is_zero=True)


def maxpool_fwd(x):
    N, D, H, W, C = x.shape
    y = torch.empty(N, D // 2, H // 2, W // 2, C, dtype=x.dtype, device=x.device)
    return hip.maxpool2_fwd(x, y)


class ResBlock:

    def __init__(self, conv1_w, conv2_w, conv3_w=None, slope=0.01):
        self.c1, self.c2 = Conv3(conv1_w, None), Conv3(conv2_w, None)
        self.c3 = Conv1(conv3_w, None) if conv3_w is not None else None
        self.n1, self.n2 = InstNormAct(None, None, slope), InstNormAct(None, None, slope)
        self.n3 = InstNormAct(None, None, 1.0) if conv3_w is not None else None

    @staticmethod
    def _small_unit(conv, nrm, x, residual=None, out=None):
        wp = conv.cache.get(conv.w, x.dtype, "fs", lambda: hip.pack_conv_k3(conv.w.detach(), x.dtype, cb=32))
        part, ng = hip.conv3d_k3_small_partials(x, wp, conv.cin, conv.cout)
        y = _empty_like_vol(x, conv.cout)
        a = out if out is not None else _empty_like_vol(x, conv.cout)
        stats = torch.empty(x.shape[0], conv.cout, 2, dtype=torch.float32, device=x.device)
        hip.conv3d_k3_small_fwd_finish(part, ng, conv.b, nrm.gamma, nrm.beta, nrm.eps, nrm.slope, y, a, None, stats, residual)
        return a, y, stats

    def fwd(self, x, out=None):
        small = (not self.c1._gather(x.dtype) and hip.conv3d_k3_small_ok(x, self.c1.cin, self.c1.cout)
                 and hip.conv3d_k3_small_ok(x, self.c2.cin, self.c2.cout))
        if small:
            a1, y1, s1 = self._small_unit(self.c1, self.n1, x)
        else:
            y1, s1 = self.c1.fwd(x, want_stats=True)
            a1, s1 = self.n1.fwd(y1, stats=s1)
        if self.c3 is not None:
            y3, s3 = self.c3.fwd(x, want_stats=True)
            r, s3 = self.n3.fwd(y3, stats=s3)
        else:
            y3 = s3 = None
            r = x
        if small:
            o, y2, s2 = self._small_unit(self.c2, self.n2, a1, residual=r, out=out)
        else:
            y2, s2 = self.c2.fwd(a1, want_stats=True)
            o, s2 = self.n2.fwd(y2, out, residual=r, stats=s2)
        return o, (x, y1, s1, a1, y2, s2, y3, s3, r, o)

    def bwd(self, saved, do, need_dx=True):
        x, y1, s1, a1, y2, s2, y3, s3, r, o = saved
        dy2, dres = self.n2.bwd(y2, s2, o, do, want_dres=True)
        da1, red1 = self.c2.bwd(a1, dy2, True, next_norm=(self.n1, y1, s1, a1))
        dy1 = self.n1.bwd(y1, s1, a1, da1, red=red1)
        if need_dx and self.c1.dgrad_accumulate_ok(dy1):
            if self.c3 is not None:
                dy3 = self.n3.bwd(y3, s3, r, dres)
                dx3 = self.c3.bwd(x, dy3, True)
            else:
                dx3 = dres
            return self.c1.bwd(x, dy1, True, dx_out=dx3, accumulate_dx=True)
        dx = self.c1.bwd(x, dy1, need_dx)
        if self.c3 is not None:
            dy3 = self.n3.bwd(y3, s3, r, dres)
            dx3 = self.c3.bwd(x, dy3, need_dx)
        else:
            dx3 = dres
        if not need_dx:
            return None
        return hip.add(dx, dx3, dx)


class UpBlock:

    def __init__(self, transp_w, conv1_w, conv2_w, conv3_w, slope=0.01):
        self.up = Deconv2(transp_w, None)
        self.res = ResBlock(conv1_w, conv2_w, conv3_w, slope)
        self.cout = transp_w.shape[1]

    def alloc_cat(self, x):
        N, D, H, W, _ = x.shape
        return torch.empty(N, 2 * D, 2 * H, 2 * W, 2 * self.cout, dtype=x.dtype, device=x.device)

    def fwd(self, x, cat):
        self.up.fwd(x, cat[..., :self.cout])
        o, s = self.res.fwd(cat)
        return o, (x, s)

    def bwd(self, saved, do):
        x, s = saved
        dcat = self.res.bwd(s, do, True)
        dx = self.up.bwd(x, dcat[..., :self.cout], True)
        return dx, dcat[..., self.cout:]


def _merge_batch(t):
    N, D, H, W, C = t.shape
    return t.view(1, N * D, H, W, C)


class BatchNormAct:

    def __init__(self, bn: torch.nn.BatchNorm3d, slope: float = 0.0, group=None):
        self.bn = bn
        self.inner = InstNormAct(bn.weight, bn.bias, slope, bn.eps)
        self.group = group

    def _all_reduce(self, t):
        import torch.distributed as dist
        dist.all_reduce(t, group=None if self.group is True else self.group)

    def _synced(self):
        import torch.distributed as dist
        if self.group is None or not (dist.is_available() and dist.is_initialized()):
            return False
        return dist.get_world_size(None if self.group is True else self.group) > 1

    def fwd(self, y_raw, out=None, stats=None):
        bn = self.bn
        N, D, H, W, C = y_raw.shape
        cnt = N * D * H * W
        if bn.training or not bn.track_running_stats:
            s = stats.sum(0, keepdim=True) if stats is not None else hip.channel_stats(_merge_batch(y_raw))
            total = cnt
            if self._synced():
                pack = torch.cat([s.reshape(-1), torch.full((1,), float(cnt), device=s.device)])
                self._all_reduce(pack)
                total = float(pack[-1])
                s = (pack[:-1] * (cnt / total)).reshape(1, C, 2)
            if bn.training and bn.track_running_stats:
                with torch.no_grad():
                    bn.num_batches_tracked.add_(1)
                    mean = s[0, :, 0] / cnt
                    var = (s[0, :, 1] / cnt - mean * mean).clamp_(min=0) * (total / max(total - 1, 1))
                    if bn.momentum is None:
                        m = 1.0 / bn.num_batches_tracked.to(torch.float32)
                        bn.running_mean.add_((mean - bn.running_mean) * m)
                        bn.running_var.add_((var - bn.running_var) * m)
                    else:
                        bn.running_mean.mul_(1 - bn.momentum).add_(mean, alpha=bn.momentum)
                        bn.running_var.mul_(1 - bn.momentum).add_(var, alpha=bn.momentum)
        else:
            eps = self.inner.eps
            rstd = torch.rsqrt(bn.running_var.double() + eps)
            g = self.inner.gamma.detach().double() if self.inner.gamma is not None else torch.ones_like(rstd)
            bta = self.inner.beta.detach().double() if self.inner.beta is not None else torch.zeros_like(rstd)
            scale = g * rstd
            shift = bta - bn.running_mean.double() * scale
            s = torch.zeros(1, C, 2, dtype=torch.float32, device=y_raw.device)
            s[0, :, 1] = (1.0 - eps) * cnt
            a = out if out is not None else torch.empty(y_raw.shape, dtype=y_raw.dtype, device=y_raw.device)
            hip.instnorm_act_fwd(_merge_batch(y_raw), s, scale.float().contiguous(), shift.float().contiguous(),
                                 _merge_batch(a), self.inner.slope, eps, None)
            return a, s
        a = out if out is not None else torch.empty(y_raw.shape, dtype=y_raw.dtype, device=y_raw.device)
# ... 38 lines not shown
```

Measured before the change: 534.6 vol/s.

## Fuse instance-norm backward into conv weight-gradient kernels for stem and k3 convs

Adds variants of the k3 and stem weight-gradient kernels that take the post-activation gradient, the raw conv output and the norm statistics, then compute the norm/LeakyReLU backward in LDS before the wgrad MMA. The k3 variant can also write the resulting dy for the data-gradient path. This is meant to remove the separate norm-backward pass and its dy round trip for large-resolution layers. The stem path is on by default when the side wgrad stream is idle. The k3 path needs an environment variable, and the fusion adds LDS use and per-tile elementwise work to the wgrad kernels.

```diff
diff --git a/include/msseg.h b/include/msseg.h
--- a/include/msseg.h
+++ b/include/msseg.h
@@ -122,6 +122,16 @@
 int msseg_conv3d_k3_wgrad(const void* x, long long ldx, const void* dy, long long lddy, float* dw,
                           int N, int D, int H, int W, int Cin, int Cout, int accumulate,
                           void* workspace, size_t workspace_bytes, int dtype, msseg_stream_t stream);
+int msseg_conv3d_k3_wgrad_inbwd_kernel(int N, int D, int H, int W, int Cin, int Cout, int dtype);
+int msseg_conv3d_k3_wgrad_inbwd(const void* x, long long ldx, const void* da, const void* yraw, long long ldd,
+                                const float* stats, const float* red, const float* gamma, const float* beta, float eps,
+                                float slope, void* dy, float* dw, int N, int D, int H, int W, int Cin, int Cout,
+                                int accumulate, void* workspace, size_t workspace_bytes, int dtype, msseg_stream_t stream);
+int msseg_conv3d_stem_wgrad_inbwd_kernel(int N, int D, int H, int W, int Cout, int dtype);
+int msseg_conv3d_stem_wgrad_inbwd(const void* x, long long ldx, const void* da, const void* yraw, long long ldd,
+                                  const float* stats, const float* red, const float* gamma, const float* beta, float eps,
+                                  float slope, float* dw, int N, int D, int H, int W, int Cout, int accumulate,
+                                  void* workspace, size_t workspace_bytes, int dtype, msseg_stream_t stream);
 int msseg_conv3d_k1_wgrad(const void* x, long long ldx, const void* dy, long long lddy, float* dw,
                           long long NV, int Cin, int Cout, int accumulate,
                           void* workspace, size_t workspace_bytes, int dtype, msseg_stream_t stream);
diff --git a/medicalsemseg_amd/csrc/conv3d_k3_wgrad_pp.hip b/medicalsemseg_amd/csrc/conv3d_k3_wgrad_pp.hip
--- a/medicalsemseg_amd/csrc/conv3d_k3_wgrad_pp.hip
+++ b/medicalsemseg_amd/csrc/conv3d_k3_wgrad_pp.hip
@@ -1,4 +1,5 @@
 #include "k3pp.h"
+#include "inorm_bwd.h"
 
 #include <stdlib.h>
 
@@ -21,6 +22,9 @@
 constexpr int TAPW = 7;
 constexpr int NTHREADS = 512;
 constexpr int SLAB_FLOATS = 27 * 32 * 32;
+constexpr int COEF_FLOATS = 6 * 32;
+constexpr int INBWD_NMAX = 4;
+constexpr int INBWD_LDS = 2 * GRP_BYTES + P_BYTES + INBWD_NMAX * COEF_FLOATS * 4;
 
 __device__ u32x4_t g_wg_zero_chunk;
 __device__ unsigned long long g_k3wg_cycles[8];
@@ -32,6 +36,7 @@
 
 typedef __attribute__((address_space(3))) unsigned char lds_u8;
 typedef __attribute__((ext_vector_type(16))) float f32x16_t;
+typedef __attribute__((ext_vector_type(2))) __bf16 bf16x2_t;
 
 MSSEG_DEVFN bf16x4_t lds_tr(lds_u8* p) {
     return __builtin_amdgcn_ds_read_tr16_b64_v4bf16((__attribute__((address_space(3))) bf16x4_t*)p);
@@ -47,7 +52,7 @@
 
 constexpr int ks_row(int ks) { return ((ks / TH) * PH + ks % TH) * PWP; }
 
-template <int TIMING>
+template <int TIMING, int INBWD>
 __global__ __launch_bounds__(NTHREADS, 1) void k3wg_pp_kernel(const K3WgParams p) {
     extern __shared__ __attribute__((aligned(256))) unsigned char smem[];
     const int tid = threadIdx.x, lane = tid & 63;
@@ -59,6 +64,8 @@
     const int mblk = blockIdx.y / p.kblks, kblk = blockIdx.y % p.kblks;
     const unsigned char* pg = (const unsigned char*)p.pten + mblk * 64;
     const unsigned char* qg = (const unsigned char*)p.qten + kblk * 64;
+    const unsigned char* yrg = (const unsigned char*)p.yraw + mblk * 64;
+    unsigned char* dog = (kblk == 0 && p.dyout != nullptr) ? (unsigned char*)p.dyout + mblk * 64 : nullptr;
 
     const int tiles_w = (p.W + TW - 1) / TW, tiles_h = (p.H + TH - 1) / TH, tiles_d = (p.D + TD - 1) / TD;
     const int ntiles = p.N * tiles_d * tiles_h * tiles_w;
@@ -98,6 +105,18 @@
         const int td = tv / (TH * TW), th = (tv / TW) % TH, tw = tv % TW;
         p_off[j] = (unsigned)((((long long)td * p.H + th) * p.W + tw) * p.ldp * 2 + lchunk * 16);
     }
+    unsigned char* ldsY = smem + 2 * GRP_BYTES;
+    float* coef = (float*)(ldsY + P_BYTES);
+    if constexpr (INBWD) {
+        const long long S = (long long)p.D * p.H * p.W;
+        for (int i = tid; i < p.N * 32; i += NTHREADS) {
+            const int n = i >> 5, cl = i & 31;
+            const InBwdCoef k = inbwd_coef(p.stats, p.red, p.gamma, p.beta, n, p.M, mblk * 32 + cl, S, p.eps);
+            float* t = coef + n * COEF_FLOATS + cl;
+            t[0] = k.mean; t[32] = k.rstd; t[64] = k.sc; t[96] = k.sh; t[128] = k.k0; t[160] = k.k1;
+        }
+        __syncthreads();
+    }
     const bool p_cok = mblk * 32 + lchunk * 8 < p.M, q_cok = kblk * 32 + lchunk * 8 < p.K;
     const bool chunks_full = (mblk + 1) * 32 <= p.M && (kblk + 1) * 32 <= p.K;
     auto load_tile = [&](const TileCo& tc) {
@@ -106,6 +125,7 @@
         const long long pvox = (((long long)tc.n * p.D + tc.d0) * p.H + tc.h0) * p.W + tc.w0;
         const unsigned char* qb = qg + qvox * p.ldq * 2;
         const unsigned char* pb = pg + pvox * p.ldp * 2;
+        const unsigned char* yb = yrg + pvox * p.ldp * 2;
         const bool interior = chunks_full && dB >= 0 && dB + PD <= p.D && hB >= 0 && hB + PH <= p.H && wB >= 0 && wB + PW <= p.W;
         if (interior) {
 #pragma unroll
@@ -113,7 +133,10 @@
                 if (q_off[j] != SKIP) glds16(qb + q_off[j], ldsQ + (wq + 4 * j) * 1024);
             }
 #pragma unroll
-            for (int j = 0; j < NIP_W; ++j) glds16(pb + p_off[j], ldsP + (wq + 4 * j) * 1024);
+            for (int j = 0; j < NIP_W; ++j) {
+                glds16(pb + p_off[j], ldsP + (wq + 4 * j) * 1024);
+                if constexpr (INBWD) glds16(yb + p_off[j], ldsY + (wq + 4 * j) * 1024);
+            }
         } else {
             const unsigned char* zsrc = (const unsigned char*)&g_wg_zero_chunk;
 #pragma unroll
@@ -131,8 +154,50 @@
                 const int tv = (wq + 4 * j) * 16 + lrow;
                 const int td = tv / (TH * TW), th = (tv / TW) % TH, tw = tv % TW;
                 const bool inb = p_cok && tc.d0 + td < p.D && tc.h0 + th < p.H && tc.w0 + tw < p.W;
-                const unsigned char* src = inb ? pb + p_off[j] : zsrc;
-                glds16(src, ldsP + (wq + 4 * j) * 1024);
+                glds16(inb ? pb + p_off[j] : zsrc, ldsP + (wq + 4 * j) * 1024);
+                if constexpr (INBWD) glds16(inb ? yb + p_off[j] : zsrc, ldsY + (wq + 4 * j) * 1024);
+            }
+        }
+        if constexpr (INBWD) {
+            asm volatile("s_waitcnt vmcnt(0)" ::: "memory");
+            const float* ct = coef + tc.n * COEF_FLOATS + lchunk * 8;
+            unsigned* pw = (unsigned*)(ldsP + wq * 1024 + lane * 16);
+            const unsigned* yw = (const unsigned*)(ldsY + wq * 1024 + lane * 16);
+#pragma unroll
+            for (int q = 0; q < 4; ++q) {
+                const float2 cm = *(const float2*)(ct + 2 * q), cr = *(const float2*)(ct + 32 + 2 * q);
+                const float2 cs = *(const float2*)(ct + 64 + 2 * q), ch = *(const float2*)(ct + 96 + 2 * q);
+                const float2 c0 = *(const float2*)(ct + 128 + 2 * q), c1 = *(const float2*)(ct + 160 + 2 * q);
+#pragma unroll
+                for (int j = 0; j < NIP_W; ++j) {
+                    const int tv = (wq + 4 * j) * 16 + lrow;
+                    const int td = tv / (TH * TW), th = (tv / TW) % TH, tw = tv % TW;
+                    const bool inb = tc.d0 + td < p.D && tc.h0 + th < p.H && tc.w0 + tw < p.W;
+                    const bf16x2_t a = __builtin_bit_cast(bf16x2_t, pw[j * 1024 + q]);
+                    const bf16x2_t y = __builtin_bit_cast(bf16x2_t, yw[j * 1024 + q]);
+                    bf16x2_t o;
+                    {
+                        const float xv = (float)y[0];
+                        const float dz = inbwd_dz(inbwd_pre(xv, cs.x, ch.x), (float)a[0], p.slope);
+                        o[0] = (bf16_t)inbwd_dy(xv, dz, cm.x, cr.x, cs.x, c0.x, c1.x);
+                    }
+                    {
+                        const float xv = (float)y[1];
+                        const float dz = inbwd_dz(inbwd_pre(xv, cs.y, ch.y), (float)a[1], p.slope);
+                        o[1] = (bf16_t)inbwd_dy(xv, dz, cm.y, cr.y, cs.y, c0.y, c1.y);
+                    }
+                    pw[j * 1024 + q] = inb ? __builtin_bit_cast(unsigned, o) : 0u;
+                }
+            }
+            if (dog != nullptr) {
+                unsigned char* ob = dog + pvox * p.ldp * 2;
+#pragma unroll
+                for (int j = 0; j < NIP_W; ++j) {
+                    const int tv = (wq + 4 * j) * 16 + lrow;
+                    const int td = tv / (TH * TW), th = (tv / TW) % TH, tw = tv % TW;
+                    if (tc.d0 + td < p.D && tc.h0 + th < p.H && tc.w0 + tw < p.W)
+                        *(u32x4_t*)(ob + p_off[j]) = *(const u32x4_t*)(pw + j * 1024);
+                }
             }
         }
     };
@@ -258,6 +323,14 @@
     return tiles * ceil_div(p.M, 32) * ceil_div(p.K, 32) >= 2LL * msseg_num_cus();
 }
 
+bool msseg_k3wg_pp_inbwd_eligible(const K3WgParams& p) {
+    if (!p.da || !p.yraw || !p.stats || !p.red || p.M % 32 || p.N > INBWD_NMAX) return false;
+    if (p.ldyr != p.ldda || (p.dyout && p.lddo != p.ldda) || (((uintptr_t)p.yraw | (uintptr_t)p.dyout) & 15)) return false;
+    K3WgParams b = p;
+    b.pten = p.da; b.ldp = p.ldda;
+    return msseg_k3wg_pp_eligible(b);
+}
+
 int msseg_k3wg_pp_grid(const K3WgParams& p) {
     const int pairs = ceil_div(p.M, 32) * ceil_div(p.K, 32);
     const int tiles = p.N * ceil_div(p.D, TD) * ceil_div(p.H, TH) * ceil_div(p.W, TW);
@@ -273,13 +346,27 @@
     static const bool noload = getenv("MSSEG_K3PP_NOLOAD") != nullptr;
     K3WgParams pl = p;
     pl.dbg_noload = noload ? 1 : 0;
-    const int lds = 2 * GRP_BYTES;
-    static msseg_lds_attr_once attr[2];
-    if (!attr[0].ensure((const void*)k3wg_pp_kernel<0>, lds) || !attr[1].ensure((const void*)k3wg_pp_kernel<1>, lds))
+    const bool inbwd = p.da != nullptr;
+    if (inbwd) {
+        if (!msseg_k3wg_pp_inbwd_eligible(p)) MSSEG_FAIL(MSSEG_EINVAL, "conv3d_k3_wgrad_pp: in-backward operand not eligible");
+        pl.pten = p.da; pl.ldp = p.ldda;
+    }
+    const int lds = inbwd ? INBWD_LDS : 2 * GRP_BYTES;
+    static msseg_lds_attr_once attr[4];
+    if (!attr[0].ensure((const void*)k3wg_pp_kernel<0, 0>, 2 * GRP_BYTES) ||
+        !attr[1].ensure((const void*)k3wg_pp_kernel<1, 0>, 2 * GRP_BYTES) ||
+        !attr[2].ensure((const void*)k3wg_pp_kernel<0, 1>, INBWD_LDS) || !attr[3].ensure((const void*)k3wg_pp_kernel<1, 1>, INBWD_LDS))
         MSSEG_FAIL(MSSEG_ELAUNCH, "conv3d_k3_wgrad_pp: cannot set dynamic LDS size %d", lds);
     const int pairs = ceil_div(p.M, 32) * ceil_div(p.K, 32);
-    if (timing) hipLaunchKernelGGL(k3wg_pp_kernel<1>, dim3(gx, pairs, 1), dim3(NTHREADS), lds, stream, pl);
-    else MSSEG_KTIMED("k3wg_pp_kernel", stream, hipLaunchKernelGGL(k3wg_pp_kernel<0>, dim3(gx, pairs, 1), dim3(NTHREADS), lds, stream, pl));
+    const dim3 grid(gx, pairs, 1);
+    if (timing) {
+        if (inbwd) hipLaunchKernelGGL((k3wg_pp_kernel<1, 1>), grid, dim3(NTHREADS), lds, stream, pl);
+        else hipLaunchKernelGGL((k3wg_pp_kernel<1, 0>), grid, dim3(NTHREADS), lds, stream, pl);
+    } else if (inbwd) {
+        MSSEG_KTIMED("k3wg_pp_kernel", stream, hipLaunchKernelGGL((k3wg_pp_kernel<0, 1>), grid, dim3(NTHREADS), lds, stream, pl));
+    } else {
+        MSSEG_KTIMED("k3wg_pp_kernel", stream, hipLaunchKernelGGL((k3wg_pp_kernel<0, 0>), grid, dim3(NTHREADS), lds, stream, pl));
+    }
     MSSEG_CHECK_LAUNCH("conv3d_k3_wgrad_pp");
     return MSSEG_OK;
 }
diff --git a/medicalsemseg_amd/csrc/elementwise.hip b/medicalsemseg_amd/csrc/elementwise.hip
--- a/medicalsemseg_amd/csrc/elementwise.hip
+++ b/medicalsemseg_amd/csrc/elementwise.hip
@@ -1,4 +1,5 @@
 #include "common.h"
+#include "inorm_bwd.h"
 
 #include <stdarg.h>
 #include <string.h>
@@ -349,14 +350,6 @@
     float* ws; unsigned int* counter; float* dgamma; float* dbeta; int accumulate;
 };
 
-MSSEG_DEVFN void mean_rstd(const float* stats, int n, int C, int c, long long S, float eps, float& mean, float& rstd) {
-    const float inv = 1.0f / (float)S;
-    const float s = stats[((long long)n * C + c) * 2 + 0], s2 = stats[((long long)n * C + c) * 2 + 1];
-    mean = s * inv;
-    float var = s2 * inv - mean * mean;
-    var = var > 0.f ? var : 0.f;
-    rstd = rsqrtf(var + eps);
-}
 
 template <typename T, bool VEC, int MODE>
 __global__ __launch_bounds__(MODE == 1 ? RED_THREADS : 256) void instnorm_kernel(const NormParams p) {
@@ -375,7 +368,6 @@
     const T* resn = (MODE == 0 && p.res) ? (const T*)p.res + (long long)n * p.S * p.ldr : nullptr;
     T* dxn = (MODE == 2) ? (T*)p.dx + (long long)n * p.S * p.lddx : nullptr;
     T* drn = (MODE == 2 && p.dres) ? (T*)p.dres + (long long)n * p.S * p.lddres : nullptr;
-    const float invS = 1.0f / (float)p.S;
 
     for (int gbase = 0; gbase * W < p.C; gbase += p.groups) {
         const int gg = gbase + g;
@@ -384,15 +376,9 @@
 #pragma unroll
         for (int e = 0; e < W; ++e) {
             const int c = act ? gg * W + e : 0;
-            mean_rstd(p.stats, n, p.C, c, p.S, p.eps, mean[e], rstd[e]);
-            const float ga = p.gamma ? p.gamma[c] : 1.f;
-            sc[e] = rstd[e] * ga;
-            sh[e] = (p.beta ? p.beta[c] : 0.f) - mean[e] * sc[e];
+            const InBwdCoef k = inbwd_coef(p.stats, MODE == 2 ? p.red : nullptr, p.gamma, p.beta, n, p.C, c, p.S, p.eps);
+            mean[e] = k.mean; rstd[e] = k.rstd; sc[e] = k.sc; sh[e] = k.sh; k0[e] = k.k0; k1[e] = k.k1;
             a0[e] = a1[e] = 0.f;
-            if constexpr (MODE == 2) {
-                k0[e] = p.red[((long long)n * p.C + c) * 2 + 0] * invS;
-                k1[e] = p.red[((long long)n * p.C + c) * 2 + 1] * invS;
-            }
         }
         if (act && rl < p.rows_par) {
 #pragma unroll 4
@@ -442,21 +428,21 @@
                             for (int e = 0; e < W; ++e) yv[e] = c.v[e];
                         } else {
 #pragma unroll
-                            for (int e = 0; e < W; ++e) yv[e] = xv[e] * sc[e] + sh[e];
+                            for (int e = 0; e < W; ++e) yv[e] = inbwd_pre(xv[e], sc[e], sh[e]);
                         }
                     } else {
                         dv[0] = DT<T>::ld(dyn + r * p.lddy + gg);
-                        yv[0] = (yn != nullptr) ? DT<T>::ld(yn + r * p.ldy + gg) : xv[0] * sc[0] + sh[0];
+                        yv[0] = (yn != nullptr) ? DT<T>::ld(yn + r * p.ldy + gg) : inbwd_pre(xv[0], sc[0], sh[0]);
                     }
 #pragma unroll
                     for (int e = 0; e < W; ++e) {
-                        const float dz = yv[e] > 0.f ? dv[e] : dv[e] * p.slope;
-                        const float xh = (xv[e] - mean[e]) * rstd[e];
+                        const float dz = inbwd_dz(yv[e], dv[e], p.slope);
                         if constexpr (MODE == 1) {
+                            const float xh = (xv[e] - mean[e]) * rstd[e];
                             a0[e] += dz;
                             a1[e] += dz * xh;
                         } else {
-                            o[e] = sc[e] * (dz - k0[e] - xh * k1[e]);
+                            o[e] = inbwd_dy(xv[e], dz, mean[e], rstd[e], sc[e], k0[e], k1[e]);
                             dv[e] = dz;
                         }
                     }
diff --git a/medicalsemseg_amd/csrc/igemm_wgrad.hip b/medicalsemseg_amd/csrc/igemm_wgrad.hip
--- a/medicalsemseg_amd/csrc/igemm_wgrad.hip
+++ b/medicalsemseg_amd/csrc/igemm_wgrad.hip
@@ -583,6 +583,95 @@
                               : launch_wg_k3<bf16_t>(p, rp, workspace, workspace_bytes, (hipStream_t)stream);
 }
 
+static void inbwd_k3_params(K3WgParams& pp, const void* x, long long ldx, const void* da, const void* yraw, long long ldd,
+                            const float* stats, const float* red, const float* gamma, const float* beta, float eps, float slope,
+                            void* dy, int N, int D, int H, int W, int Cin, int Cout) {
+    pp.qten = x; pp.ldq = ldx; pp.pten = da; pp.ldp = ldd;
+    pp.N = N; pp.D = D; pp.H = H; pp.W = W; pp.M = Cout; pp.K = Cin; pp.kblks = ceil_div(Cin, 32);
+    pp.da = da; pp.ldda = ldd; pp.yraw = yraw; pp.ldyr = ldd; pp.dyout = dy; pp.lddo = ldd;
+    pp.stats = stats; pp.red = red; pp.gamma = gamma; pp.beta = beta; pp.eps = eps; pp.slope = slope;
+}
+
+static bool inbwd_k3_ok(const K3WgParams& pp) {
+    static const int pp_min_dim = getenv("MSSEG_K3WG_MINDIM") ? atoi(getenv("MSSEG_K3WG_MINDIM")) : 8;
+    const int mnd = pp.D < pp.H ? (pp.D < pp.W ? pp.D : pp.W) : (pp.H < pp.W ? pp.H : pp.W);
+    return mnd >= pp_min_dim && msseg_k3wg_pp_inbwd_eligible(pp);
+}
+
+int msseg_conv3d_k3_wgrad_inbwd_kernel(int N, int D, int H, int W, int Cin, int Cout, int dtype) {
+    if (dtype != MSSEG_BF16) return 0;
+    const float f = 0.f;
+    K3WgParams pp{};
+    inbwd_k3_params(pp, (const void*)256, Cin, (const void*)256, (const void*)256, Cout, &f, &f, nullptr, nullptr, 0.f, 0.f,
+                    (void*)256, N, D, H, W, Cin, Cout);
+    return inbwd_k3_ok(pp) ? 1 : 0;
+}
+
+int msseg_conv3d_k3_wgrad_inbwd(const void* x, long long ldx, const void* da, const void* yraw, long long ldd,
+                                const float* stats, const float* red, const float* gamma, const float* beta, float eps,
+                                float slope, void* dy, float* dw, int N, int D, int H, int W, int Cin, int Cout,
+                                int accumulate, void* workspace, size_t workspace_bytes, int dtype, msseg_stream_t stream) {
+    int rc = wg_check(x, ldx, da, ldd, dw, workspace, dtype);
+    if (rc) return rc;
+    if (!yraw || !stats || !red) MSSEG_FAIL(MSSEG_EINVAL, "conv3d_k3_wgrad_inbwd: null pointer");
+    K3WgParams pp{};
+    inbwd_k3_params(pp, x, ldx, da, yraw, ldd, stats, red, gamma, beta, eps, slope, dy, N, D, H, W, Cin, Cout);
+    if (dtype != MSSEG_BF16 || !inbwd_k3_ok(pp)) MSSEG_FAIL(MSSEG_EINVAL, "conv3d_k3_wgrad_inbwd: shape / operands not eligible");
+    const int pairs = ceil_div(Cout, 32) * ceil_div(Cin, 32);
+    int gx = msseg_k3wg_pp_grid(pp);
+    const long long fit = (long long)(workspace_bytes / ((size_t)27 * 32 * 32 * 4 * pairs));
+    if (fit < 8) MSSEG_FAIL(MSSEG_EWORKSPACE, "conv3d_k3_wgrad_inbwd: workspace too small");
+    if (gx > fit) gx = (int)(fit & ~7LL);
+    pp.slabs = (float*)workspace;
+    rc = msseg_k3wg_pp_launch(pp, gx, (hipStream_t)stream);
+    if (rc) return rc;
+    ReduceParams rp{};
+    rp.dw = dw; rp.M = Cout; rp.M0 = Cout; rp.T = 27; rp.K = Cin; rp.K0 = Cin;
+    rp.s_m1 = 0; rp.s_m0 = (long long)Cin * 27; rp.s_t = 1; rp.s_k1 = 0; rp.s_k0 = 27; rp.accumulate = accumulate;
+    rp.slabs = pp.slabs; rp.mblks = ceil_div(Cout, 32); rp.kblks = ceil_div(Cin, 32); rp.nslots = gx; rp.cbw = 32;
+    return launch_reduce(rp, (hipStream_t)stream);
+}
+
+static void inbwd_stem_params(StemWgParams& sp, const void* x, long long ldx, const void* da, const void* yraw, long long ldd,
+                              const float* stats, const float* red, const float* gamma, const float* beta, float eps,
+                              float slope, int N, int D, int H, int W, int Cout) {
+    sp.x = x; sp.ldx = ldx; sp.dy = nullptr; sp.lddy = ldd; sp.N = N; sp.D = D; sp.H = H; sp.W = W; sp.M = Cout;
+    sp.da = da; sp.ldda = ldd; sp.yraw = yraw; sp.ldyr = ldd;
+    sp.stats = stats; sp.red = red; sp.gamma = gamma; sp.beta = beta; sp.eps = eps; sp.slope = slope;
+}
+
+int msseg_conv3d_stem_wgrad_inbwd_kernel(int N, int D, int H, int W, int Cout, int dtype) {
+    if (!msseg_stem_eligible(dtype, 1, Cout, 3, 1, 1, 1, Cout, (const void*)256)) return 0;
+    const float f = 0.f;
+    StemWgParams sp{};
+    inbwd_stem_params(sp, (const void*)256, 1, (const void*)256, (const void*)256, Cout, &f, &f, nullptr, nullptr, 0.f, 0.f,
+                      N, D, H, W, Cout);
+    return msseg_stem_wgrad_inbwd_eligible(sp) ? 1 : 0;
+}
+
+int msseg_conv3d_stem_wgrad_inbwd(const void* x, long long ldx, const void* da, const void* yraw, long long ldd,
+                                  const float* stats, const float* red, const float* gamma, const float* beta, float eps,
+                                  float slope, float* dw, int N, int D, int H, int W, int Cout, int accumulate,
+                                  void* workspace, size_t workspace_bytes, int dtype, msseg_stream_t stream) {
+    if (!x || !da || !yraw || !stats || !red || !dw || !workspace) MSSEG_FAIL(MSSEG_EINVAL, "conv3d_stem_wgrad_inbwd: null pointer");
+    StemWgParams sp{};
+    inbwd_stem_params(sp, x, ldx, da, yraw, ldd, stats, red, gamma, beta, eps, slope, N, D, H, W, Cout);
+    if (!msseg_stem_eligible(dtype, 1, Cout, 3, 1, 1, ldx, ldd, da) || !msseg_stem_wgrad_inbwd_eligible(sp))
+        MSSEG_FAIL(MSSEG_EINVAL, "conv3d_stem_wgrad_inbwd: shape / operands not eligible");
+    if (workspace_bytes < (size_t)8 * 4096 * ceil_div(Cout, 32)) MSSEG_FAIL(MSSEG_EWORKSPACE, "conv3d_stem_wgrad_inbwd: workspace too small");
+    int gx = msseg_stem_wgrad_grid(sp);
+    const long long fit = (long long)(workspace_bytes / ((size_t)4096 * ceil_div(Cout, 32)));
+    if (gx > fit) gx = (int)(fit & ~7LL);
+    sp.slabs = (float*)workspace;
+    int rc = msseg_stem_wgrad_launch(sp, gx, (hipStream_t)stream);
+    if (rc) return rc;
+    ReduceParams rq{};
+    rq.dw = dw; rq.M = Cout; rq.M0 = Cout; rq.T = 1; rq.K = 27; rq.K0 = 1;
+    rq.s_m0 = 27; rq.s_k1 = 1; rq.s_k0 = 27; rq.accumulate = accumulate;
+    rq.slabs = sp.slabs; rq.mblks = ceil_div(Cout, 32); rq.kblks = 1; rq.nslots = gx; rq.cbw = 32;
+    return launch_reduce(rq, (hipStream_t)stream);
+}
+
 int msseg_conv3d_k1_wgrad(const void* x, long long ldx, const void* dy, long long lddy, float* dw, long long NV, int Cin,
                           int Cout, int accumulate, void* workspace, size_t workspace_bytes, int dtype,
                           msseg_stream_t stream) {
diff --git a/medicalsemseg_amd/csrc/inorm_bwd.h b/medicalsemseg_amd/csrc/inorm_bwd.h
--- /dev/null
+++ b/medicalsemseg_amd/csrc/inorm_bwd.h
@@ -0,0 +1,38 @@
+#pragma once
+#include "common.h"
+
+struct InBwdCoef { float mean, rstd, sc, sh, k0, k1; };
+
+MSSEG_DEVFN void mean_rstd(const float* stats, int n, int C, int c, long long S, float eps, float& mean, float& rstd) {
+    const float inv = 1.0f / (float)S;
+    const float s = stats[((long long)n * C + c) * 2 + 0], s2 = stats[((long long)n * C + c) * 2 + 1];
+    mean = s * inv;
+    float var = s2 * inv - mean * mean;
+    var = var > 0.f ? var : 0.f;
+    rstd = rsqrtf(var + eps);
+}
+
+MSSEG_DEVFN InBwdCoef inbwd_coef(const float* stats, const float* red, const float* gamma, const float* beta, int n, int C,
+                                 int c, long long S, float eps) {
+    InBwdCoef k;
+    mean_rstd(stats, n, C, c, S, eps, k.mean, k.rstd);
+    const float ga = gamma ? gamma[c] : 1.f;
+    k.sc = k.rstd * ga;
+    k.sh = (beta ? beta[c] : 0.f) - k.mean * k.sc;
+    k.k0 = k.k1 = 0.f;
+    if (red) {
+        const float invS = 1.0f / (float)S;
+        k.k0 = red[((long long)n * C + c) * 2 + 0] * invS;
+        k.k1 = red[((long long)n * C + c) * 2 + 1] * invS;
+    }
+    return k;
+}
+
+MSSEG_DEVFN float inbwd_pre(float x, float sc, float sh) { return x * sc + sh; }
+
+MSSEG_DEVFN float inbwd_dz(float pre, float da, float slope) { return pre > 0.f ? da : da * slope; }
+
+MSSEG_DEVFN float inbwd_dy(float x, float dz, float mean, float rstd, float sc, float k0, float k1) {
+    const float xh = (x - mean) * rstd;
+    return sc * (dz - k0 - xh * k1);
+}
diff --git a/medicalsemseg_amd/csrc/k3pp.h b/medicalsemseg_amd/csrc/k3pp.h
--- a/medicalsemseg_amd/csrc/k3pp.h
+++ b/medicalsemseg_amd/csrc/k3pp.h
@@ -43,8 +43,14 @@
     float* slabs;
     int N, D, H, W, M, K, kblks;
     int dbg_noload;
+    const void* da; long long ldda;
+    const void* yraw; long long ldyr;
+    void* dyout; long long lddo;
+    const float* stats; const float* red; const float* gamma; const float* beta;
+    float eps, slope;
 };
 bool msseg_k3wg_pp_eligible(const K3WgParams& p);
+bool msseg_k3wg_pp_inbwd_eligible(const K3WgParams& p);
 int msseg_k3wg_pp_grid(const K3WgParams& p);
 int msseg_k3wg_pp_launch(const K3WgParams& p, int gx, hipStream_t stream);
 
@@ -63,11 +69,16 @@
     const void* dy; long long lddy;
     float* slabs;
     int N, D, H, W, M;
+    const void* da; long long ldda;
+    const void* yraw; long long ldyr;
+    const float* stats; const float* red; const float* gamma; const float* beta;
+    float eps, slope;
 };
 bool msseg_stem_eligible(int dtype, int Cin, int Cout, int k, int s, int pd, long long ldx, long long ldy, const void* y);
 int msseg_stem_fwd_launch(const StemParams& p, hipStream_t stream);
 int msseg_stem_wgrad_grid(const StemWgParams& p);
 int msseg_stem_wgrad_launch(const StemWgParams& p, int gx, hipStream_t stream);
+bool msseg_stem_wgrad_inbwd_eligible(const StemWgParams& p);
 
 bool msseg_deconv2_fast_eligible(int dtype, int Cin, int Cout, const void* coarse, long long ldc, const void* fine,
                                  long long ldf, const float* bias);
diff --git a/medicalsemseg_amd/csrc/stem_conv.hip b/medicalsemseg_amd/csrc/stem_conv.hip
--- a/medicalsemseg_amd/csrc/stem_conv.hip
+++ b/medicalsemseg_amd/csrc/stem_conv.hip
@@ -1,3 +1,4 @@
+#include "inorm_bwd.h"
 #include "k3pp.h"
 
 namespace {
@@ -218,6 +219,11 @@
 constexpr int XP = 24;
 constexpr int XS_ELEMS = PD * PH * XP;
 constexpr int P_BYTES = TD * TH * TW * 64;
+constexpr int W_BUF_BYTES = P_BYTES + 3 * XS_ELEMS * 2 + 64;
+constexpr int W_COEF_FLOATS = 6 * 32;
+constexpr int W_INBWD_NMAX = 4;
+constexpr int W_INBWD_LDS = 2 * W_BUF_BYTES + 2 * P_BYTES + W_INBWD_NMAX * W_COEF_FLOATS * 4;
+typedef __attribute__((ext_vector_type(2))) __bf16 bf16x2_t;
 
 __device__ u32x4_t g_stem_zero_chunk;
 
@@ -229,14 +235,18 @@
     return __builtin_amdgcn_ds_read_tr16_b64_v4bf16((__attribute__((address_space(3))) bf16x4_t*)p);
 }
 
+template <int INBWD>
 __global__ __launch_bounds__(W_THREADS) void stem_wgrad_kernel(const StemWgParams p) {
     extern __shared__ __attribute__((aligned(256))) unsigned char smem[];
-    constexpr int BUF_BYTES = P_BYTES + 3 * XS_ELEMS * 2 + 64;
+    constexpr int BUF_BYTES = W_BUF_BYTES;
     lds_u8* smem3 = (lds_u8*)smem;
     const int tid = threadIdx.x, lane = tid & 63;
     const int wave = __builtin_amdgcn_readfirstlane(tid >> 6);
     const int mblk = blockIdx.y;
-    const unsigned char* dyg = (const unsigned char*)p.dy + mblk * 64;
+    const unsigned char* dyg = (const unsigned char*)(INBWD ? p.da : p.dy) + mblk * 64;
+    const unsigned char* yrg = (const unsigned char*)p.yraw + mblk * 64;
+    unsigned char* ldsY = smem + 2 * BUF_BYTES;
+    float* coef = (float*)(ldsY + 2 * P_BYTES);
     const unsigned short* __restrict__ xg = (const unsigned short*)p.x;
     Sched sc;
     sc.init(p.N, p.D, p.H, p.W);
@@ -253,19 +263,22 @@
         unsigned char* base = smem + buf * BUF_BYTES;
         const long long pvox = (((long long)tc.n * p.D + tc.d0) * p.H + tc.h0) * p.W + tc.w0;
         const unsigned char* pb = dyg + pvox * p.lddy * 2;
+        const unsigned char* yb = yrg + pvox * p.lddy * 2;
         const bool full = tc.d0 + TD <= p.D && tc.h0 + TH <= p.H && tc.w0 + TW <= p.W;
         const unsigned char* zsrc = (const unsigned char*)&g_stem_zero_chunk;
         const bool ch_ok = mblk * 32 + (lane & 3) * 8 < p.M;
 #pragma unroll
         for (int j = 0; j < 4; ++j) {
             const unsigned char* src = pb + p_off[j];
-            if (!ch_ok) src = zsrc;
+            const unsigned char* ysrc = yb + p_off[j];
+            if (!ch_ok) src = ysrc = zsrc;
             if (!full) {
                 const int tv = (wave + 4 * j) * 16 + (lane >> 2);
                 const int td = tv / (TH * TW), th = (tv / TW) % TH, tw = tv % TW;
-                if (!(tc.d0 + td < p.D && tc.h0 + th < p.H && tc.w0 + tw < p.W)) src = zsrc;
+                if (!(tc.d0 + td < p.D && tc.h0 + th < p.H && tc.w0 + tw < p.W)) src = ysrc = zsrc;
             }
             glds16(src, base + (wave + 4 * j) * 1024);
+            if constexpr (INBWD) glds16(ysrc, ldsY + buf * P_BYTES + (wave + 4 * j) * 1024);
         }
 #pragma unroll
         for (int it = 0; it < 3; ++it) {
@@ -276,6 +289,40 @@
             st[it] = inb ? xg[((((long long)tc.n * p.D + d) * p.H + h) * p.W + w) * p.ldx] : (unsigned short)0;
         }
     };
+    auto commit_p = [&](const TileCo& tc, int buf) {
+        if constexpr (INBWD) {
+            const float* ct = coef + tc.n * W_COEF_FLOATS + (lane & 3) * 8;
+            unsigned* pw = (unsigned*)(smem + buf * BUF_BYTES + wave * 1024 + lane * 16);
+            const unsigned* yw = (const unsigned*)(ldsY + buf * P_BYTES + wave * 1024 + lane * 16);
+            const bool ch_ok = mblk * 32 + (lane & 3) * 8 < p.M;
+#pragma unroll
+            for (int q = 0; q < 4; ++q) {
+                const float2 cm = *(const float2*)(ct + 2 * q), cr = *(const float2*)(ct + 32 + 2 * q);
+                const float2 cs = *(const float2*)(ct + 64 + 2 * q), ch = *(const float2*)(ct + 96 + 2 * q);
+                const float2 c0 = *(const float2*)(ct + 128 + 2 * q), c1 = *(const float2*)(ct + 160 + 2 * q);
+#pragma unroll
+                for (int j = 0; j < 4; ++j) {
+                    const int tv = (wave + 4 * j) * 16 + (lane >> 2);
+                    const int td = tv / (TH * TW), th = (tv / TW) % TH, tw = tv % TW;
+                    const bool inb = ch_ok && tc.d0 + td < p.D && tc.h0 + th < p.H && tc.w0 + tw < p.W;
+                    const bf16x2_t a = __builtin_bit_cast(bf16x2_t, pw[j * 1024 + q]);
+                    const bf16x2_t y = __builtin_bit_cast(bf16x2_t, yw[j * 1024 + q]);
+                    bf16x2_t o;
+                    {
+                        const float xv = (float)y[0];
+                        const float dz = inbwd_dz(inbwd_pre(xv, cs.x, ch.x), (float)a[0], p.slope);
+                        o[0] = (bf16_t)inbwd_dy(xv, dz, cm.x, cr.x, cs.x, c0.x, c1.x);
+                    }
+                    {
+                        const float xv = (float)y[1];
+                        const float dz = inbwd_dz(inbwd_pre(xv, cs.y, ch.y), (float)a[1], p.slope);
+                        o[1] = (bf16_t)inbwd_dy(xv, dz, cm.y, cr.y, cs.y, c0.y, c1.y);
+                    }
+                    pw[j * 1024 + q] = inb ? __builtin_bit_cast(unsigned, o) : 0u;
+                }
+            }
+        }
+    };
     auto commit_x = [&](int buf) {
         unsigned short* xs = (unsigned short*)(smem + buf * BUF_BYTES + P_BYTES);
 #pragma unroll
@@ -305,11 +352,22 @@
 #pragma unroll
     for (int e = 0; e < 16; ++e) acc[e] = 0.f;
 
+    if constexpr (INBWD) {
+        const long long S = (long long)p.D * p.H * p.W;
+        for (int i = tid; i < p.N * 32; i += W_THREADS) {
+            const int n = i >> 5, cl = i & 31, c = mblk * 32 + cl;
+            const InBwdCoef k = inbwd_coef(p.stats, p.red, p.gamma, p.beta, n, p.M, c < p.M ? c : 0, S, p.eps);
+            float* t = coef + n * W_COEF_FLOATS + cl;
+            t[0] = k.mean; t[32] = k.rstd; t[64] = k.sc; t[96] = k.sh; t[128] = k.k0; t[160] = k.k1;
+        }
+        __syncthreads();
+    }
     if (sc.n_my > 0) {
         load_tile(sc.tile(0), 0);
         commit_x(0);
     }
     asm volatile("s_waitcnt vmcnt(0)" ::: "memory");
+    if (sc.n_my > 0) commit_p(sc.tile(0), 0);
     __syncthreads();
     for (int k = 0; k < sc.n_my; ++k) {
         const int buf = k & 1;
@@ -327,6 +385,7 @@
         }
         if (k + 1 < sc.n_my) commit_x(buf ^ 1);
         asm volatile("s_waitcnt vmcnt(0)" ::: "memory");
+        if (k + 1 < sc.n_my) commit_p(sc.tile(k + 1), buf ^ 1);
         __syncthreads();
     }
     float* xch = (float*)smem;
@@ -384,11 +443,20 @@
     return gx;
 }
 
+bool msseg_stem_wgrad_inbwd_eligible(const StemWgParams& p) {
+    return p.da && p.yraw && p.stats && p.red && p.M % 32 == 0 && p.N <= W_INBWD_NMAX && p.lddy % 8 == 0 &&
+           (((uintptr_t)p.da | (uintptr_t)p.yraw) & 15) == 0;
+}
+
 int msseg_stem_wgrad_launch(const StemWgParams& p, int gx, hipStream_t stream) {
-    const int lds = 2 * (P_BYTES + 3 * XS_ELEMS * 2 + 64);
-    static msseg_lds_attr_once attr;
-    if (!attr.ensure((const void*)stem_wgrad_kernel, lds)) MSSEG_FAIL(MSSEG_ELAUNCH, "stem_wgrad: cannot set dynamic LDS size %d", lds);
-    hipLaunchKernelGGL(stem_wgrad_kernel, dim3(gx, ceil_div(p.M, 32)), dim3(W_THREADS), lds, stream, p);
+    const bool inbwd = p.da != nullptr;
+    if (inbwd && !msseg_stem_wgrad_inbwd_eligible(p)) MSSEG_FAIL(MSSEG_EINVAL, "stem_wgrad: in-backward operand not eligible");
+    const int lds = inbwd ? W_INBWD_LDS : 2 * W_BUF_BYTES;
+    static msseg_lds_attr_once attr[2];
+    if (!attr[0].ensure((const void*)stem_wgrad_kernel<0>, 2 * W_BUF_BYTES) || !attr[1].ensure((const void*)stem_wgrad_kernel<1>, W_INBWD_LDS))
+        MSSEG_FAIL(MSSEG_ELAUNCH, "stem_wgrad: cannot set dynamic LDS size %d", lds);
+    if (inbwd) hipLaunchKernelGGL((stem_wgrad_kernel<1>), dim3(gx, ceil_div(p.M, 32)), dim3(W_THREADS), lds, stream, p);
+    else hipLaunchKernelGGL((stem_wgrad_kernel<0>), dim3(gx, ceil_div(p.M, 32)), dim3(W_THREADS), lds, stream, p);
     MSSEG_CHECK_LAUNCH("stem_wgrad");
     return MSSEG_OK;
 }
diff --git a/medicalsemseg_amd/hip.py b/medicalsemseg_amd/hip.py
--- a/medicalsemseg_amd/hip.py
+++ b/medicalsemseg_amd/hip.py
@@ -94,6 +94,12 @@
     "msseg_wgrad_workspace_bytes": ([_i, _i, _i], _sz),
     "msseg_conv3d_k3_wgrad_kernel": ([_i, _i, _i, _i, _i, _i, _i], _i),
     "msseg_conv3d_k3_wgrad": ([_vp, _ll, _vp, _ll, _vp, _i, _i, _i, _i, _i, _i, _i, _vp, _sz, _i, _vp], _i),
+    "msseg_conv3d_k3_wgrad_inbwd_kernel": ([_i, _i, _i, _i, _i, _i, _i], _i),
+    "msseg_conv3d_k3_wgrad_inbwd": ([_vp, _ll, _vp, _vp, _ll, _vp, _vp, _vp, _vp, _f, _f, _vp, _vp, _i, _i, _i, _i, _i, _i,
+                                     _i, _vp, _sz, _i, _vp], _i),
+    "msseg_conv3d_stem_wgrad_inbwd_kernel": ([_i, _i, _i, _i, _i, _i], _i),
+    "msseg_conv3d_stem_wgrad_inbwd": ([_vp, _ll, _vp, _vp, _ll, _vp, _vp, _vp, _vp, _f, _f, _vp, _i, _i, _i, _i, _i, _i,
+                                       _vp, _sz, _i, _vp], _i),
     "msseg_conv3d_k1_wgrad": ([_vp, _ll, _vp, _ll, _vp, _ll, _i, _i, _i, _vp, _sz, _i, _vp], _i),
     "msseg_conv3d_gather_wgrad": ([_vp, _ll, _vp, _ll, _vp, _i, _i, _i, _i, _i, _i, _i, _i, _i, _i, _vp, _sz, _i, _vp], _i),
     "msseg_deconv_k2s2_wgrad": ([_vp, _ll, _vp, _ll, _vp, _i, _i, _i, _i, _i, _i, _i, _vp, _sz, _i, _vp], _i),
@@ -725,6 +731,45 @@
     TIMER.launch(key, 2.0 * nv * 27 * cin * cout, nv * (cin + cout) * x.element_size() + 27 * cin * cout * 4, go)
 
 
+def conv3d_k3_wgrad_inbwd_ok(x, yraw, cin, cout) -> bool:
+    return bool(x.is_cuda and x.dtype == torch.bfloat16 and yraw.dtype == torch.bfloat16 and
+                lib().msseg_conv3d_k3_wgrad_inbwd_kernel(*x.shape[:4], cin, cout, BF16) == 1)
+
+
+def conv3d_k3_wgrad_inbwd(x, yraw, da, stats, red, gamma, beta, slope, eps, dy, dw, cin, cout, accumulate=False):
+    _need_gpu(x, yraw, da, dw, red)
+    if ld(da) != ld(yraw) or (dy is not None and ld(dy) != ld(da)):
+        raise ValueError("conv3d_k3_wgrad_inbwd: da, y_raw and dy must share one row stride")
+    N, D, H, W = x.shape[:4]
+    ws = _wg_ws(cout, 27, cin, x.device)
+    nv = N * D * H * W
+
+    def go():
+        _ck(lib().msseg_conv3d_k3_wgrad_inbwd(_p(x), ld(x), _p(da), _p(yraw), ld(da), _p(stats), _p(red), _p(gamma),
+                                              _p(beta), eps, slope, _p(dy), _p(dw), N, D, H, W, cin, cout,
+                                              int(accumulate), _p(ws), ws.numel(), dt(x), _stream()),
+            "conv3d_k3_wgrad_inbwd")
+    TIMER.launch("conv3d_k3_wgrad/v3", 2.0 * nv * 27 * cin * cout,
+                 nv * (cin + 2 * cout + (cout if dy is not None else 0)) * x.element_size() + 27 * cin * cout * 4, go)
+    return dy
+
+
+def conv3d_stem_wgrad_inbwd_ok(x, yraw, cout) -> bool:
+    return bool(x.is_cuda and x.dtype == torch.bfloat16 and yraw.dtype == torch.bfloat16 and x.shape[-1] == 1 and
+                lib().msseg_conv3d_stem_wgrad_inbwd_kernel(*x.shape[:4], cout, BF16) == 1)
+
+
+def conv3d_stem_wgrad_inbwd(x, yraw, da, stats, red, gamma, beta, slope, eps, dw, cout, accumulate=False):
+    _need_gpu(x, yraw, da, dw, red)
+    if ld(da) != ld(yraw):
+        raise ValueError("conv3d_stem_wgrad_inbwd: da and y_raw must share one row stride")
+    N, D, H, W = x.shape[:4]
+    ws = _wg_ws(cout, 1, 27, x.device)
+    _ck(lib().msseg_conv3d_stem_wgrad_inbwd(_p(x), ld(x), _p(da), _p(yraw), ld(da), _p(stats), _p(red), _p(gamma),
+                                            _p(beta), eps, slope, _p(dw), N, D, H, W, cout, int(accumulate), _p(ws),
+                                            ws.numel(), dt(x), _stream()), "conv3d_stem_wgrad_inbwd")
+
+
 def conv3d_k1_wgrad(x, dy, dw, cin, cout, accumulate=False):
     _need_gpu(x, dy, dw)
     nv = x.numel() // x.shape[-1]
diff --git a/medicalsemseg_amd/layers.py b/medicalsemseg_amd/layers.py
--- a/medicalsemseg_amd/layers.py
+++ b/medicalsemseg_amd/layers.py
@@ -288,9 +288,10 @@
         vol = tuple(dy.shape[:4])
         return hip.lib().msseg_conv3d_k3_kernel(*vol, self.cout, self.cin, hip.BF16) == (4 if self.cout == 48 else 3)
 
-    def bwd(self, x, dy, need_dx=True, dx_out=None, bias_grad_is_zero=False, next_norm=None, accumulate_dx=False):
+    def bwd(self, x, dy, need_dx=True, dx_out=None, bias_grad_is_zero=False, next_norm=None, accumulate_dx=False,
+            wgrad_done=False):
         dtype = x.dtype
-        if self.w.requires_grad:
+        if self.w.requires_grad and not wgrad_done:
             g, acc = _grad_buf(self.w)
             if self._gather(dtype):
                 WGRAD_SIDE.run(lambda: hip.conv3d_gather_wgrad(x, dy, g, self.cin, self.cout, 3, 1, 1, acc), x, dy)
@@ -582,11 +583,35 @@
 
     def bwd(self, saved, da, need_dx=True, red=None, next_saved=None, next_cna=None):
         x, y, stats, a = saved
-        dy = self.norm.bwd(y, stats, a, da, red=red)
+        fused = self._wgrad_inbwd_ok(x, y, da, red, need_dx)
+        if fused:
+            cv, nm = self.conv, self.norm
+            g, acc = _grad_buf(cv.w)
+            if cv._gather(x.dtype):
+                hip.conv3d_stem_wgrad_inbwd(x, y, da, stats, red, nm.gamma, nm.beta, nm.slope, nm.eps, g, cv.cout, acc)
+                return cv.bwd(x, None, False, bias_grad_is_zero=True, wgrad_done=True)
+            dy = torch.empty(y.shape, dtype=y.dtype, device=y.device)
+            hip.conv3d_k3_wgrad_inbwd(x, y, da, stats, red, nm.gamma, nm.beta, nm.slope, nm.eps, dy, g, cv.cin, cv.cout, acc)
+        else:
+            dy = self.norm.bwd(y, stats, a, da, red=red)
         if next_cna is not None and need_dx:
             nx, ny, nstats, na = next_saved
-            return self.conv.bwd(x, dy, True, bias_grad_is_zero=True, next_norm=(next_cna.norm, ny, nstats, na))
-        return self.conv.bwd(x, dy, need_dx, bias_grad_is_zero=True)
+            return self.conv.bwd(x, dy, True, bias_grad_is_zero=True, next_norm=(next_cna.norm, ny, nstats, na),
+                                 wgrad_done=fused)
+        return self.conv.bwd(x, dy, need_dx, bias_grad_is_zero=True, wgrad_done=fused)
+
+    INBWD_MIN_DIM = 48
+    K3_INBWD = bool(os.environ.get("MSSEG_WGRAD_INBWD_K3"))
+
+    def _wgrad_inbwd_ok(self, x, y, da, red, need_dx) -> bool:
+        cv = self.conv
+        if (red is None or red is APPLIED or x.dtype != torch.bfloat16 or not cv.w.requires_grad
+                or WGRAD_SIDE.active is not None or os.environ.get("MSSEG_NO_WGRAD_INBWD")
+                or min(y.shape[1:4]) < self.INBWD_MIN_DIM or da.stride() != y.stride()):
+            return False
+        if cv._gather(x.dtype):
+            return cv.cin == 1 and not need_dx and hip.conv3d_stem_wgrad_inbwd_ok(x, y, cv.cout)
+        return self.K3_INBWD and hip.conv3d_k3_wgrad_inbwd_ok(x, y, cv.cin, cv.cout)
 
 
 def maxpool_fwd(x):
```

Result: no change. 537.6 vol/s, median of 6 (+0.6%).
